# drscotthawley/SPNet

Hardware: AMD Instinct MI355X
Metric: training images/sec on 512×384 fake-ESPI, Xception backbone, 1/2/4/8 GPU (higher is better)
Workload: dtype f32 (bf16x3 MFMA for pointwise fwd/dgrad/wgrad GEMMs); 1 GPU; configs[1]: Xception, fake-ESPI 512x384 (HxW 384x512x1, model_type 'big'), batch 32 per GPU, full train step (augment+fwd+custom_loss+bwd+Adam+l2); global_batch=32, pool_frames_per_gpu=4096, parallelism=dp1, n_ranks_seen=1, devices_visible=1, wgrad_overlap=True

## Files before the change

### include/spnet_hip.h

```cpp
#ifndef SPNET_HIP_H
#define SPNET_HIP_H
#include <stdint.h>
#ifdef __cplusplus
extern "C" {
#endif

int spnet_gemm_f32(const float* A, int a_major, int lda, const float* B, int b_major, int ldb, float* C,
                   int ldc, int M, int N, int K, int split_k, float* workspace, long ws_floats,
                   const float* bias, int tile, void* stream);
long spnet_bf16x3_kp(int K);
long spnet_bf16x3_plane_elems(long R, int K);
int spnet_split_bf16x3(const float* W, void* planes, int K, int N, void* stream);
int spnet_split_rows_bf16x3(const float* A, long lda, void* planes, long R, int K, void* stream);
int spnet_split_bf16x3_batched(const void* jobs, int njobs, long max_elems, void* stream);
int spnet_gemm_bf16x3_fwd(const float* A, int lda, const void* planes, float* C, int ldc, int M, int N, int K, void* stream);
int spnet_gemm_bf16x3_fwd_colstats(const float* A, int lda, const void* planes, float* C, int ldc, int M, int N, int K,
                                   float* colstats, int* stat_rows, void* stream);
int spnet_gemm_bf16x3_pp(const void* a_planes, const void* b_planes, float* C, int ldc, int M, int N, int K, float* colstats,
                         int* stat_rows, void* stream);
long spnet_gemm_bf16x3_wgrad_ksplit(int cin, int cout, int M, int nbatch);
int spnet_gemm_bf16x3_pp_dwfwd(const void* z_planes, const void* w_planes, int B, int H, int W, int cin, int cout,
                               const float* scale_shift, int relu_next, const float* w_next, void* out_planes, void* stream);
long spnet_gemm_bf16x3_dwbwd_rows(long M);
long spnet_gemm_bf16x3_dwbwd_ok(int H, int W, int cin);
int spnet_gemm_bf16x3_pp_dwbwd(const void* dy_planes, const void* w_planes, int B, int H, int W, int cin, int cout,
                               const float* x_fwd, const float* w, float* dx, int relu_in, const float* add, float* partial,
                               const float* in_scale, const float* in_shift, const float* bn_mean, const float* bn_invstd,
                               float* bn_partial, const float* bn_x, void* stream);
int spnet_gemm_bf16x3_wgrad_batched(const void* jobs, int nbatch, int cin, int cout, int M, int ksplit, void* stream);
int spnet_gemm_f32_accumulate(const float* A, int a_major, int lda, const float* B, int b_major, int ldb, float* C,
                              int ldc, int M, int N, int K, int tile, void* stream);

int spnet_gemm_f32_colstats(const float* A, int a_major, int lda, const float* B, int b_major, int ldb,
                            float* C, int ldc, int M, int N, int K, int tile, float* colstats,
                            int* stat_rows, void* stream);
int spnet_gemm_f32_batched(const float* A0, const float* B0, float* C0, const long long* offsets, int nbatch,
                           int a_major, int lda, int b_major, int ldb, int ldc, int M, int N, int K, int tile,
                           void* stream);
long spnet_gemm_batched_ksplit(int M, int N, int K, int nbatch, int* tile_out);
int spnet_gemm_f32_batched_splitk(const float* A0, const float* B0, float* C0, const long long* offsets, int nbatch,
                                  int a_major, int lda, int b_major, int ldb, int ldc, int M, int N, int K, int tile,
                                  int ksplit, float* workspace, long ws_floats, void* stream);

int spnet_gemm_f32_bnblend(const float* g, const float* yp, const float* coef, int cld, int lda, const float* B,
                           int ldb, float* C, int ldc, int M, int N, int K, int tile, float* dy_out, void* stream);

int spnet_conv3x3_fwd(const float* x, const float* w, float* y, int B, int H, int W, int cin, int cout,
                      void* stream);
int spnet_conv3x3_dgrad(const float* dy, const float* w, float* dx, int B, int H, int W, int cin, int cout,
                        void* stream);
long spnet_conv3x3_wgrad_ws(int B, int H, int W, int cin, int cout);
int spnet_conv3x3_wgrad(const float* x, const float* dy, float* dw, int B, int H, int W, int cin, int cout,
                        float* workspace, long ws_floats, void* stream);
int spnet_transpose_batched(const void* jobs, int njobs, int max_rows, int max_cols, void* stream);
int spnet_reduce_slabs(const float* ws, int nslab, int M, int N, float* out, int ldc, void* stream);
int spnet_gather_s2(const float* x, float* xs, int B, int H, int W, int C, void* stream);
int spnet_scatter_add_s2(const float* dxs, float* dx, int B, int H, int W, int C, void* stream);

int spnet_reduce_rows(const float* in, int P, int L, float* out, void* stream);
int spnet_reduce_rows_ws(const float* in, int P, int L, float* out, float* scratch, long scratch_floats, void* stream);
int spnet_reduce_rows_batched(const void* jobs, int njobs, int max_L, void* stream);
long spnet_dwconv3x3_strided_ws(int B, int H, int W, int C, int stride);
int spnet_dwconv3x3_strided(int op, const float* a, const float* b, float* out, int B, int H, int W, int C, int stride,
                            float* workspace, void* stream);
int spnet_dwconv3x3_tiled_fwd(const float* x, const float* w, float* y, int B, int H, int W, int C,
                              int relu_in, const float* in_scale, const float* in_shift, void* stream);
int spnet_dwconv3x3_tiled_fwd_bnfin(const float* x, const float* w, float* y, int B, int H, int W, int C, int relu_in,
                                    const float* partial, int rows, long M, const float* gamma, const float* beta,
                                    float* moving_mean, float* moving_var, float* save_mean, float* save_invstd,
                                    float* scale_shift, float eps, float momentum, void* stream);
int spnet_dwconv3x3_tiled_fwd_x3(const float* x, const float* w, void* y_planes, int B, int H, int W, int C,
                                 int relu_in, const float* in_scale, const float* in_shift, void* stream);
int spnet_dwconv3x3_tiled_fwd_bnfin_x3(const float* x, const float* w, void* y_planes, int B, int H, int W, int C, int relu_in,
                                       const float* partial, int rows, long M, const float* gamma, const float* beta,
                                       float* moving_mean, float* moving_var, float* save_mean, float* save_invstd,
                                       float* scale_shift, float eps, float momentum, void* stream);
int spnet_dwconv3x3_stream_fwd_x3(const float* x, const float* w, void* y_planes, int B, int H, int W, int C, int relu_in,
                                  const float* in_scale, const float* in_shift, int rows_per_seg, void* stream);
long spnet_dwconv3x3_tiled_bwd_ws(int B, int H, int W, int C);
long spnet_dwconv3x3_tiled_rows(int B, int H, int W, int C);
int spnet_dwconv3x3_tiled_bwd(const float* dy, const float* x_fwd, const float* w, float* dx, float* dw,
                              int B, int H, int W, int C, int relu_in, const float* add, float* workspace,
                              const float* in_scale, const float* in_shift, const float* bn_mean,
                              const float* bn_invstd, float* bn_partial, const float* bn_x, void* stream);
long spnet_dwconv3x3_prefers_stream(int B, int H, int W, int C, int backward);
long spnet_dwconv3x3_stream_rows(int B, int H, int W, int C, int rows_per_seg);
long spnet_dwconv3x3_stream_bwd_ws(int B, int H, int W, int C, int rows_per_seg);
int spnet_dwconv3x3_stream_fwd(const float* x, const float* w, float* y, int B, int H, int W, int C, int relu_in,
                               const float* in_scale, const float* in_shift, int rows_per_seg, void* stream);
int spnet_dwconv3x3_stream_bwd(const float* dy, const float* x_fwd, const float* w, float* dx, float* dw, int B, int H,
                               int W, int C, int relu_in, const float* add, float* workspace, const float* in_scale,
                               const float* in_shift, const float* bn_mean, const float* bn_invstd, float* bn_partial,
                               const float* bn_x, int rows_per_seg, void* stream);

long spnet_bn_ws(long M, int C);
int spnet_bn_fwd_train(const float* x, long M, int C, const float* gamma, const float* beta,
                       float* moving_mean, float* moving_var, float* save_mean, float* save_invstd,
                       float* scale_shift, int act, const float* residual, int res_bcast, float* y,
                       float eps, float momentum, float* workspace, void* stream);
int spnet_bn_fwd_infer(const float* x, long M, int C, const float* gamma, const float* beta,
                       const float* moving_mean, const float* moving_var, float* scale_shift, int act,
                       const float* residual, int res_bcast, float* y, float eps, void* stream);
int spnet_bn_bwd(const float* x, const float* dy, long M, int C, const float* gamma, const float* beta,
                 const float* save_mean, const float* save_invstd, int act, float* dx, float* dgamma,
                 float* dbeta, float* coeffs, float* workspace, void* stream);
int spnet_bn_finalize_fwd(float* partial, int P, long M, int C, const float* gamma, const float* beta,
                          float* moving_mean, float* moving_var, float* save_mean, float* save_invstd,
                          float* scale_shift, float eps, float momentum, void* stream);
int spnet_bn_infer_coeffs(int C, const float* gamma, const float* beta, const float* moving_mean,
                          const float* moving_var, float* scale_shift, float eps, void* stream);
int spnet_bn_apply(const float* x, long M, int C, const float* scale_shift, int act, const float* residual,
                   int res_bcast, float* y, void* stream);
int spnet_bn_finalize_apply(float* partial, int P, const float* x, long M, int C, const float* gamma,
                            const float* beta, float* moving_mean, float* moving_var, float* save_mean,
                            float* save_invstd, float* scale_shift, int act, const float* residual, float* y, float eps,
                            float momentum, void* stream);
int spnet_bn_finalize_apply_ld(float* partial, int P, const float* x, long M, int C, const float* gamma,
                               const float* beta, float* moving_mean, float* moving_var, float* save_mean,
                               float* save_invstd, float* scale_shift, int act, const float* residual, float* y, long ldy,
                               float eps, float momentum, void* stream);
int spnet_bn_fwd_train_ld(const float* x, long M, int C, const float* gamma, const float* beta, float* moving_mean,
                          float* moving_var, float* save_mean, float* save_invstd, float* scale_shift, int act,
                          const float* residual, int res_bcast, float* y, long ldy, float eps, float momentum,
                          float* workspace, void* stream);
int spnet_bn_fwd_infer_ld(const float* x, long M, int C, const float* gamma, const float* beta, const float* moving_mean,
                          const float* moving_var, float* scale_shift, int act, const float* residual, int res_bcast,
                          float* y, long ldy, float eps, void* stream);
int spnet_bn_bwd_from_partials(const float* x, const float* dy, long M, int C, const float* gamma,
                               const float* beta, const float* save_mean, const float* save_invstd, int P,
                               const float* partial, float* dx, float* dgamma, float* dbeta, float* coeffs,
                               void* stream);
int spnet_bn_bwd_x3(const float* x, const float* dy, long M, int C, const float* gamma, const float* beta,
                    const float* save_mean, const float* save_invstd, int act, void* dx_planes, float* dgamma,
                    float* dbeta, float* coeffs, float* workspace, void* stream);
int spnet_bn_bwd_from_partials_x3(const float* x, const float* dy, long M, int C, const float* gamma,
                                  const float* beta, const float* save_mean, const float* save_invstd, int P,
                                  const float* partial, void* dx_planes, float* dgamma, float* dbeta, float* coeffs,
                                  void* stream);

int spnet_bn_bwd_coeffs_from_partials(int P, const float* partial, long M, int C, const float* gamma,
                                      const float* save_mean, const float* save_invstd, float* dgamma, float* dbeta,
                                      float* coef, int cld, void* stream);
int spnet_bn_bwd_coeffs(const float* x, const float* dy, long M, int C, const float* gamma, const float* beta,
                        const float* save_mean, const float* save_invstd, float* dgamma, float* dbeta, float* coef,
                        int cld, float* workspace, void* stream);

int spnet_maxpool3x3s2_add_fwd(const float* x, const float* residual, float* y, uint32_t* idx4, int B,
                               int H, int W, int C, const float* x_ss, const float* r_ss, void* stream);
int spnet_maxpool3x3s2_bwd(const float* dy, const uint32_t* idx4, float* dx, int B, int H, int W, int C,
                           void* stream);
long spnet_maxpool3x3s2_bwd_rows(int B, int H, int W, int C, int max_rows);
int spnet_maxpool3x3s2_bwd_bnsums(const float* dy, const uint32_t* idx4, float* dx, int B, int H, int W, int C,
                                  const float* yp, const float* mean, const float* invstd, float* partial, int rows,
                                  void* stream);
int spnet_avgpool2_fwd(const float* x, float* y, int B, int H, int W, int C, void* stream);
int spnet_avgpool2_bwd(const float* dy, float* dx, int B, int H, int W, int C, void* stream);

int spnet_maxpool3x3s2_valid_fwd(const float* x, float* y, uint32_t* idx4, int B, int H, int W, int C, void* stream);
int spnet_maxpool3x3s2_valid_bwd(const float* dy, const uint32_t* idx4, float* dx, int B, int H, int W, int C, void* stream);
int spnet_avgpool3x3s1_same(const float* in, float* out, int B, int H, int W, int C, int backward, void* stream);
int spnet_patches(const float* in, float* out, int B, int H, int W, int C, int KH, int KW, int stride, int same, int backward,
                  void* stream);
int spnet_patches_ld(const float* in, long ldx, float* out, int B, int H, int W, int C, int KH, int KW, int stride, int same,
                     void* stream);
int spnet_conv_gemm_f32(const float* x, long ldx, const float* Wk, float* y, int ldy, int B, int H, int W, int C, int Cout,
                        int KH, int KW, int stride, int same, const float* bias, int tile, float* colstats,
                        int* stat_rows, void* stream);
long spnet_grad_bnsums_rows(long npix, int max_rows);
int spnet_patches_bwd_bnsums(const float* dcol, float* dx, int B, int H, int W, int C, int KH, int KW, int stride, int same,
                             const float* y, const float* yp, const float* mean, const float* invstd, int relu,
                             float* partial, int rows, void* stream);
int spnet_copy_cols_bnsums(const float* src, int lds, float* dst, long M, int C, const float* y, long ldy, const float* yp,
                           const float* mean, const float* invstd, int relu, float* partial, int rows, void* stream);
int spnet_patches_bwd_bnsums_ld(const float* dcol, float* dx, long lddx, int B, int H, int W, int C, int KH, int KW, int stride,
                                int same, const float* y, long ldy, const float* yp, long ldyp, const float* mean,
                                const float* invstd, int relu, float* partial, long ldp, int rows, void* stream);
int spnet_copy_cols_bnsums_ld(const float* src, int lds, float* dst, long ldd, long M, int C, const float* y, long ldy,
                              const float* yp, long ldyp, const float* mean, const float* invstd, int relu, float* partial,
                              long ldp, int rows, void* stream);
int spnet_copy_cols_batched(const void* jobs, int njobs, long max_elems, void* stream);
int spnet_resadd(const float* x, const float* up, float* y, long n, float scale, int relu, void* stream);
int spnet_resadd_bwd(const float* y, const float* g, float* dx, float* dup, long n, float scale, int relu, void* stream);
int spnet_copy_cols(const float* src, int lds, float* dst, int ldd, long rows, int cols, int accumulate, void* stream);

int spnet_conv3x3_small(int op, int cin, int cout, int stride, int same, const float* a, const float* b,
                        float* out, int B, int H, int W, float* workspace, long ws_floats, void* stream);

int spnet_stem_head(int op, const float* x, const float* a, float* out, float* out2, int B, int H, int W,
                    float* workspace, long ws_floats, void* stream);

int spnet_ellipse_loss(const float* y_true, const float* y_pred, float* grad, float* parts,
                       float* loss_out, int B, int ncols, int hybrid, void* stream);
int spnet_selective_sigmoid(float* y, float* grad, int B, int ncols, int start, int step, int backward, void* stream);
int spnet_decode(const float* y_norm, const float* means, const float* ranges, float* out, int B,
                 int ncols, int sigmoid_noobj, void* stream);

int spnet_ellipse_iou(const float* yp, const float* yt, long npairs, int nx, int ny, double* iou, void* stream);

int spnet_calc_errors(const float* yp, const float* yt, long N, int ncols, int* counts, float* pix_err, void* stream);

int spnet_adam_step(float* p, const float* g, float* m, float* v, long n, long l2_n, float lr_t,
                    float beta1, float beta2, float eps, float l2, float grad_scale, const float* mask,
                    float* sq_scratch, float* l2_loss_out, const float* lr_t_dev, void* stream);
long spnet_adam_parts(long n);
int spnet_adam_part(float* p, const float* g, float* m, float* v, long n, long l2_n, float lr_t, float beta1, float beta2,
                    float eps, float l2, float grad_scale, const float* mask, float* sq_partial, const float* lr_t_dev,
                    void* stream);
int spnet_adam_l2_sum(const float* sq_partial, int count, float l2, float* l2_loss_out, void* stream);

int spnet_u8_to_input(const unsigned char* src, float* dst, long n, void* stream);
int spnet_resize_u8(const unsigned char* src, int N, int H, int W, const int* xtab, int xtaps, const int* ytab, int ytaps,
                    int OH, int OW, unsigned char* out_u8, float* out_f, void* stream);
int spnet_gather_rows(const float* src, long src_rows, const void* index, int idx_bytes, float* dst, int n, long L,
                      void* stream);

int spnet_minmax(const float* x, int N, long hw, float* mm, float* scratch, void* stream);
int spnet_cutout(const float* src, const int* src_index, float* dst, int N, int H, int W,
                 const int* rects, const float* vals, const int* nrect, void* stream);
int spnet_saltpepper(float* x, int N, int H, int W, const int* coords, int n_salt, int n_pepper,
                     const int* flag, const float* mm, void* stream);
int spnet_gaussian_blur(const float* src, float* dst, int N, int H, int W, const int* ksize, void* stream);
int spnet_warp_affine(const float* src, float* dst, int N, int H, int W, int C, const float* minv,
                      void* stream);
int spnet_warp_affine_fixed(const float* src, float* dst, int N, int H, int W, int C, const int* xrow, const int* xcol,
                            void* stream);
int spnet_warp_chain_u8(const unsigned char* src, int n_src, const int* sel, const void* params, int N, int H, int W,
                        unsigned char* out_u8, float* out_f, void* stream);
int spnet_dropout(const float* x, float* y, long n, unsigned seed, float rate, const unsigned* seed_dev,
                  void* stream);

int spnet_fake_espi(const float* waves, const float* nodes, const int* nnode, int N, int H, int W, unsigned seed,
                    int noise, float* out_f, unsigned char* out_u8, void* stream);

long spnet_bandpass_ws(int N, int H, int W);
int spnet_bandpass_project(const void* x, int x_kind, int N, int H, int W, const int* flip, float* win, float* ws,
                           void* stream);
int spnet_bandpass_apply(const void* x, int x_kind, const int* sel, int n_src, int N, int H, int W, const float* table,
                         int n_table, const int* row, const float* s, float* out_f, int f_kind, unsigned char* out_u8,
                         float* ws, void* stream);

int spnet_gemm_f32_bnrelu(const float* x, int ldx, const float* coef, int cld, const float* W, int ldw, float* Y, int ldy,
                          int M, int N, int K, int tile, float* colstats, int* stat_rows, void* stream);
int spnet_pad_nhwc(const float* in, float* out, int B, int H, int W, int C, int pt, int pb, int pl, int pr, int backward,
                   void* stream);
long spnet_dense_conv7_ws(int B, int H, int W);
int spnet_dense_conv7(int op, const float* a, const float* b, float* out, int B, int H, int W, float* workspace,
                      long ws_floats, void* stream);
long spnet_dense_rows(long M);
int spnet_dense_colsums_ld(const float* x, long ldx, long M, int C, float* partial, void* stream);
int spnet_dense_coeffs(int c, int cld, const float* gamma, const float* beta, const float* mean, const float* invstd,
                       const float* bmean, const float* bvar, float* mm, float* mv, float* coef, float eps, float momentum,
                       int training, void* stream);
int spnet_dense_apply_ld(const float* x, long ldx, long M, int C, const float* coef, int cld, int relu, float* y, long ldy,
                         void* stream);
int spnet_dense_consumer_bwd(const float* dz, long ldz, const float* x, long ldx, long M, int c, const float* coef, int cld,
                             const float* mean, const float* invstd, const float* gamma, int relu, float* G, long ldg,
                             float* partial, void* stream);
int spnet_dense_consumer_fin(const float* partial, int P, int c, const float* gamma, float* dgamma, float* dbeta, float* u,
                             float* v, void* stream);
int spnet_dense_producer_fin(const float* G, long ldg, const float* u, const float* v, const float* x, long ldx,
                             const float* mean, const float* invstd, long M, int c0, int c1, float* out, long ldo,
                             void* stream);

#ifdef __cplusplus
}
#endif
#endif
```

### spnet_amd/_lib.py

```python
import ctypes
import os
from ctypes import POINTER, byref, c_float, c_int, c_long, c_uint, c_void_p

_HERE = os.path.dirname(os.path.abspath(__file__))
LIB_PATH = os.environ.get("SPNET_HIP_LIB") or os.path.join(_HERE, "lib", "libspnet_hip.so")

if not os.path.exists(LIB_PATH):
    raise ImportError(
        "spnet_amd: %s is missing -- build it with `python -c 'import __graft_entry__ as g; g.build()'` "
        "or `make -C spnet_amd/csrc` (hipcc, gfx950).  There is no CPU fallback." % LIB_PATH)

import numpy as np
import torch

_lib = ctypes.CDLL(LIB_PATH)

P = c_void_p

_SIGS = {
    "spnet_gemm_f32": (c_int, [P, c_int, c_int, P, c_int, c_int, P, c_int, c_int, c_int, c_int, c_int, P, c_long, P, c_int, P]),
    "spnet_bf16x3_kp": (c_long, [c_int]),
    "spnet_bf16x3_plane_elems": (c_long, [c_long, c_int]),
    "spnet_split_bf16x3": (c_int, [P, P, c_int, c_int, P]),
    "spnet_split_rows_bf16x3": (c_int, [P, c_long, P, c_long, c_int, P]),
    "spnet_gemm_bf16x3_pp": (c_int, [P, P, P, c_int, c_int, c_int, c_int, P, P, P]),
    "spnet_gemm_bf16x3_wgrad_ksplit": (c_long, [c_int, c_int, c_int, c_int]),
    "spnet_gemm_bf16x3_dwbwd_rows": (c_long, [c_long]),
    "spnet_gemm_bf16x3_dwbwd_ok": (c_long, [c_int, c_int, c_int]),
    "spnet_gemm_bf16x3_pp_dwbwd": (c_int, [P, P, c_int, c_int, c_int, c_int, c_int, P, P, P, c_int, P, P, P, P, P, P, P, P, P]),
    "spnet_gemm_bf16x3_pp_dwfwd": (c_int, [P, P, c_int, c_int, c_int, c_int, c_int, P, c_int, P, P, P]),
    "spnet_gemm_bf16x3_wgrad_batched": (c_int, [P, c_int, c_int, c_int, c_int, c_int, P]),
    "spnet_split_bf16x3_batched": (c_int, [P, c_int, c_long, P]),
    "spnet_gemm_bf16x3_fwd": (c_int, [P, c_int, P, P, c_int, c_int, c_int, c_int, P]),
    "spnet_gemm_bf16x3_fwd_colstats": (c_int, [P, c_int, P, P, c_int, c_int, c_int, c_int, P, P, P]),
    "spnet_gemm_f32_accumulate": (c_int, [P, c_int, c_int, P, c_int, c_int, P, c_int, c_int, c_int, c_int, c_int, P]),
    "spnet_conv3x3_fwd": (c_int, [P, P, P, c_int, c_int, c_int, c_int, c_int, P]),
    "spnet_conv3x3_dgrad": (c_int, [P, P, P, c_int, c_int, c_int, c_int, c_int, P]),
    "spnet_conv3x3_wgrad_ws": (c_long, [c_int, c_int, c_int, c_int, c_int]),
    "spnet_conv3x3_wgrad": (c_int, [P, P, P, c_int, c_int, c_int, c_int, c_int, P, c_long, P]),
    "spnet_reduce_slabs": (c_int, [P, c_int, c_int, c_int, P, c_int, P]),
    "spnet_transpose_batched": (c_int, [P, c_int, c_int, c_int, P]),
    "spnet_gather_s2": (c_int, [P, P, c_int, c_int, c_int, c_int, P]),
    "spnet_scatter_add_s2": (c_int, [P, P, c_int, c_int, c_int, c_int, P]),
    "spnet_dwconv3x3_strided_ws": (c_long, [c_int, c_int, c_int, c_int, c_int]),
    "spnet_dwconv3x3_strided": (c_int, [c_int, P, P, P, c_int, c_int, c_int, c_int, c_int, P, P]),
    "spnet_reduce_rows": (c_int, [P, c_int, c_int, P, P]),
    "spnet_reduce_rows_ws": (c_int, [P, c_int, c_int, P, P, c_long, P]),
    "spnet_reduce_rows_batched": (c_int, [P, c_int, c_int, P]),
    "spnet_dwconv3x3_tiled_fwd": (c_int, [P, P, P, c_int, c_int, c_int, c_int, c_int, P, P, P]),
    "spnet_dwconv3x3_tiled_fwd_bnfin": (c_int, [P, P, P, c_int, c_int, c_int, c_int, c_int, P, c_int, c_long, P, P, P, P, P, P, P,
                                                c_float, c_float, P]),
    "spnet_dwconv3x3_tiled_fwd_x3": (c_int, [P, P, P, c_int, c_int, c_int, c_int, c_int, P, P, P]),
    "spnet_dwconv3x3_tiled_fwd_bnfin_x3": (c_int, [P, P, P, c_int, c_int, c_int, c_int, c_int, P, c_int, c_long, P, P, P, P, P, P, P,
                                                   c_float, c_float, P]),
    "spnet_dwconv3x3_stream_fwd_x3": (c_int, [P, P, P, c_int, c_int, c_int, c_int, c_int, P, P, c_int, P]),
    "spnet_dwconv3x3_tiled_bwd_ws": (c_long, [c_int, c_int, c_int, c_int]),
    "spnet_dwconv3x3_tiled_rows": (c_long, [c_int, c_int, c_int, c_int]),
    "spnet_dwconv3x3_tiled_bwd": (c_int, [P, P, P, P, P, c_int, c_int, c_int, c_int, c_int, P, P, P, P, P, P, P, P, P]),
    "spnet_dwconv3x3_prefers_stream": (c_long, [c_int, c_int, c_int, c_int, c_int]),
    "spnet_dwconv3x3_stream_rows": (c_long, [c_int, c_int, c_int, c_int, c_int]),
    "spnet_dwconv3x3_stream_bwd_ws": (c_long, [c_int, c_int, c_int, c_int, c_int]),
    "spnet_dwconv3x3_stream_fwd": (c_int, [P, P, P, c_int, c_int, c_int, c_int, c_int, P, P, c_int, P]),
    "spnet_dwconv3x3_stream_bwd": (c_int, [P, P, P, P, P, c_int, c_int, c_int, c_int, c_int, P, P, P, P, P, P, P, P, c_int, P]),
    "spnet_bn_finalize_fwd": (c_int, [P, c_int, c_long, c_int, P, P, P, P, P, P, P, c_float, c_float, P]),
    "spnet_bn_infer_coeffs": (c_int, [c_int, P, P, P, P, P, c_float, P]),
    "spnet_bn_apply": (c_int, [P, c_long, c_int, P, c_int, P, c_int, P, P]),
    "spnet_bn_finalize_apply": (c_int, [P, c_int, P, c_long, c_int, P, P, P, P, P, P, P, c_int, P, P, c_float, c_float, P]),
    "spnet_bn_finalize_apply_ld": (c_int, [P, c_int, P, c_long, c_int, P, P, P, P, P, P, P, c_int, P, P, c_long, c_float, c_float, P]),
    "spnet_bn_bwd_from_partials": (c_int, [P, P, c_long, c_int, P, P, P, P, c_int, P, P, P, P, P, P]),
    "spnet_bn_bwd_from_partials_x3": (c_int, [P, P, c_long, c_int, P, P, P, P, c_int, P, P, P, P, P, P]),
    "spnet_bn_bwd_x3": (c_int, [P, P, c_long, c_int, P, P, P, P, c_int, P, P, P, P, P, P]),
    "spnet_gemm_f32_colstats": (c_int, [P, c_int, c_int, P, c_int, c_int, P, c_int, c_int, c_int, c_int, c_int, P, P, P]),
    "spnet_gemm_f32_bnblend": (c_int, [P, P, P, c_int, c_int, P, c_int, P, c_int, c_int, c_int, c_int, c_int, P, P]),
    "spnet_bn_bwd_coeffs_from_partials": (c_int, [c_int, P, c_long, c_int, P, P, P, P, P, P, c_int, P]),
    "spnet_bn_bwd_coeffs": (c_int, [P, P, c_long, c_int, P, P, P, P, P, P, P, c_int, P, P]),
    "spnet_gemm_f32_batched": (c_int, [P, P, P, P, c_int, c_int, c_int, c_int, c_int, c_int, c_int, c_int, c_int, c_int, P]),
    "spnet_gemm_batched_ksplit": (c_long, [c_int, c_int, c_int, c_int, P]),
    "spnet_gemm_f32_batched_splitk": (c_int, [P, P, P, P, c_int, c_int, c_int, c_int, c_int, c_int, c_int, c_int, c_int, c_int,
                                              c_int, P, c_long, P]),
    "spnet_bn_ws": (c_long, [c_long, c_int]),
    "spnet_bn_fwd_train": (c_int, [P, c_long, c_int, P, P, P, P, P, P, P, c_int, P, c_int, P, c_float, c_float, P, P]),
    "spnet_bn_fwd_infer": (c_int, [P, c_long, c_int, P, P, P, P, P, c_int, P, c_int, P, c_float, P]),
    "spnet_bn_fwd_train_ld": (c_int, [P, c_long, c_int, P, P, P, P, P, P, P, c_int, P, c_int, P, c_long, c_float, c_float, P, P]),
    "spnet_bn_fwd_infer_ld": (c_int, [P, c_long, c_int, P, P, P, P, P, c_int, P, c_int, P, c_long, c_float, P]),
    "spnet_bn_bwd": (c_int, [P, P, c_long, c_int, P, P, P, P, c_int, P, P, P, P, P, P]),
    "spnet_maxpool3x3s2_add_fwd": (c_int, [P, P, P, P, c_int, c_int, c_int, c_int, P, P, P]),
    "spnet_maxpool3x3s2_bwd": (c_int, [P, P, P, c_int, c_int, c_int, c_int, P]),
    "spnet_maxpool3x3s2_bwd_rows": (c_long, [c_int, c_int, c_int, c_int, c_int]),
    "spnet_maxpool3x3s2_bwd_bnsums": (c_int, [P, P, P, c_int, c_int, c_int, c_int, P, P, P, P, c_int, P]),
    "spnet_maxpool3x3s2_valid_fwd": (c_int, [P, P, P, c_int, c_int, c_int, c_int, P]),
    "spnet_maxpool3x3s2_valid_bwd": (c_int, [P, P, P, c_int, c_int, c_int, c_int, P]),
    "spnet_avgpool3x3s1_same": (c_int, [P, P, c_int, c_int, c_int, c_int, c_int, P]),
    "spnet_patches": (c_int, [P, P, c_int, c_int, c_int, c_int, c_int, c_int, c_int, c_int, c_int, P]),
    "spnet_patches_ld": (c_int, [P, c_long, P, c_int, c_int, c_int, c_int, c_int, c_int, c_int, c_int, P]),
    "spnet_conv_gemm_f32": (c_int, [P, c_long, P, P, c_int, c_int, c_int, c_int, c_int, c_int, c_int, c_int, c_int, c_int, P, c_int, P, P, P]),
    "spnet_grad_bnsums_rows": (c_long, [c_long, c_int]),
    "spnet_patches_bwd_bnsums": (c_int, [P, P, c_int, c_int, c_int, c_int, c_int, c_int, c_int, c_int, P, P, P, P, c_int, P,
                                         c_int, P]),
    "spnet_copy_cols_bnsums": (c_int, [P, c_int, P, c_long, c_int, P, c_long, P, P, P, c_int, P, c_int, P]),
    "spnet_patches_bwd_bnsums_ld": (c_int, [P, P, c_long, c_int, c_int, c_int, c_int, c_int, c_int, c_int, c_int, P, c_long, P,
                                            c_long, P, P, c_int, P, c_long, c_int, P]),
    "spnet_copy_cols_bnsums_ld": (c_int, [P, c_int, P, c_long, c_long, c_int, P, c_long, P, c_long, P, P, c_int, P, c_long,
                                          c_int, P]),
    "spnet_copy_cols_batched": (c_int, [P, c_int, c_long, P]),
    "spnet_resadd": (c_int, [P, P, P, c_long, c_float, c_int, P]),
    "spnet_resadd_bwd": (c_int, [P, P, P, P, c_long, c_float, c_int, P]),
    "spnet_copy_cols": (c_int, [P, c_int, P, c_int, c_long, c_int, c_int, P]),
    "spnet_avgpool2_fwd": (c_int, [P, P, c_int, c_int, c_int, c_int, P]),
    "spnet_avgpool2_bwd": (c_int, [P, P, c_int, c_int, c_int, c_int, P]),
    "spnet_conv3x3_small": (c_int, [c_int, c_int, c_int, c_int, c_int, P, P, P, c_int, c_int, c_int, P, c_long, P]),
    "spnet_stem_head": (c_int, [c_int, P, P, P, P, c_int, c_int, c_int, P, c_long, P]),
    "spnet_ellipse_loss": (c_int, [P, P, P, P, P, c_int, c_int, c_int, P]),
    "spnet_selective_sigmoid": (c_int, [P, P, c_int, c_int, c_int, c_int, c_int, P]),
    "spnet_decode": (c_int, [P, P, P, P, c_int, c_int, c_int, P]),
    "spnet_ellipse_iou": (c_int, [P, P, c_long, c_int, c_int, P, P]),
    "spnet_calc_errors": (c_int, [P, P, c_long, c_int, P, P, P]),
    "spnet_adam_step": (c_int, [P, P, P, P, c_long, c_long, c_float, c_float, c_float, c_float, c_float, c_float, P, P, P, P, P]),
    "spnet_adam_parts": (c_long, [c_long]),
    "spnet_adam_part": (c_int, [P, P, P, P, c_long, c_long, c_float, c_float, c_float, c_float, c_float, c_float, P, P, P, P]),
    "spnet_adam_l2_sum": (c_int, [P, c_int, c_float, P, P]),
    "spnet_u8_to_input": (c_int, [P, P, c_long, P]),
    "spnet_resize_u8": (c_int, [P, c_int, c_int, c_int, P, c_int, P, c_int, c_int, c_int, P, P, P]),
    "spnet_gather_rows": (c_int, [P, c_long, P, c_int, P, c_int, c_long, P]),
    "spnet_minmax": (c_int, [P, c_int, c_long, P, P, P]),
    "spnet_cutout": (c_int, [P, P, P, c_int, c_int, c_int, P, P, P, P]),
    "spnet_saltpepper": (c_int, [P, c_int, c_int, c_int, P, c_int, c_int, P, P, P]),
    "spnet_gaussian_blur": (c_int, [P, P, c_int, c_int, c_int, P, P]),
    "spnet_warp_affine": (c_int, [P, P, c_int, c_int, c_int, c_int, P, P]),
    "spnet_warp_affine_fixed": (c_int, [P, P, c_int, c_int, c_int, c_int, P, P, P]),
    "spnet_warp_chain_u8": (c_int, [P, c_int, P, P, c_int, c_int, c_int, P, P, P]),
    "spnet_fake_espi": (c_int, [P, P, P, c_int, c_int, c_int, c_uint, c_int, P, P, P]),
    "spnet_dropout": (c_int, [P, P, c_long, c_uint, c_float, P, P]),
    "spnet_bandpass_ws": (c_long, [c_int, c_int, c_int]),
    "spnet_bandpass_project": (c_int, [P, c_int, c_int, c_int, c_int, P, P, P, P]),
    "spnet_bandpass_apply": (c_int, [P, c_int, P, c_int, c_int, c_int, c_int, P, c_int, P, P, P, c_int, P, P, P]),
    "spnet_gemm_f32_bnrelu": (c_int, [P, c_int, P, c_int, P, c_int, P, c_int, c_int, c_int, c_int, c_int, P, P, P]),
    "spnet_pad_nhwc": (c_int, [P, P, c_int, c_int, c_int, c_int, c_int, c_int, c_int, c_int, c_int, P]),
    "spnet_dense_conv7_ws": (c_long, [c_int, c_int, c_int]),
    "spnet_dense_conv7": (c_int, [c_int, P, P, P, c_int, c_int, c_int, P, c_long, P]),
    "spnet_dense_rows": (c_long, [c_long]),
    "spnet_dense_colsums_ld": (c_int, [P, c_long, c_long, c_int, P, P]),
    "spnet_dense_coeffs": (c_int, [c_int, c_int, P, P, P, P, P, P, P, P, P, c_float, c_float, c_int, P]),
    "spnet_dense_apply_ld": (c_int, [P, c_long, c_long, c_int, P, c_int, c_int, P, c_long, P]),
    "spnet_dense_consumer_bwd": (c_int, [P, c_long, P, c_long, c_long, c_int, P, c_int, P, P, P, c_int, P, c_long, P, P]),
    "spnet_dense_consumer_fin": (c_int, [P, c_int, c_int, P, P, P, P, P, P]),
    "spnet_dense_producer_fin": (c_int, [P, c_long, P, P, P, c_long, P, P, c_long, c_int, c_int, P, c_long, P]),
}

EXPORTS = tuple(_SIGS)


class HipError(RuntimeError):
    pass


_TRACER = [None]


def set_tracer(tracer):
    _TRACER[0] = tracer


def _bind(name, restype, argtypes):
    fn = getattr(_lib, name)
    fn.restype = restype
    fn.argtypes = argtypes
    if restype is not c_int:
        return fn

    def checked(*args):
        tr = _TRACER[0]
        if tr is None:
            rc = fn(*args)
        else:
            tok = tr(name, args, None)
            rc = fn(*args)
            tr(name, args, tok)
        if rc != 0:
            raise HipError("%s failed with hipError_t %d" % (name, rc))
    checked.__name__ = name
    return checked


for _n, (_r, _a) in _SIGS.items():
    globals()[_n] = _bind(_n, _r, _a)


def _public_stream():
    return torch.cuda.current_stream().cuda_stream


def _resolve_current_stream():
    raw = getattr(torch._C, "_cuda_getCurrentRawStream", None)
    dev = getattr(torch._C, "_cuda_getDevice", None)
    if raw is None or dev is None:
        return _public_stream, "public"
    return (lambda: raw(dev())), "raw"


current_stream, STREAM_ACCESSOR = _resolve_current_stream()


def gather_rows(src, index, dst):
    n = int(index.numel())
    rows = int(src.shape[0])
    L_ = src.numel() // max(rows, 1)
    if dst.numel() != n * L_ or src.dtype != torch.float32 or dst.dtype != torch.float32 or not (src.is_contiguous() and dst.is_contiguous()):
        raise ValueError("gather_rows: shape / dtype / layout mismatch")
    ib = {torch.int32: 4, torch.int64: 8}[index.dtype]
    spnet_gather_rows(src.data_ptr(), rows, index.data_ptr(), ib, dst.data_ptr(), n, L_, current_stream())


def ptr(t):
    return None if t is None else t.data_ptr()


class AsyncUploader:

    def __init__(self, device, depth=None):
        self.device = device
        self.depth = int(os.environ.get("SPNET_UPLOAD_DEPTH", "1")) if depth is None else depth
        self.rings, self.count = {}, {}

# ... 18 lines not shown
```

### spnet_amd/csrc/bn.hip

```cpp
#include "x3t.h"

#define BN_MAX_PARTS 256

__device__ __forceinline__ float act_fwd(float v, int act) {
  if (act == 1) return fmaxf(v, 0.f);
  if (act == 2) return v > 0.f ? v : 0.1f * v;
  if (act == 3) return fminf(fmaxf(v, 0.f), 6.f);
  return v;
}
__device__ __forceinline__ float act_grad(float out_pre, int act) {
  if (act == 1) return out_pre > 0.f ? 1.f : 0.f;
  if (act == 2) return out_pre > 0.f ? 1.f : 0.1f;
  if (act == 3) return (out_pre > 0.f && out_pre < 6.f) ? 1.f : 0.f;
  return 1.f;
}

template <int MODE>
__global__ __launch_bounds__(256) void bn_partial_vec_kernel(
    const float* __restrict__ x, const float* __restrict__ dy, long M, int C,
    const float* __restrict__ mean, const float* __restrict__ invstd,
    const float* __restrict__ gamma, const float* __restrict__ beta, int act,
    float* __restrict__ partial) {
  extern __shared__ __attribute__((aligned(16))) float4 red4[];
  const int c4n = C >> 2;
// ... 668 lines not shown
                       const float* beta, const float* save_mean, const float* save_invstd,
                       int act, float* dx, unsigned short* planes, float* dgamma, float* dbeta, float* coeffs,
                       float* workspace, void* stream) {
  hipStream_t st = (hipStream_t)stream;
  if ((C & 3) && C > 4) return (int)hipErrorInvalidValue;
  if (planes && !bn_planes_ok(planes, M, C)) return (int)hipErrorInvalidValue;
  const long ps = x3t_plane_elems(M, C);
  const int parts = bn_parts(M, C);
  launch_partial<1>(x, dy, M, C, save_mean, save_invstd, gamma, beta, act, workspace, parts, st);
  if (!(C & 3) && bn_fuse_ok(parts, M, C)) {
    const int rps = bn_fuse_rows_per_slab(M, C);
    const int chunks = (C + BN_FUSE_CH - 1) / BN_FUSE_CH;
    dim3 grid((unsigned)(chunks * ((M + rps - 1) / rps)));
    hipLaunchKernelGGL(bn_bwd_fused_vec_kernel, grid, dim3(256), 0, st, x, dy, M, C, workspace, parts, gamma, beta,
                       save_mean, save_invstd, act, dgamma, dbeta, dx, rps, chunks, planes, ps);
    SPNET_RETURN_LAUNCH_STATUS();
  }
  hipLaunchKernelGGL(bn_bwd_finalize_kernel<0>, dim3((C + BN_FIN_CH - 1) / BN_FIN_CH), dim3(256), 0, st, workspace, parts,
                     C, M, gamma, save_invstd, save_mean, dgamma, dbeta, coeffs, coeffs + C, coeffs + 2 * C);
  if (C & 3) {
    const long n = M * C;
    hipLaunchKernelGGL(bn_bwd_apply_scalar_kernel, dim3(spnet_ew_grid(n, 256)), dim3(256), 0, st, x,
                       dy, n, C, save_mean, save_invstd, gamma, beta, act, coeffs, coeffs + C,
                       coeffs + 2 * C, dx);
  } else {
    const long n4 = M * (C / 4);
    hipLaunchKernelGGL(bn_bwd_apply_vec_kernel, dim3(spnet_ew_grid(n4, 256)), dim3(256), 0, st, x, dy,
                       M, C, save_mean, save_invstd, gamma, beta, act, coeffs, coeffs + C,
                       coeffs + 2 * C, dx, planes, ps);
  }
  SPNET_RETURN_LAUNCH_STATUS();
}
extern "C" int spnet_bn_bwd(const float* x, const float* dy, long M, int C, const float* gamma,
                            const float* beta, const float* save_mean, const float* save_invstd,
                            int act, float* dx, float* dgamma, float* dbeta, float* coeffs,
                            float* workspace, void* stream) {
  return bn_bwd_impl(x, dy, M, C, gamma, beta, save_mean, save_invstd, act, dx, nullptr, dgamma, dbeta, coeffs, workspace, stream);
}
extern "C" int spnet_bn_bwd_x3(const float* x, const float* dy, long M, int C, const float* gamma,
                               const float* beta, const float* save_mean, const float* save_invstd,
                               int act, void* dx_planes, float* dgamma, float* dbeta, float* coeffs,
                               float* workspace, void* stream) {
  if (!dx_planes) return (int)hipErrorInvalidValue;
  return bn_bwd_impl(x, dy, M, C, gamma, beta, save_mean, save_invstd, act, nullptr, reinterpret_cast<unsigned short*>(dx_planes),
                     dgamma, dbeta, coeffs, workspace, stream);
}


extern "C" int spnet_bn_finalize_fwd(float* partial, int P, long M, int C, const float* gamma,
                                     const float* beta, float* moving_mean, float* moving_var,
                                     float* save_mean, float* save_invstd, float* scale_shift, float eps,
                                     float momentum, void* stream) {
  const unsigned gx = (C + BN_FIN_CH - 1) / BN_FIN_CH;
  if (P >= BN_SLICE_MIN_P) {
    const int L = P / BN_SLICES, S = BN_SLICES;
    hipLaunchKernelGGL(bn_slice_partials_kernel, dim3(gx, S), dim3(256), 0, (hipStream_t)stream,
                       partial, P, C, L, S);
    hipLaunchKernelGGL(bn_fwd_finalize_kernel, dim3(gx), dim3(256), 0, (hipStream_t)stream, partial, S, C, M, gamma,
                       beta, moving_mean, moving_var, save_mean, save_invstd, scale_shift, scale_shift + C, eps,
                       momentum, L);
    SPNET_RETURN_LAUNCH_STATUS();
  }
  hipLaunchKernelGGL(bn_fwd_finalize_kernel, dim3(gx), dim3(256), 0,
                     (hipStream_t)stream, partial, P, C, M, gamma, beta, moving_mean, moving_var, save_mean,
                     save_invstd, scale_shift, scale_shift + C, eps, momentum, 0);
  SPNET_RETURN_LAUNCH_STATUS();
}

extern "C" int spnet_bn_infer_coeffs(int C, const float* gamma, const float* beta, const float* moving_mean,
                                     const float* moving_var, float* scale_shift, float eps, void* stream) {
  hipLaunchKernelGGL(bn_infer_coeffs_kernel, dim3((C + 255) / 256), dim3(256), 0, (hipStream_t)stream, C, gamma,
                     beta, moving_mean, moving_var, scale_shift, scale_shift + C, eps);
  SPNET_RETURN_LAUNCH_STATUS();
}

extern "C" int spnet_bn_apply(const float* x, long M, int C, const float* scale_shift, int act,
                              const float* residual, int res_bcast, float* y, void* stream) {
  if ((C & 3) && C > 4) return (int)hipErrorInvalidValue;
  if (res_bcast && !(C & 3)) return (int)hipErrorInvalidValue;
  launch_apply(x, M, C, scale_shift, scale_shift + C, act, residual, res_bcast, y, (hipStream_t)stream);
  SPNET_RETURN_LAUNCH_STATUS();
}

extern "C" int spnet_bn_finalize_apply_ld(float* partial, int P, const float* x, long M, int C, const float* gamma,
                                          const float* beta, float* moving_mean, float* moving_var, float* save_mean,
                                          float* save_invstd, float* scale_shift, int act, const float* residual, float* y,
                                          long ldy, float eps, float momentum, void* stream) {
  hipStream_t st = (hipStream_t)stream;
  if ((C & 3) || P < 1 || (ldy & 3) || ldy < C) return (int)hipErrorInvalidValue;
  if (bn_fuse_ok(P, M, C)) {
    const int rps = bn_fuse_rows_per_slab(M, C);
    const int chunks = (C + BN_FUSE_CH - 1) / BN_FUSE_CH;
    dim3 grid((unsigned)(chunks * ((M + rps - 1) / rps)));
    hipLaunchKernelGGL(bn_fwd_fused_vec_kernel, grid, dim3(256), 0, st, x, M, C, partial, P, gamma, beta, moving_mean,
                       moving_var, save_mean, save_invstd, scale_shift, scale_shift + C, eps, momentum, act, residual, y,
                       rps, chunks, ldy);
    SPNET_RETURN_LAUNCH_STATUS();
  }
  {
    const int rc = spnet_bn_finalize_fwd(partial, P, M, C, gamma, beta, moving_mean, moving_var, save_mean, save_invstd,
                                         scale_shift, eps, momentum, stream);
    if (rc) return rc;
  }
  launch_apply(x, M, C, scale_shift, scale_shift + C, act, residual, 0, y, st, ldy);
  SPNET_RETURN_LAUNCH_STATUS();
}
extern "C" int spnet_bn_finalize_apply(float* partial, int P, const float* x, long M, int C, const float* gamma,
                                       const float* beta, float* moving_mean, float* moving_var, float* save_mean,
                                       float* save_invstd, float* scale_shift, int act, const float* residual, float* y,
                                       float eps, float momentum, void* stream) {
  return spnet_bn_finalize_apply_ld(partial, P, x, M, C, gamma, beta, moving_mean, moving_var, save_mean, save_invstd,
                                    scale_shift, act, residual, y, C, eps, momentum, stream);
}

static int bn_bwd_from_partials_impl(const float* x, const float* dy, long M, int C, const float* gamma,
                                     const float* beta, const float* save_mean,
                                     const float* save_invstd, int P, const float* partial, float* dx, unsigned short* planes,
                                     float* dgamma, float* dbeta, float* coeffs, void* stream) {
  hipStream_t st = (hipStream_t)stream;
  if (C & 3) return (int)hipErrorInvalidValue;
  if (planes && !bn_planes_ok(planes, M, C)) return (int)hipErrorInvalidValue;
  const long ps = x3t_plane_elems(M, C);
  if (bn_fuse_ok(P, M, C)) {
    const int rps = bn_fuse_rows_per_slab(M, C);
    const int chunks = (C + BN_FUSE_CH - 1) / BN_FUSE_CH;
    dim3 grid((unsigned)(chunks * ((M + rps - 1) / rps)));
    hipLaunchKernelGGL(bn_bwd_fused_vec_kernel, grid, dim3(256), 0, st, x, dy, M, C, partial, P, gamma, beta, save_mean,
                       save_invstd, 0, dgamma, dbeta, dx, rps, chunks, planes, ps);
    SPNET_RETURN_LAUNCH_STATUS();
  }
  hipLaunchKernelGGL(bn_bwd_finalize_kernel<0>, dim3((C + BN_FIN_CH - 1) / BN_FIN_CH), dim3(256), 0, st, partial, P,
                     C, M, gamma, save_invstd, save_mean, dgamma, dbeta, coeffs, coeffs + C, coeffs + 2 * C);
  const long n4 = M * (C / 4);
  hipLaunchKernelGGL(bn_bwd_apply_vec_kernel, dim3(spnet_ew_grid(n4, 256)), dim3(256), 0, st, x, dy, M, C,
                     save_mean, save_invstd, gamma, beta, 0, coeffs, coeffs + C, coeffs + 2 * C, dx, planes, ps);
  SPNET_RETURN_LAUNCH_STATUS();
}
extern "C" int spnet_bn_bwd_from_partials(const float* x, const float* dy, long M, int C, const float* gamma,
                                          const float* beta, const float* save_mean,
                                          const float* save_invstd, int P, const float* partial, float* dx,
                                          float* dgamma, float* dbeta, float* coeffs, void* stream) {
  return bn_bwd_from_partials_impl(x, dy, M, C, gamma, beta, save_mean, save_invstd, P, partial, dx, nullptr, dgamma, dbeta,
                                   coeffs, stream);
}
extern "C" int spnet_bn_bwd_from_partials_x3(const float* x, const float* dy, long M, int C, const float* gamma,
                                             const float* beta, const float* save_mean,
                                             const float* save_invstd, int P, const float* partial, void* dx_planes,
                                             float* dgamma, float* dbeta, float* coeffs, void* stream) {
  if (!dx_planes) return (int)hipErrorInvalidValue;
  return bn_bwd_from_partials_impl(x, dy, M, C, gamma, beta, save_mean, save_invstd, P, partial, nullptr,
                                   reinterpret_cast<unsigned short*>(dx_planes), dgamma, dbeta, coeffs, stream);
}

extern "C" int spnet_bn_bwd_coeffs_from_partials(int P, const float* partial, long M, int C, const float* gamma,
                                                 const float* save_mean, const float* save_invstd, float* dgamma,
                                                 float* dbeta, float* coef, int cld, void* stream) {
  if (cld < C || !coef) return (int)hipErrorInvalidValue;
  hipLaunchKernelGGL(bn_bwd_finalize_kernel<1>, dim3((C + BN_FIN_CH - 1) / BN_FIN_CH), dim3(256), 0, (hipStream_t)stream,
                     partial, P, C, M, gamma, save_invstd, save_mean, dgamma, dbeta, coef, coef + cld, coef + 2 * cld);
  SPNET_RETURN_LAUNCH_STATUS();
}

extern "C" int spnet_bn_bwd_coeffs(const float* x, const float* dy, long M, int C, const float* gamma,
                                   const float* beta, const float* save_mean, const float* save_invstd,
                                   float* dgamma, float* dbeta, float* coef, int cld, float* workspace, void* stream) {
  hipStream_t st = (hipStream_t)stream;
  if ((C & 3) || cld < C || !coef) return (int)hipErrorInvalidValue;
  const int parts = bn_parts(M, C);
  launch_partial<1>(x, dy, M, C, save_mean, save_invstd, gamma, beta, 0, workspace, parts, st);
  hipLaunchKernelGGL(bn_bwd_finalize_kernel<1>, dim3((C + BN_FIN_CH - 1) / BN_FIN_CH), dim3(256), 0, st, workspace, parts,
                     C, M, gamma, save_invstd, save_mean, dgamma, dbeta, coef, coef + cld, coef + 2 * cld);
  SPNET_RETURN_LAUNCH_STATUS();
}
```

### spnet_amd/csrc/common.h

```cpp
#pragma once
#include <hip/hip_runtime.h>
#include <stdint.h>

#define SPNET_WAVE 64

static inline int spnet_cdiv(long a, long b) { return (int)((a + b - 1) / b); }

#define SPNET_RETURN_LAUNCH_STATUS()            \
  do {                                          \
    hipError_t e__ = hipGetLastError();         \
    return (int)e__;                            \
  } while (0)

static inline int spnet_ew_grid(long n_items, int block) {
  long g = (n_items + block - 1) / block;
  if (g > 2048 * 4) g = 2048 * 4;
  if (g < 1) g = 1;
  return (int)g;
}

__device__ __forceinline__ float wave_sum(float v) {
#pragma unroll
  for (int off = 32; off > 0; off >>= 1) v += __shfl_xor(v, off, 64);
  return v;
}
__device__ __forceinline__ float wave_max(float v) {
#pragma unroll
  for (int off = 32; off > 0; off >>= 1) v = fmaxf(v, __shfl_xor(v, off, 64));
  return v;
}
__device__ __forceinline__ float wave_min(float v) {
#pragma unroll
  for (int off = 32; off > 0; off >>= 1) v = fminf(v, __shfl_xor(v, off, 64));
  return v;
}

__device__ __forceinline__ float spnet_u8_to_input_f(unsigned v) {
  return __fmul_rn(__fsub_rn(__fdiv_rn((float)v, 255.f), 0.5f), 2.f);
}

__device__ __forceinline__ float bn_moving_update(float moving, float momentum, float value) {
  return __fadd_rn(__fmul_rn(momentum, moving), __fmul_rn(1.f - momentum, value));
}

__device__ __forceinline__ float bn_shift(float beta, float mean, float scale) {
  return __fsub_rn(beta, __fmul_rn(mean, scale));
}

struct BnChannelStats {
  float mean, invstd, scale, shift, unbiased_var;
};
__device__ __forceinline__ BnChannelStats bn_channel_stats(double s, double q, long M, float gamma, float beta, float eps) {
  BnChannelStats r;
  const double mean = s / (double)M;
  double var = __dsub_rn(q / (double)M, __dmul_rn(mean, mean));
  if (var < 0.0) var = 0.0;
  r.mean = (float)mean;
  r.invstd = (float)(1.0 / sqrt(__dadd_rn(var, (double)eps)));
  r.scale = __fmul_rn(gamma, r.invstd);
  r.shift = bn_shift(beta, r.mean, r.scale);
  r.unbiased_var = (float)((M > 1) ? __dmul_rn(var, (double)M / (double)(M - 1)) : var);
  return r;
}

__device__ __forceinline__ int xcd_remap(int bid, int nblk) {
  const int nx = 8;
  int q = nblk / nx, r = nblk % nx;
  int x = bid % nx, i = bid / nx;
  int base = (x < r) ? x * (q + 1) : r * (q + 1) + (x - r) * q;
  return base + i;
}
```

### spnet_amd/csrc/gemm_bf16x3.hip

```cpp
#include "x3t.h"
#include <type_traits>

typedef short bf16x8 __attribute__((ext_vector_type(8)));
typedef short bf16x4 __attribute__((ext_vector_type(4)));
typedef float f32x4v __attribute__((ext_vector_type(4)));
typedef __attribute__((address_space(3))) void* lds_ptr_t;
typedef __attribute__((address_space(3))) bf16x4* lds_b64_t;

#define X3_BM 96
#define X3_BN 96
#define X3_LDR 32
#define X3_SWZ(ROW_, CHUNK_) ((((CHUNK_) ^ (0 - ((ROW_) >> 2))) & 3) * 8)
#define X3_PLANE (X3_BM * X3_LDR)
#define X3_STEP (6 * X3_PLANE)
#define X3_PIECES 36
#define X3_PER 9
#define X3_NDMA X3_PER

__device__ __forceinline__ void x3_split_job(const float* __restrict__ W, unsigned short* __restrict__ planes, int K, long N,
                                             long sn, long sk) {
  const int nk = (K + 31) / 32;
  const long npieces = ((N + 15) / 16) * nk, ps = npieces * 512;
  const int lane = threadIdx.x & 63, wave = threadIdx.x >> 6;
  const int r16 = lane >> 2, chunk = ((lane & 3) ^ (0 - (r16 >> 2))) & 3;
  const bool vec = sk == 1 && !(sn & 3) && !((uintptr_t)W & 15);
  for (long piece = (long)blockIdx.x * 4 + wave; piece < npieces; piece += (long)gridDim.x * 4) {
    const long n = (piece / nk) * 16 + r16;
    const int k0 = (int)(piece % nk) * 32 + chunk * 8;
    float v[8];
    if (vec && n < N && k0 + 8 <= K) {
      const float4 a = *reinterpret_cast<const float4*>(W + n * sn + k0), b = *reinterpret_cast<const float4*>(W + n * sn + k0 + 4);
      v[0] = a.x; v[1] = a.y; v[2] = a.z; v[3] = a.w; v[4] = b.x; v[5] = b.y; v[6] = b.z; v[7] = b.w;
    } else {
#pragma unroll
      for (int e = 0; e < 8; ++e) v[e] = (n < N && k0 + e < K) ? W[n * sn + (long)(k0 + e) * sk] : 0.f;
    }
    uint4 h, m, l;
    x3_split_pk(v[0], v[1], h.x, m.x, l.x);
    x3_split_pk(v[2], v[3], h.y, m.y, l.y);
    x3_split_pk(v[4], v[5], h.z, m.z, l.z);
    x3_split_pk(v[6], v[7], h.w, m.w, l.w);
    unsigned short* dst = planes + piece * 512 + lane * 8;
    *reinterpret_cast<uint4*>(dst) = h;
    *reinterpret_cast<uint4*>(dst + ps) = m;
    *reinterpret_cast<uint4*>(dst + 2 * ps) = l;
  }
}
__global__ __launch_bounds__(256) void split_bf16x3_tiled_kernel(const long long* __restrict__ jobs) {
  const long long* jb = jobs + 6 * blockIdx.y;
  x3_split_job(reinterpret_cast<const float*>(jb[0]), reinterpret_cast<unsigned short*>(jb[1]), (int)jb[2], jb[3], jb[4], jb[5]);
}
__global__ __launch_bounds__(256) void split_bf16x3_one_kernel(const float* __restrict__ W, unsigned short* __restrict__ planes,
                                                               int K, long N, long sn, long sk) {
  x3_split_job(W, planes, K, N, sn, sk);
}

#define X3_DMA(SOFF_, KSTRIDE_A_, KSTRIDE_B_, KS_, BUF_)                                                       \
  do {                                                                                                         \
    unsigned short* base_ = smem + ((BUF_) & 1) * X3_STEP;                                                     \
    _Pragma("unroll") for (int i = 0; i < X3_PER; ++i) {                                                       \
      const int c = wave + 4 * i;                                                                              \
      const bool is_a = i < 4 ? true : (i > 4 ? false : (c < 18));                                             \
      const __amdgpu_buffer_rsrc_t rs_ = is_a ? rs_a : rs_b;                                                   \
      __builtin_amdgcn_raw_ptr_buffer_load_lds(rs_, (lds_ptr_t)(base_ + c * 512), 16, lane * 16,               \
                                               SOFF_[i] + (KS_) * (is_a ? (KSTRIDE_A_) : (KSTRIDE_B_)), 0, 0); \
    }                                                                                                          \
  } while (0)
#define X3_MFMA(FA_, FB_)                                                                                      \
  _Pragma("unroll") for (int t = 0; t < 6; ++t)                                                                \
  _Pragma("unroll") for (int i = 0; i < 3; ++i)                                                                \
  _Pragma("unroll") for (int j = 0; j < 3; ++j)                                                                \
      acc[i][j] = __builtin_amdgcn_mfma_f32_16x16x32_bf16(FA_[i][TA[t]], FB_[j][TB[t]], acc[i][j], 0, 0, 0)
#define X3_BODY(KS_, CA_, CB_, NA_, NB_, DMA_, RD_, READ_, RPG_)                                               \
  do {                                                                                                         \
    __syncthreads();                                                        \
    if (DMA_) X3_ISSUE((KS_) + 2, (KS_));                                                                      \
    if (RD_) READ_((KS_) + 1, NA_, NB_);                                                                       \
    X3_MFMA(CA_, CB_);                                                                                         \
    if ((DMA_) && (RD_)) {                                                                                     \
      _Pragma("unroll") for (int g = 0; g < 18; ++g) {                                                         \
        __builtin_amdgcn_sched_group_barrier(0x008, 1, 0);                                                     \
        if (g % 2 == 0 && g / 2 < X3_NDMA) __builtin_amdgcn_sched_group_barrier(0x020, 1, 0);                  \
        __builtin_amdgcn_sched_group_barrier(0x008, 1, 0);                                                     \
        __builtin_amdgcn_sched_group_barrier(0x100, RPG_, 0);                                                  \
        __builtin_amdgcn_sched_group_barrier(0x008, 1, 0);                                                     \
      }                                                                                                        \
    }                                                                                                          \
    __builtin_amdgcn_sched_barrier(0);                                                                         \
  } while (0)
#define X3_PIPELINE(NSTEPS_, READ_, RPG_)                                                                      \
  do {                                                                                                         \
    bf16x8 xa[3][3], xb[3][3], ya[3][3], yb[3][3];                                                             \
    X3_ISSUE(0, 0);                                                                                            \
    if ((NSTEPS_) > 1) {                                                                                       \
      X3_ISSUE(1, 1);                                                                                          \
      asm volatile("s_waitcnt vmcnt(%0)" ::"n"(X3_NDMA) : "memory");                                            \
    } else {                                                                                                   \
      asm volatile("s_waitcnt vmcnt(0)" ::: "memory");                                                         \
    }                                                                                                          \
    __builtin_amdgcn_s_barrier();                                                                              \
    READ_(0, xa, xb);                                                                                          \
    int ks = 0;                                                                                                \
    for (; ks + 3 < (NSTEPS_); ks += 2) {                                                                      \
      X3_BODY(ks, xa, xb, ya, yb, true, true, READ_, RPG_);                                                    \
      X3_BODY(ks + 1, ya, yb, xa, xb, true, true, READ_, RPG_);                                                \
    }                                                                                                          \
    for (; ks < (NSTEPS_); ks += 2) {                                                                          \
      if (ks + 2 < (NSTEPS_)) X3_BODY(ks, xa, xb, ya, yb, true, true, READ_, RPG_);                            \
      else if (ks + 1 < (NSTEPS_)) X3_BODY(ks, xa, xb, ya, yb, false, true, READ_, RPG_);                      \
      else X3_BODY(ks, xa, xb, ya, yb, false, false, READ_, RPG_);                                             \
      if (ks + 1 < (NSTEPS_)) {                                                                                \
        if (ks + 3 < (NSTEPS_)) X3_BODY(ks + 1, ya, yb, xa, xb, true, true, READ_, RPG_);                      \
        else if (ks + 2 < (NSTEPS_)) X3_BODY(ks + 1, ya, yb, xa, xb, false, true, READ_, RPG_);                \
        else X3_BODY(ks + 1, ya, yb, xa, xb, false, false, READ_, RPG_);                                       \
      }                                                                                                        \
    }                                                                                                          \
  } while (0)

#define X3_STORE_C(C_, LDC_, ROW0_, COL0_, MROWS_, NCOLS_)                                                     \
  _Pragma("unroll") for (int i = 0; i < 3; ++i)                                                                \
  _Pragma("unroll") for (int r = 0; r < 4; ++r) {                                                              \
    const int row = (ROW0_) + wm * 48 + i * 16 + kg * 4 + r;                                                   \
    if (row < (MROWS_)) {                                                                                      \
      _Pragma("unroll") for (int j = 0; j < 3; ++j) {                                                          \
        const int col = (COL0_) + wn * 48 + j * 16 + p16;                                                      \
        if (col < (NCOLS_)) (C_)[(long)row * (LDC_) + col] = acc[i][j][r];                                     \
      }                                                                                                        \
    }                                                                                                          \
  }

#define X3_COLSTATS()                                                                                          \
  do {                                                                                                         \
    __syncthreads();                                                                                           \
    float* sred = reinterpret_cast<float*>(smem);                              \
    _Pragma("unroll") for (int j = 0; j < 3; ++j) {                                                            \
      float sv = 0.f, qv = 0.f;                                                                                \
      _Pragma("unroll") for (int i = 0; i < 3; ++i)                                                            \
      _Pragma("unroll") for (int r = 0; r < 4; ++r) {                                                          \
        const int row = m0 + wm * 48 + i * 16 + kg * 4 + r;                                                    \
        const float v = row < M ? acc[i][j][r] : 0.f;                                                          \
        sv += v;                                                                                               \
        qv = fmaf(v, v, qv);                                                                                   \
      }                                                                                                        \
      sv += __shfl_xor(sv, 16, 64); qv += __shfl_xor(qv, 16, 64);                                              \
      sv += __shfl_xor(sv, 32, 64); qv += __shfl_xor(qv, 32, 64);                                              \
      if (lane < 16) {                                                                                         \
        const int cl = wn * 48 + j * 16 + p16;                                                                 \
        sred[(0 * 2 + wm) * X3_BN + cl] = sv;                                                                  \
        sred[(1 * 2 + wm) * X3_BN + cl] = qv;                                                                  \
      }                                                                                                        \
    }                                                                                                          \
    __syncthreads();                                                                                           \
    if (tid < 2 * X3_BN) {                                                                                     \
      const int q = tid / X3_BN, cl = tid % X3_BN, col = n0 + cl;                                              \
      if (col < N) colstats[((long)tm * 2 + q) * N + col] = sred[(q * 2 + 0) * X3_BN + cl] + sred[(q * 2 + 1) * X3_BN + cl]; \
    }                                                                                                          \
  } while (0)

__global__ __launch_bounds__(256, 2) void gemm_bf16x3_pp_kernel(const unsigned short* __restrict__ Ap, long a_ps,
                                                                const unsigned short* __restrict__ Bp, long b_ps,
                                                                float* __restrict__ C, int ldc, int M, int N, int nk, int tiles_n,
                                                                float* __restrict__ colstats) {
  __shared__ __attribute__((aligned(16))) unsigned short smem[2 * X3_STEP];
  const int tid = threadIdx.x, lane = tid & 63;
  const int wave = __builtin_amdgcn_readfirstlane(tid >> 6);
  const int wm = wave >> 1, wn = wave & 1;
  const int lid = xcd_remap(blockIdx.x, gridDim.x);
  const int tn = lid % tiles_n, tm = lid / tiles_n;
  const int m0 = tm * X3_BM, n0 = tn * X3_BN;
  const int rg_a = (M + 15) / 16, rg_b = (N + 15) / 16;
  const __amdgpu_buffer_rsrc_t rs_a = __builtin_amdgcn_make_buffer_rsrc((void*)Ap, 0, (int)(3 * a_ps * 2), 0x00020000);
  const __amdgpu_buffer_rsrc_t rs_b = __builtin_amdgcn_make_buffer_rsrc((void*)Bp, 0, (int)(3 * b_ps * 2), 0x00020000);
  int soff[X3_PER];
#pragma unroll
  for (int i = 0; i < X3_PER; ++i) {
    const int c = wave + 4 * i;
    soff[i] = c < 18 ? (int)(((c / 6) * a_ps + (long)min(m0 / 16 + c % 6, rg_a - 1) * nk * 512) * 2)
                     : (int)((((c - 18) / 6) * b_ps + (long)min(n0 / 16 + (c - 18) % 6, rg_b - 1) * nk * 512) * 2);
  }
#define X3_ISSUE(KS_, BUF_) X3_DMA(soff, 1024, 1024, KS_, BUF_)
  f32x4v acc[3][3];
#pragma unroll
  for (int i = 0; i < 3; ++i)
#pragma unroll
    for (int j = 0; j < 3; ++j)
#pragma unroll
      for (int r = 0; r < 4; ++r) acc[i][j][r] = 0.f;
  const int p16 = lane & 15, kg = lane >> 4;
  constexpr int TA[6] = {2, 1, 0, 1, 0, 0}, TB[6] = {0, 1, 2, 0, 1, 0};
  const int a_off = (wm * 48 + p16) * X3_LDR + X3_SWZ(p16, kg);
  const int b_off = (3 * X3_BM + wn * 48 + p16) * X3_LDR + X3_SWZ(p16, kg);
#define X3_READ_ROWS(KS_, FA_, FB_)                                                                            \
  do {                                                                                                         \
    const unsigned short* base_ = smem + ((KS_) & 1) * X3_STEP;                                                \
    _Pragma("unroll") for (int p = 0; p < 3; ++p)                                                              \
    _Pragma("unroll") for (int t = 0; t < 3; ++t) {                                                            \
      FA_[t][p] = *reinterpret_cast<const bf16x8*>(base_ + a_off + (p * X3_BM + t * 16) * X3_LDR);             \
      FB_[t][p] = *reinterpret_cast<const bf16x8*>(base_ + b_off + (p * X3_BN + t * 16) * X3_LDR);             \
    }                                                                                                          \
  } while (0)
  X3_PIPELINE(nk, X3_READ_ROWS, 1);
#undef X3_ISSUE
  X3_STORE_C(C, ldc, m0, n0, M, N);
  if (colstats) X3_COLSTATS();
}

#undef X3_NDMA
#define X3_NDMA 7
#define FB_BM 192
#define FB_STEP (3 * (FB_BM + X3_BN) * X3_LDR)
#define FB_LD 100
template <int MODE, bool ADD, bool BNX>
__global__ __launch_bounds__(512, 2) void gemm_bf16x3_pp_dwbwd_kernel(
    const unsigned short* __restrict__ Ap, long a_ps, const unsigned short* __restrict__ Bp, long b_ps, int M, int N, int nk,
    int tiles_n, int H, int W, const float* __restrict__ x, const float* __restrict__ wt, float* __restrict__ dx, int relu_in,
    const float* __restrict__ add, float* __restrict__ partial, const float* __restrict__ in_scale,
    const float* __restrict__ in_shift, const float* __restrict__ bn_mean, const float* __restrict__ bn_invstd,
    float* __restrict__ bn_partial, const float* __restrict__ bn_x, unsigned short* __restrict__ out_planes, long out_ps) {
  __shared__ __attribute__((aligned(16))) unsigned short smem[2 * FB_STEP];
  const int tid = threadIdx.x, lane = tid & 63;
  const int wave = __builtin_amdgcn_readfirstlane(tid >> 6);
  const int wm = wave >> 1, wn = wave & 1;
  const int lid = xcd_remap(blockIdx.x, gridDim.x);
  const int tn = lid % tiles_n, tm = lid / tiles_n;
  const int m0 = tm * FB_BM, n0 = tn * X3_BN;
  const int rg_a = (M + 15) / 16, rg_b = (N + 15) / 16;
  const __amdgpu_buffer_rsrc_t rs_a = __builtin_amdgcn_make_buffer_rsrc((void*)Ap, 0, (int)(3 * a_ps * 2), 0x00020000);
  const __amdgpu_buffer_rsrc_t rs_b = __builtin_amdgcn_make_buffer_rsrc((void*)Bp, 0, (int)(3 * b_ps * 2), 0x00020000);
  int soff[X3_NDMA];
#pragma unroll
  for (int i = 0; i < X3_NDMA; ++i) {
    const int c = min(wave + 8 * i, 53);
    soff[i] = c < 36 ? (int)(((c / 12) * a_ps + (long)min(m0 / 16 + c % 12, rg_a - 1) * nk * 512) * 2)
                     : (int)((((c - 36) / 6) * b_ps + (long)min(n0 / 16 + (c - 36) % 6, rg_b - 1) * nk * 512) * 2);
  }
#define X3_ISSUE(KS_, BUF_)                                                                                    \
  do {                                                                                                         \
    unsigned short* base_ = smem + ((BUF_) & 1) * FB_STEP;                                                     \
    _Pragma("unroll") for (int i = 0; i < X3_NDMA; ++i) {                                                      \
      const int c = min(wave + 8 * i, 53);                                                                     \
      const bool is_a = i < 4 ? true : (i > 4 ? false : (c < 36));                                             \
      const __amdgpu_buffer_rsrc_t rs_ = is_a ? rs_a : rs_b;                                                   \
      __builtin_amdgcn_raw_ptr_buffer_load_lds(rs_, (lds_ptr_t)(base_ + c * 512), 16, lane * 16,               \
                                               soff[i] + (KS_) * 1024, 0, 0);                                  \
    }                                                                                                          \
  } while (0)
  f32x4v acc[3][3];
#pragma unroll
  for (int i = 0; i < 3; ++i)
#pragma unroll
    for (int j = 0; j < 3; ++j)
#pragma unroll
      for (int r = 0; r < 4; ++r) acc[i][j][r] = 0.f;
  const int p16 = lane & 15, kg = lane >> 4;
  constexpr int TA[6] = {2, 1, 0, 1, 0, 0}, TB[6] = {0, 1, 2, 0, 1, 0};
  const int a_off = (wm * 48 + p16) * X3_LDR + X3_SWZ(p16, kg);
  const int b_off = (3 * FB_BM + wn * 48 + p16) * X3_LDR + X3_SWZ(p16, kg);
#define FB_READ_ROWS(KS_, FA_, FB_)                                                                            \
  do {                                                                                                         \
    const unsigned short* base_ = smem + ((KS_) & 1) * FB_STEP;                                                \
    _Pragma("unroll") for (int p = 0; p < 3; ++p)                                                              \
    _Pragma("unroll") for (int t = 0; t < 3; ++t) {                                                            \
      FA_[t][p] = *reinterpret_cast<const bf16x8*>(base_ + a_off + (p * FB_BM + t * 16) * X3_LDR);             \
      FB_[t][p] = *reinterpret_cast<const bf16x8*>(base_ + b_off + (p * X3_BN + t * 16) * X3_LDR);             \
    }                                                                                                          \
  } while (0)
  X3_PIPELINE(nk, FB_READ_ROWS, 1);
#undef X3_ISSUE

#ifdef FB_SKIP_EPILOGUE
  {
    float keep = 0.f;
#pragma unroll
    for (int i = 0; i < 3; ++i)
#pragma unroll
      for (int j = 0; j < 3; ++j)
#pragma unroll
        for (int r = 0; r < 4; ++r) keep += acc[i][j][r];
    if (keep == 1.2345f) dx[0] = keep;
    return;
  }
#endif
  if constexpr (MODE == 1) {
    typedef float v4 __attribute__((ext_vector_type(4)));
    const v4 zero = {0.f, 0.f, 0.f, 0.f};
    __syncthreads();
    float* ct = reinterpret_cast<float*>(smem);
    float scv[3], shv[3];
#pragma unroll
    for (int j = 0; j < 3; ++j) {
      const int col = min(n0 + wn * 48 + j * 16 + p16, N - 1);
      scv[j] = in_scale ? in_scale[col] : 1.f;
      shv[j] = in_scale ? in_shift[col] : 0.f;
    }
#pragma unroll
    for (int i = 0; i < 3; ++i)
#pragma unroll
      for (int r = 0; r < 4; ++r)
#pragma unroll
        for (int j = 0; j < 3; ++j) {
          float v = acc[i][j][r];
          if (in_scale) v = fmaf(v, scv[j], shv[j]);
          if (relu_in) v = fmaxf(v, 0.f);
          ct[(wm * 48 + i * 16 + kg * 4 + r) * FB_LD + wn * 48 + j * 16 + p16] = v;
        }
    const int cq = tid & 31, pg = tid >> 5;
    const int c = n0 + cq * 4;
    const bool active = cq < 24 && c < N;
    const int nk_out = (N + 31) >> 5;
    auto walk_fwd = [&](auto ph_tag, auto pw_tag) {
      constexpr int PH = decltype(ph_tag)::value, PW = decltype(pw_tag)::value, HW = PH * PW;
      constexpr int WALKS = (FB_BM / PH) / 16;
      v4 k[9];
      const int cc = active ? c : 0;
#pragma unroll
      for (int tp = 0; tp < 9; ++tp) k[tp] = *reinterpret_cast<const v4*>(wt + (long)tp * N + cc);
      __syncthreads();
#define FB_FMA(D_, A_, B_) D_ = v4{fmaf(A_.x, B_.x, D_.x), fmaf(A_.y, B_.y, D_.y), fmaf(A_.z, B_.z, D_.z), fmaf(A_.w, B_.w, D_.w)}
#pragma unroll
      for (int wk = 0; wk < WALKS; ++wk) {
        const int col = pg + 16 * wk, img = col / PW, w = col % PW;
        const int base = img * HW + w;
        const bool ok = active && m0 + img * HW < M;
        const float* col0 = ct + base * FB_LD + cq * 4;
        const int ol = w > 0 ? -FB_LD : 0, orr = w < PW - 1 ? FB_LD : 0;
        const float fl = w > 0 ? 1.f : 0.f, fr = w < PW - 1 ? 1.f : 0.f;
        v4 a_prev = zero, a_cur = zero;
#pragma unroll
        for (int r = -1; r <= PH; ++r) {
          v4 v0 = zero, v1 = zero, v2 = zero;
          if (r >= 0 && r < PH) {
            const float* rp = col0 + r * PW * FB_LD;
            v0 = *reinterpret_cast<const v4*>(rp + ol) * fl;
            v1 = *reinterpret_cast<const v4*>(rp);
            v2 = *reinterpret_cast<const v4*>(rp + orr) * fr;
          }
          FB_FMA(a_prev, v0, k[6]); FB_FMA(a_prev, v1, k[7]); FB_FMA(a_prev, v2, k[8]);
          FB_FMA(a_cur, v0, k[3]); FB_FMA(a_cur, v1, k[4]); FB_FMA(a_cur, v2, k[5]);
          v4 a_next = v0 * k[0];
          FB_FMA(a_next, v1, k[1]); FB_FMA(a_next, v2, k[2]);
          const int t = r - 1;
          if (t >= 0 && t < PH && ok)
            x3t_store4(out_planes, out_ps, x3t_off(m0 + base + t * PW, c, nk_out), a_prev.x, a_prev.y, a_prev.z, a_prev.w);
          a_prev = a_cur;
          a_cur = a_next;
        }
      }
#undef FB_FMA
    };
    if (H == 12) walk_fwd(std::integral_constant<int, 12>{}, std::integral_constant<int, 16>{});
    else walk_fwd(std::integral_constant<int, 6>{}, std::integral_constant<int, 8>{});
    return;
  }
  __syncthreads();
  float* ct = reinterpret_cast<float*>(smem);
#pragma unroll
  for (int i = 0; i < 3; ++i)
#pragma unroll
    for (int r = 0; r < 4; ++r)
#pragma unroll
      for (int j = 0; j < 3; ++j)
        ct[(wm * 48 + i * 16 + kg * 4 + r) * FB_LD + wn * 48 + j * 16 + p16] = acc[i][j][r];
  const int cq = tid & 31, pg = tid >> 5;
  const int c = n0 + cq * 4;
  const bool active = cq < 24 && c < N;
  typedef float v4 __attribute__((ext_vector_type(4)));
  const v4 zero = {0.f, 0.f, 0.f, 0.f};
  v4 accw[9], bsg = zero, bsgx = zero;
#pragma unroll
  for (int tp = 0; tp < 9; ++tp) accw[tp] = zero;
  auto walk_columns = [&](auto ph_tag, auto pw_tag) {
    constexpr int PH = decltype(ph_tag)::value, PW = decltype(pw_tag)::value, HW = PH * PW;
    constexpr int WALKS = (FB_BM / PH) / 16;
    static_assert(PH * WALKS == 12, "12 pixels per thread");
    v4 xq[12], aq[ADD ? 12 : 1], bq[BNX ? 12 : 1];
    int base[WALKS];
    bool ok[WALKS], lft[WALKS], rgt[WALKS];
#pragma unroll
    for (int wk = 0; wk < WALKS; ++wk) {
      const int col = pg + 16 * wk, img = col / PW, w = col % PW;
      base[wk] = img * HW + w;
      ok[wk] = active && m0 + img * HW < M;
      lft[wk] = w > 0;
      rgt[wk] = w < PW - 1;
#pragma unroll
      for (int h = 0; h < PH; ++h) {
        const long o = (long)(m0 + (ok[wk] ? base[wk] + h * PW : 0)) * N + (active ? c : 0);
        xq[wk * PH + h] = *reinterpret_cast<const v4*>(x + o);
        if (ADD) aq[wk * PH + h] = *reinterpret_cast<const v4*>(add + o);
        if (BNX) bq[wk * PH + h] = *reinterpret_cast<const v4*>(bn_x + o);
      }
    }
    v4 k[9], sc = {1.f, 1.f, 1.f, 1.f}, sh = zero, mu = zero, is = zero;
    const int cc = active ? c : 0;
#pragma unroll
    for (int tp = 0; tp < 9; ++tp) k[tp] = *reinterpret_cast<const v4*>(wt + (long)tp * N + cc);
    const bool affine = in_scale != nullptr;
    if (affine) { sc = *reinterpret_cast<const v4*>(in_scale + cc); sh = *reinterpret_cast<const v4*>(in_shift + cc); }
    if (bn_partial) { mu = *reinterpret_cast<const v4*>(bn_mean + cc); is = *reinterpret_cast<const v4*>(bn_invstd + cc); }
    __syncthreads();
#define FB_FMA(D_, A_, B_) D_ = v4{fmaf(A_.x, B_.x, D_.x), fmaf(A_.y, B_.y, D_.y), fmaf(A_.z, B_.z, D_.z), fmaf(A_.w, B_.w, D_.w)}
#pragma unroll
    for (int wk = 0; wk < WALKS; ++wk) {
      const float* col0 = ct + base[wk] * FB_LD + cq * 4;
      const int ol = lft[wk] ? -FB_LD : 0, orr = rgt[wk] ? FB_LD : 0;
      const float fl = lft[wk] ? 1.f : 0.f, fr = rgt[wk] ? 1.f : 0.f;
      v4 m0_ = zero, m1 = zero, m2 = zero;
      v4 c0 = *reinterpret_cast<const v4*>(col0 + ol) * fl, c1 = *reinterpret_cast<const v4*>(col0),
         c2 = *reinterpret_cast<const v4*>(col0 + orr) * fr;
#pragma unroll
      for (int h = 0; h < PH; ++h) {
        v4 n0_ = zero, n1 = zero, n2 = zero;
        if (h + 1 < PH) {
          const float* rn = col0 + (h + 1) * PW * FB_LD;
          n0_ = *reinterpret_cast<const v4*>(rn + ol) * fl;
          n1 = *reinterpret_cast<const v4*>(rn);
          n2 = *reinterpret_cast<const v4*>(rn + orr) * fr;
        }
        const v4 raw = xq[wk * PH + h];
        v4 a = raw;
        if (affine) a = v4{fmaf(raw.x, sc.x, sh.x), fmaf(raw.y, sc.y, sh.y), fmaf(raw.z, sc.z, sh.z), fmaf(raw.w, sc.w, sh.w)};
        const v4 xin = relu_in ? v4{fmaxf(a.x, 0.f), fmaxf(a.y, 0.f), fmaxf(a.z, 0.f), fmaxf(a.w, 0.f)} : a;
        v4 res = n2 * k[0];
        FB_FMA(res, n1, k[1]); FB_FMA(res, n0_, k[2]);
        FB_FMA(res, c2, k[3]); FB_FMA(res, c1, k[4]); FB_FMA(res, c0, k[5]);
        FB_FMA(res, m2, k[6]); FB_FMA(res, m1, k[7]); FB_FMA(res, m0_, k[8]);
        if (relu_in) res = v4{a.x > 0.f ? res.x : 0.f, a.y > 0.f ? res.y : 0.f, a.z > 0.f ? res.z : 0.f, a.w > 0.f ? res.w : 0.f};
        if (ADD) res += aq[wk * PH + h];
        if (ok[wk]) {
          FB_FMA(accw[0], xin, n2); FB_FMA(accw[1], xin, n1); FB_FMA(accw[2], xin, n0_);
          FB_FMA(accw[3], xin, c2); FB_FMA(accw[4], xin, c1); FB_FMA(accw[5], xin, c0);
          FB_FMA(accw[6], xin, m2); FB_FMA(accw[7], xin, m1); FB_FMA(accw[8], xin, m0_);
          *reinterpret_cast<v4*>(dx + (long)(m0 + base[wk] + h * PW) * N + c) = res;
          if (bn_partial) {
            const v4 pre = BNX ? bq[wk * PH + h] : raw;
            bsg += res;
            bsgx = v4{fmaf(res.x, (pre.x - mu.x) * is.x, bsgx.x), fmaf(res.y, (pre.y - mu.y) * is.y, bsgx.y),
                      fmaf(res.z, (pre.z - mu.z) * is.z, bsgx.z), fmaf(res.w, (pre.w - mu.w) * is.w, bsgx.w)};
          }
        }
        m0_ = c0; m1 = c1; m2 = c2;
        c0 = n0_; c1 = n1; c2 = n2;
      }
    }
  };
  if (H == 12) walk_columns(std::integral_constant<int, 12>{}, std::integral_constant<int, 16>{});
  else walk_columns(std::integral_constant<int, 6>{}, std::integral_constant<int, 8>{});
  __syncthreads();
  v4* red = reinterpret_cast<v4*>(smem);
#pragma unroll
  for (int tp = 0; tp < 9; ++tp) red[(tp * 16 + pg) * 32 + cq] = accw[tp];
  red[(9 * 16 + pg) * 32 + cq] = bsg;
  red[(10 * 16 + pg) * 32 + cq] = bsgx;
  __syncthreads();
  for (int q = tid; q < 11 * 32; q += 512) {
    const int tp = q / 32, ll = q % 32, co = n0 + ll * 4;
    if (ll < 24 && co < N && (tp < 9 || bn_partial)) {
      v4 sum = red[(tp * 16) * 32 + ll];
      for (int g = 1; g < 16; ++g) sum += red[(tp * 16 + g) * 32 + ll];
      if (tp < 9) *reinterpret_cast<v4*>(partial + ((long)tm * 9 + tp) * N + co) = sum;
      else *reinterpret_cast<v4*>(bn_partial + ((long)tm * 2 + (tp - 9)) * N + co) = sum;
    }
  }
}
#undef X3_NDMA
#define X3_NDMA X3_PER

__global__ __launch_bounds__(256, 2) void gemm_bf16x3_wgrad_kernel(const long long* __restrict__ jobs, int cin, int cout, int M,
                                                                   int tiles_n, int tiles, int nbatch, int steps_per_slice) {
  __shared__ __attribute__((aligned(16))) unsigned short smem[2 * X3_STEP];
  const int wid = xcd_remap(blockIdx.x, gridDim.x);
  const int lid = wid % tiles, job = (wid / tiles) % nbatch, slice = wid / (tiles * nbatch);
  const long long* jb = jobs + 3 * job;
  const unsigned short* __restrict__ Zp = reinterpret_cast<const unsigned short*>(jb[0]);
  const unsigned short* __restrict__ Gp = reinterpret_cast<const unsigned short*>(jb[1]);
  float* __restrict__ dst = reinterpret_cast<float*>(jb[2]) + (long)slice * cin * cout;
  const int tid = threadIdx.x, lane = tid & 63;
  const int wave = __builtin_amdgcn_readfirstlane(tid >> 6);
  const int wm = wave >> 1, wn = wave & 1;
  const int tn = lid % tiles_n, tm = lid / tiles_n;
  const int m0 = tm * X3_BM, n0 = tn * X3_BN;
  const int nkz = (cin + 31) / 32, nkg = (cout + 31) / 32, rgm = (M + 15) / 16;
  const long z_ps = (long)rgm * nkz * 512, g_ps = (long)rgm * nkg * 512;
  const int nsteps_all = (M + 31) / 32;
  const int s_beg = slice * steps_per_slice, nsteps = min(steps_per_slice, nsteps_all - s_beg);
  const __amdgpu_buffer_rsrc_t rs_a = __builtin_amdgcn_make_buffer_rsrc((void*)Zp, 0, (int)(3 * z_ps * 2), 0x00020000);
  const __amdgpu_buffer_rsrc_t rs_b = __builtin_amdgcn_make_buffer_rsrc((void*)Gp, 0, (int)(3 * g_ps * 2), 0x00020000);
  int soff[X3_PER];
#pragma unroll
  for (int i = 0; i < X3_PER; ++i) {
    const int c = wave + 4 * i;
    const int q = c < 18 ? c : c - 18;
    const int plane = q / 6, j = (q % 6) / 2, half = q % 2;
    soff[i] = c < 18 ? (int)((plane * z_ps + ((long)(2 * s_beg + half) * nkz + min(m0 / 32 + j, nkz - 1)) * 512) * 2)
                     : (int)((plane * g_ps + ((long)(2 * s_beg + half) * nkg + min(n0 / 32 + j, nkg - 1)) * 512) * 2);
  }
  const bool odd_tail = (rgm & 1) && s_beg + nsteps == nsteps_all;
  const int kst_a = nkz * 2048, kst_b = nkg * 2048;
#define X3_ISSUE(KS_, BUF_)                                                                                    \
  do {                                                                                                         \
    unsigned short* base_ = smem + ((BUF_) & 1) * X3_STEP;                                                     \
    const bool tail_ = odd_tail && (KS_) == nsteps - 1;                                                        \
    _Pragma("unroll") for (int i = 0; i < X3_PER; ++i) {                                                       \
      const int c = wave + 4 * i;                                                                              \
      const bool is_a = i < 4 ? true : (i > 4 ? false : (c < 18));                                             \
      const __amdgpu_buffer_rsrc_t rs_ = is_a ? rs_a : rs_b;                                                   \
      const int so_ = (tail_ && (c & 1)) ? 0x7ffffff0 : soff[i] + (KS_) * (is_a ? kst_a : kst_b);              \
      __builtin_amdgcn_raw_ptr_buffer_load_lds(rs_, (lds_ptr_t)(base_ + c * 512), 16, lane * 16, so_, 0, 0);   \
    }                                                                                                          \
  } while (0)
  f32x4v acc[3][3];
#pragma unroll
  for (int i = 0; i < 3; ++i)
#pragma unroll
    for (int j = 0; j < 3; ++j)
#pragma unroll
      for (int r = 0; r < 4; ++r) acc[i][j][r] = 0.f;
  const int p16 = lane & 15, kg = lane >> 4;
  constexpr int TA[6] = {2, 1, 0, 1, 0, 0}, TB[6] = {0, 1, 2, 0, 1, 0};
  const int tq = p16 >> 2, tp = p16 & 3;
  int zaddr[3][2], gaddr[3][2];
#pragma unroll
  for (int t = 0; t < 3; ++t)
#pragma unroll
    for (int h2 = 0; h2 < 2; ++h2) {
      const int r16 = 8 * (kg & 1) + 4 * h2 + tq;
      const int ctz = 3 * wm + t, ctg = 3 * wn + t;
      const int cz = 2 * (ctz & 1) + (tp >> 1), cg = 2 * (ctg & 1) + (tp >> 1);
      zaddr[t][h2] = ((ctz >> 1) * 2 + (kg >> 1)) * 512 + r16 * 32 + X3_SWZ(r16, cz) + (tp & 1) * 4;
      gaddr[t][h2] = 18 * 512 + ((ctg >> 1) * 2 + (kg >> 1)) * 512 + r16 * 32 + X3_SWZ(r16, cg) + (tp & 1) * 4;
    }
#define X3_TR(PTR_) __builtin_amdgcn_ds_read_tr16_b64_v4i16((lds_b64_t)(PTR_))
#define X3_READ_COLS(KS_, FA_, FB_)                                                                            \
  do {                                                                                                         \
    unsigned short* base_ = smem + ((KS_) & 1) * X3_STEP;                                                      \
    _Pragma("unroll") for (int p = 0; p < 3; ++p)                                                              \
    _Pragma("unroll") for (int t = 0; t < 3; ++t) {                                                            \
      const bf16x4 a0_ = X3_TR(base_ + p * 6 * 512 + zaddr[t][0]), a1_ = X3_TR(base_ + p * 6 * 512 + zaddr[t][1]);   \
      const bf16x4 b0_ = X3_TR(base_ + p * 6 * 512 + gaddr[t][0]), b1_ = X3_TR(base_ + p * 6 * 512 + gaddr[t][1]);   \
      FA_[t][p] = __builtin_shufflevector(a0_, a1_, 0, 1, 2, 3, 4, 5, 6, 7);                                   \
      FB_[t][p] = __builtin_shufflevector(b0_, b1_, 0, 1, 2, 3, 4, 5, 6, 7);                                   \
    }                                                                                                          \
  } while (0)
  X3_PIPELINE(nsteps, X3_READ_COLS, 2);
#undef X3_ISSUE
  X3_STORE_C(dst, cout, m0, n0, cin, cout);
}

#define X3_BSRC(S_) (Bp + ((S_) / 384) * plane_stride + ((long)min(n0 / 16 + ((S_) % 384) / 64, rg_b - 1) * nk + ks_) * 512 + ((S_) % 64) * 8)
#define X3_BDST(S_) (base_ + (3 + (S_) / 384) * X3_PLANE + ((S_) % 384) * 8)

__global__ __launch_bounds__(256, 2) void gemm_bf16x3_fwd_kernel(const float* __restrict__ A, int lda,
                                                                 const unsigned short* __restrict__ Bp,
                                                                 float* __restrict__ C, int ldc, int M, int N, int K,
                                                                 int tiles_n, float* __restrict__ colstats) {
  __shared__ __attribute__((aligned(16))) unsigned short smem[2 * X3_STEP];
  const int tid = threadIdx.x, lane = tid & 63;
  const int wave = __builtin_amdgcn_readfirstlane(tid >> 6);
  const int wm = wave >> 1, wn = wave & 1;
  const int lid = xcd_remap(blockIdx.x, gridDim.x);
  const int tn = lid % tiles_n, tm = lid / tiles_n;
  const int m0 = tm * X3_BM, n0 = tn * X3_BN;
  const int nk = (K + 31) / 32, rg_b = (N + 15) / 16;
  const long plane_stride = (long)rg_b * nk * 512;

  float4 ax0, ax1, ax2, ay0, ay1, ay2;
  uint4 bx0, bx1, bx2, bx3, bx4, by0, by1, by2, by3, by4;
  const int ar0 = min(m0 + tid / 8, M - 1), ar1 = min(m0 + (tid + 256) / 8, M - 1), ar2 = min(m0 + (tid + 512) / 8, M - 1);
  const int akq = (tid % 8) * 4;
  const float4 zero4 = make_float4(0.f, 0.f, 0.f, 0.f);
  const int s4 = tid < 128 ? tid + 1024 : tid;
#define X3_FETCH(KS_, S_)                                                                                      \
  do {                                                                                                         \
    const int ks_ = (KS_);                                                                                     \
    const int kk_ = min(ks_ * 32 + akq, K - 4);     \
    a##S_##0 = *reinterpret_cast<const float4*>(A + (long)ar0 * lda + kk_);                                    \
    a##S_##1 = *reinterpret_cast<const float4*>(A + (long)ar1 * lda + kk_);                                    \
    a##S_##2 = *reinterpret_cast<const float4*>(A + (long)ar2 * lda + kk_);                                    \
    b##S_##0 = *reinterpret_cast<const uint4*>(X3_BSRC(tid));                                                  \
    b##S_##1 = *reinterpret_cast<const uint4*>(X3_BSRC(tid + 256));                                            \
    b##S_##2 = *reinterpret_cast<const uint4*>(X3_BSRC(tid + 512));                                            \
    b##S_##3 = *reinterpret_cast<const uint4*>(X3_BSRC(tid + 768));                                            \
    b##S_##4 = *reinterpret_cast<const uint4*>(X3_BSRC(s4));                                                   \
  } while (0)
#define X3_SPLIT_STORE(AV_, S_)                                                                                \
  do {                                                                                                         \
    unsigned h0_, m0_, l0_, h1_, m1_, l1_;                                                                     \
    const float4 v_ = kok_ ? (AV_) : zero4;                                                                    \
    x3_split_pk(v_.x, v_.y, h0_, m0_, l0_);                                                                    \
    x3_split_pk(v_.z, v_.w, h1_, m1_, l1_);                                                                    \
    const int o_ = ((S_) / 8) * X3_LDR + X3_SWZ((S_) / 8, akq / 8) + (akq & 4);                                \
    *reinterpret_cast<uint2*>(base_ + 0 * X3_PLANE + o_) = make_uint2(h0_, h1_);                               \
    *reinterpret_cast<uint2*>(base_ + 1 * X3_PLANE + o_) = make_uint2(m0_, m1_);                               \
    *reinterpret_cast<uint2*>(base_ + 2 * X3_PLANE + o_) = make_uint2(l0_, l1_);                               \
  } while (0)
#define X3_STAGE(KS_, S_, ALLK_)                                                                               \
  do {                                                                                                         \
    unsigned short* base_ = smem + ((KS_) & 1) * X3_STEP;                                                      \
    const bool kok_ = (ALLK_) || (KS_) * 32 + akq < K;         \
    X3_SPLIT_STORE(a##S_##0, tid);                                                                             \
    X3_SPLIT_STORE(a##S_##1, tid + 256);                                                                       \
    X3_SPLIT_STORE(a##S_##2, tid + 512);                                                                       \
    *reinterpret_cast<uint4*>(X3_BDST(tid)) = b##S_##0;                                                        \
    *reinterpret_cast<uint4*>(X3_BDST(tid + 256)) = b##S_##1;                                                  \
    *reinterpret_cast<uint4*>(X3_BDST(tid + 512)) = b##S_##2;                                                  \
    *reinterpret_cast<uint4*>(X3_BDST(tid + 768)) = b##S_##3;                                                  \
    *reinterpret_cast<uint4*>(X3_BDST(s4)) = b##S_##4;      \
  } while (0)

  f32x4v acc[3][3];
#pragma unroll
  for (int i = 0; i < 3; ++i)
#pragma unroll
    for (int j = 0; j < 3; ++j)
#pragma unroll
      for (int r = 0; r < 4; ++r) acc[i][j][r] = 0.f;

  X3_FETCH(0, x);
  X3_STAGE(0, x, false);
  const int p16 = lane & 15, kg = lane >> 4;
  constexpr int TA[6] = {2, 1, 0, 1, 0, 0}, TB[6] = {0, 1, 2, 0, 1, 0};
#define X3_FBODY(KS_, S_, STEADY_)                                                                             \
    if ((STEADY_) || (KS_) + 1 < nk) {                                                                         \
      X3_STAGE((KS_) + 1, S_, STEADY_);                                                                        \
      X3_MFMA(af, bfr);                                                                                        \
      _Pragma("unroll") for (int g = 0; g < 54; ++g) {                                                         \
        __builtin_amdgcn_sched_group_barrier(0x008, 1, 0);                                                     \
        __builtin_amdgcn_sched_group_barrier(0x002, 2, 0);                                                     \
        if (g % 3 == 0) __builtin_amdgcn_sched_group_barrier(0x200, 1, 0);                                     \
      }                                                                                                        \
      if ((STEADY_) || (KS_) + 3 < nk) X3_FETCH((KS_) + 3, S_);                                                \
    } else {                                                                                                   \
      X3_MFMA(af, bfr);                                                                                        \
    }
#define X3_ITER(KS_, S_, STEADY_)                                                                              \
  do {                                                                                                         \
    const unsigned short* base = smem + ((KS_) & 1) * X3_STEP;                                                 \
    bf16x8 af[3][3], bfr[3][3];                                                             \
    _Pragma("unroll") for (int t = 0; t < 3; ++t)                                                              \
    _Pragma("unroll") for (int p = 0; p < 3; ++p) {                                                            \
      af[t][p] = *reinterpret_cast<const bf16x8*>(base + p * X3_PLANE + (wm * 48 + t * 16 + p16) * X3_LDR + X3_SWZ(p16, kg));        \
      bfr[t][p] = *reinterpret_cast<const bf16x8*>(base + (3 + p) * X3_PLANE + (wn * 48 + t * 16 + p16) * X3_LDR + X3_SWZ(p16, kg)); \
    }                                                                                                          \
    X3_FBODY(KS_, S_, STEADY_);                                                                                \
    __syncthreads();                                                                                           \
  } while (0)
  int ks = 0;
  if (nk > 4) {
    X3_FETCH(1, x);
    X3_FETCH(2, y);
    __syncthreads();
    for (; ks + 4 < nk; ks += 2) {
      X3_ITER(ks, x, true);
      X3_ITER(ks + 1, y, true);
    }
  } else {
    if (nk > 1) X3_FETCH(1, x);
    if (nk > 2) X3_FETCH(2, y);
    __syncthreads();
  }
  for (; ks < nk; ks += 2) {
    X3_ITER(ks, x, false);
    if (ks + 1 < nk) X3_ITER(ks + 1, y, false);
  }
  X3_STORE_C(C, ldc, m0, n0, M, N);
  if (colstats) X3_COLSTATS();
}

extern "C" long spnet_bf16x3_kp(int K) { return (long)(K + 31) / 32 * 32; }
extern "C" long spnet_bf16x3_plane_elems(long R, int K) { return x3t_plane_elems(R, K); }

extern "C" int spnet_split_bf16x3_batched(const void* jobs, int njobs, long max_elems, void* stream) {
  if (!jobs || njobs < 1 || max_elems < 1) return (int)hipErrorInvalidValue;
  long gx = (max_elems / 512 + 3) / 4;
  if (gx > 2048) gx = 2048;
  if (gx < 1) gx = 1;
  hipLaunchKernelGGL(split_bf16x3_tiled_kernel, dim3((unsigned)gx, njobs), dim3(256), 0, (hipStream_t)stream,
                     reinterpret_cast<const long long*>(jobs));
  SPNET_RETURN_LAUNCH_STATUS();
}

static int x3_split_one(const float* W, void* planes, int K, long N, long sn, long sk, void* stream) {
  if (!W || !planes || K < 1 || N < 1 || (((uintptr_t)planes) & 15)) return (int)hipErrorInvalidValue;
  long gx = (x3t_plane_elems(N, K) / 512 + 3) / 4;
  if (gx > 2048) gx = 2048;
  hipLaunchKernelGGL(split_bf16x3_one_kernel, dim3((unsigned)gx), dim3(256), 0, (hipStream_t)stream, W,
                     reinterpret_cast<unsigned short*>(planes), K, N, sn, sk);
  SPNET_RETURN_LAUNCH_STATUS();
}
extern "C" int spnet_split_bf16x3(const float* W, void* planes, int K, int N, void* stream) {
  return x3_split_one(W, planes, K, N, 1, N, stream);
}
extern "C" int spnet_split_rows_bf16x3(const float* A, long lda, void* planes, long R, int K, void* stream) {
  return x3_split_one(A, planes, K, R, lda, 1, stream);
}

static bool x3_planes_ok(const void* p, long R, int K) {
  return p && !(((uintptr_t)p) & 15) && 3 * x3t_plane_elems(R, K) * 2 < (1L << 31);
}

static int x3_launch(const float* A, int lda, const void* planes, float* C, int ldc, int M, int N, int K, float* colstats,
                     int* stat_rows, void* stream) {
  if (!A || !C || M < 1 || N < 1 || K < 4 || (lda & 3) || (K & 3)) return (int)hipErrorInvalidValue;
  if ((((uintptr_t)A) & 15) || !x3_planes_ok(planes, N, K)) return (int)hipErrorInvalidValue;
  const int tm = spnet_cdiv(M, X3_BM), tn = spnet_cdiv(N, X3_BN);
  if (stat_rows) *stat_rows = tm;
  hipLaunchKernelGGL(gemm_bf16x3_fwd_kernel, dim3(tm * tn), dim3(256), 0, (hipStream_t)stream, A, lda,
                     reinterpret_cast<const unsigned short*>(planes), C, ldc, M, N, K, tn, colstats);
  SPNET_RETURN_LAUNCH_STATUS();
}

extern "C" int spnet_gemm_bf16x3_fwd(const float* A, int lda, const void* planes, float* C, int ldc, int M, int N, int K,
                                     void* stream) {
  return x3_launch(A, lda, planes, C, ldc, M, N, K, nullptr, nullptr, stream);
}

extern "C" int spnet_gemm_bf16x3_fwd_colstats(const float* A, int lda, const void* planes, float* C, int ldc, int M, int N,
                                              int K, float* colstats, int* stat_rows, void* stream) {
  if (!colstats || !stat_rows) return (int)hipErrorInvalidValue;
  return x3_launch(A, lda, planes, C, ldc, M, N, K, colstats, stat_rows, stream);
}

extern "C" int spnet_gemm_bf16x3_pp(const void* a_planes, const void* b_planes, float* C, int ldc, int M, int N, int K,
                                    float* colstats, int* stat_rows, void* stream) {
  if (!C || M < 1 || N < 1 || K < 1 || ldc < N || (colstats && !stat_rows)) return (int)hipErrorInvalidValue;
  if (!x3_planes_ok(a_planes, M, K) || !x3_planes_ok(b_planes, N, K)) return (int)hipErrorInvalidValue;
  const int tm = spnet_cdiv(M, X3_BM), tn = spnet_cdiv(N, X3_BN);
  if (stat_rows) *stat_rows = tm;
  hipLaunchKernelGGL(gemm_bf16x3_pp_kernel, dim3(tm * tn), dim3(256), 0, (hipStream_t)stream,
                     reinterpret_cast<const unsigned short*>(a_planes), x3t_plane_elems(M, K),
                     reinterpret_cast<const unsigned short*>(b_planes), x3t_plane_elems(N, K), C, ldc, M, N, (K + 31) / 32, tn,
                     colstats);
  SPNET_RETURN_LAUNCH_STATUS();
}

extern "C" long spnet_gemm_bf16x3_dwbwd_rows(long M) { return (M + FB_BM - 1) / FB_BM; }
extern "C" long spnet_gemm_bf16x3_dwbwd_ok(int H, int W, int cin) {
  return (((H == 12 && W == 16) || (H == 6 && W == 8)) && !(cin & 3)) ? 1 : 0;
}
extern "C" int spnet_gemm_bf16x3_pp_dwbwd(const void* dy_planes, const void* w_planes, int B, int H, int W, int cin, int cout,
                                          const float* x_fwd, const float* w, float* dx, int relu_in, const float* add,
                                          float* partial, const float* in_scale, const float* in_shift, const float* bn_mean,
                                          const float* bn_invstd, float* bn_partial, const float* bn_x, void* stream) {
  const long M = (long)B * H * W;
  if (!x_fwd || !w || !dx || !partial || B < 1 || !spnet_gemm_bf16x3_dwbwd_ok(H, W, cin)) return (int)hipErrorInvalidValue;
  if (bn_partial && (!bn_mean || !bn_invstd)) return (int)hipErrorInvalidValue;
  if (!x3_planes_ok(dy_planes, M, cout) || !x3_planes_ok(w_planes, cin, cout)) return (int)hipErrorInvalidValue;
  if ((((uintptr_t)x_fwd) | ((uintptr_t)dx) | ((uintptr_t)add) | ((uintptr_t)bn_x) | ((uintptr_t)w)) & 15) return (int)hipErrorInvalidValue;
  const int tm = spnet_cdiv(M, FB_BM), tn = spnet_cdiv(cin, X3_BN);
#define FB_LAUNCH(ADD_, BNX_)                                                                                  \
  hipLaunchKernelGGL((gemm_bf16x3_pp_dwbwd_kernel<0, ADD_, BNX_>), dim3(tm * tn), dim3(512), 0, (hipStream_t)stream,                \
                     reinterpret_cast<const unsigned short*>(dy_planes), x3t_plane_elems(M, cout),                              \
                     reinterpret_cast<const unsigned short*>(w_planes), x3t_plane_elems(cin, cout), (int)M, cin, (cout + 31) / 32, tn, \
                     H, W, x_fwd, w, dx, relu_in, add, partial, in_scale, in_shift, bn_mean, bn_invstd, bn_partial, bn_x,        \
                     (unsigned short*)nullptr, 0L)
  if (add && bn_x) FB_LAUNCH(true, true);
  else if (add) FB_LAUNCH(true, false);
  else if (bn_x) FB_LAUNCH(false, true);
  else FB_LAUNCH(false, false);
#undef FB_LAUNCH
  SPNET_RETURN_LAUNCH_STATUS();
}

extern "C" int spnet_gemm_bf16x3_pp_dwfwd(const void* z_planes, const void* w_planes, int B, int H, int W, int cin, int cout,
                                          const float* scale_shift, int relu_next, const float* w_next, void* out_planes,
                                          void* stream) {
  const long M = (long)B * H * W;
  if (!w_next || B < 1 || !spnet_gemm_bf16x3_dwbwd_ok(H, W, cout)) return (int)hipErrorInvalidValue;
  if (!x3_planes_ok(z_planes, M, cin) || !x3_planes_ok(w_planes, cout, cin) || !x3_planes_ok(out_planes, M, cout))
    return (int)hipErrorInvalidValue;
  if ((((uintptr_t)w_next) | ((uintptr_t)scale_shift)) & 15) return (int)hipErrorInvalidValue;
  const int tm = spnet_cdiv(M, FB_BM), tn = spnet_cdiv(cout, X3_BN);
  hipLaunchKernelGGL((gemm_bf16x3_pp_dwbwd_kernel<1, false, false>), dim3(tm * tn), dim3(512), 0, (hipStream_t)stream,
                     reinterpret_cast<const unsigned short*>(z_planes), x3t_plane_elems(M, cin),
                     reinterpret_cast<const unsigned short*>(w_planes), x3t_plane_elems(cout, cin), (int)M, cout, (cin + 31) / 32, tn,
                     H, W, (const float*)nullptr, w_next, (float*)nullptr, relu_next, (const float*)nullptr, (float*)nullptr,
                     scale_shift, scale_shift ? scale_shift + cout : nullptr, (const float*)nullptr, (const float*)nullptr,
                     (float*)nullptr, (const float*)nullptr, reinterpret_cast<unsigned short*>(out_planes), x3t_plane_elems(M, cout));
  SPNET_RETURN_LAUNCH_STATUS();
}

extern "C" long spnet_gemm_bf16x3_wgrad_ksplit(int cin, int cout, int M, int nbatch) {
  const long tiles = (long)spnet_cdiv(cin, X3_BM) * spnet_cdiv(cout, X3_BN) * (nbatch < 1 ? 1 : nbatch);
  const int steps = (M + 31) / 32;
  long s = (512 + tiles - 1) / tiles;
  if (s > steps / 24) s = steps / 24;
  if (s < 1) s = 1;
  const int per = (int)((steps + s - 1) / s);
  return (steps + per - 1) / per;
}

extern "C" int spnet_gemm_bf16x3_wgrad_batched(const void* jobs, int nbatch, int cin, int cout, int M, int ksplit,
                                               void* stream) {
  if (!jobs || nbatch < 1 || cin < 1 || cout < 1 || M < 1 || ksplit < 1) return (int)hipErrorInvalidValue;
  if (3 * x3t_plane_elems(M, cin) * 2 >= (1L << 31) || 3 * x3t_plane_elems(M, cout) * 2 >= (1L << 31))
    return (int)hipErrorInvalidValue;
  const int steps = (M + 31) / 32;
  if (ksplit > steps) return (int)hipErrorInvalidValue;
  const int per = (steps + ksplit - 1) / ksplit;
  if ((long)per * (ksplit - 1) >= steps) return (int)hipErrorInvalidValue;
  const int tm = spnet_cdiv(cin, X3_BM), tn = spnet_cdiv(cout, X3_BN);
  if ((long)tm * tn * nbatch * ksplit >= (1L << 31)) return (int)hipErrorInvalidValue;
  hipLaunchKernelGGL(gemm_bf16x3_wgrad_kernel, dim3(tm * tn * nbatch * ksplit), dim3(256), 0, (hipStream_t)stream,
                     reinterpret_cast<const long long*>(jobs), cin, cout, M, tn, tm * tn, nbatch, per);
  SPNET_RETURN_LAUNCH_STATUS();
}
```

### spnet_amd/engine.py

```python
import math
import os
from collections import OrderedDict

import numpy as np
import torch

from . import _lib as L

BN_EPS = 1e-3
BN_MOMENTUM = 0.99
L2_COEF = 1e-4
ACT_NONE, ACT_RELU, ACT_LRELU, ACT_RELU6 = 0, 1, 2, 3
BACKBONES = ("Xception", "MobileNet", "InceptionResNetV2", "DenseNet121")
MOBILENET_BLOCKS = [(64, 1), (128, 2), (128, 1), (256, 2), (256, 1), (512, 2), (512, 1), (512, 1), (512, 1), (512, 1),
                    (512, 1), (1024, 2), (1024, 1)]
K_MAJOR, OUT_MAJOR = 0, 1
WS_FLOATS = 48 * 1024 * 1024
WS_GEMM = (0, 16 * 1024 * 1024)
WS_DW = (16 * 1024 * 1024, 16 * 1024 * 1024)
WS_BNP = (32 * 1024 * 1024, 8 * 1024 * 1024)
WS_MISC = (40 * 1024 * 1024, 8 * 1024 * 1024)
WS_GEMM2 = (48 * 1024 * 1024, 16 * 1024 * 1024)
WS_BNP2 = (64 * 1024 * 1024, 4 * 1024 * 1024)
WS_TOTAL = 68 * 1024 * 1024
ALIGN = 64


def _capture(fn):
    import gc
    torch.cuda.synchronize()
    gc.collect()
    was_enabled = gc.isenabled()
    gc.disable()
    try:
        g = torch.cuda.CUDAGraph()
        with torch.cuda.graph(g):
            fn()
    finally:
        if was_enabled:
            gc.enable()
    return g


_stream = L.current_stream


class KernelTimer:

    def __init__(self):
        self.records = []
        self.tags = {}
        self.keys = {}

    def start(self):
        e = torch.cuda.Event(enable_timing=True)
        e.record()
        return e

    def stop(self, family, start, work, tag=None):
        e = torch.cuda.Event(enable_timing=True)
        e.record()
        self.records.append((family, start, e, work))
        if tag is not None:
            self.tags[len(self.records) - 1] = tag

    def tagged(self):
        out = {}
        for i, tag in self.tags.items():
            fam, s, e, w = self.records[i]
            n, ms, tw = out.get(tag, (0, 0.0, 0.0))
            out[tag] = (n + 1, ms + s.elapsed_time(e), tw + w)
        return out

    def totals(self):
        out = {}
        for fam, s, e, w in self.records:
            n, ms, tw = out.get(fam, (0, 0.0, 0.0))
            out[fam] = (n + 1, ms + s.elapsed_time(e), tw + w)
        return out


def xception_plan():
    blocks = [("entry",)]
    blocks.append(("strided", 2, 64, 128, 128, False, "conv2d_4", "batch_normalization_4"))
    blocks.append(("strided", 3, 128, 256, 256, True, "conv2d_5", "batch_normalization_5"))
    blocks.append(("strided", 4, 256, 728, 728, True, "conv2d_6", "batch_normalization_6"))
    for b in range(5, 13):
        blocks.append(("middle", b, 728))
    blocks.append(("strided", 13, 728, 728, 1024, True, "conv2d_7", "batch_normalization_7"))
    blocks.append(("exit", 14, 1024, 1536, 2048))
    return blocks


def backbone_out_hw(H, W):
    h, w = H // 2, W // 2
    h, w = (h - 3) // 2 + 1, (w - 3) // 2 + 1
    h, w = h - 2, w - 2
    for _ in range(4):
        h, w = (h + 1) // 2, (w + 1) // 2
    return h, w


def irv2_program():
    ops, ctr = [], [3]

    def conv(src, dst, cin, cout, k, stride=1, same=True, relu=True, name=None, bias=False):
        kk = (k, k) if isinstance(k, int) else tuple(k)
        if name is None:
            ctr[0] += 1
            cname, bname = "conv2d_%d" % ctr[0], "batch_normalization_%d" % ctr[0]
        else:
            cname, bname = name, name + "_bn"
        ops.append(("conv", cname, None if bias else bname, src, dst, cin, cout, kk, stride, same, relu, bias))

    conv("in", "x", 3, 32, 3, 2, False)
    conv("x", "x", 32, 32, 3, 1, False)
    conv("x", "x", 32, 64, 3)
    ops.append(("maxpool", "x", "x"))
    conv("x", "x", 64, 80, 1, 1, False)
    conv("x", "x", 80, 192, 3, 1, False)
    ops.append(("maxpool", "x", "x"))
    conv("x", "b0", 192, 96, 1)
    conv("x", "b1", 192, 48, 1)
    conv("b1", "b1", 48, 64, 5)
    conv("x", "b2", 192, 64, 1)
    conv("b2", "b2", 64, 96, 3)
    conv("b2", "b2", 96, 96, 3)
    ops.append(("avgpool", "x", "bp"))
    conv("bp", "bp", 192, 64, 1)
    ops.append(("concat", ["b0", "b1", "b2", "bp"], "x", "mixed_5b"))

    def block(kind, idx, c, scale, relu=True):
        if kind == "block35":
            conv("x", "b0", c, 32, 1)
            conv("x", "b1", c, 32, 1)
            conv("b1", "b1", 32, 32, 3)
            conv("x", "b2", c, 32, 1)
            conv("b2", "b2", 32, 48, 3)
            conv("b2", "b2", 48, 64, 3)
            br, cm = ["b0", "b1", "b2"], 128
        elif kind == "block17":
            conv("x", "b0", c, 192, 1)
            conv("x", "b1", c, 128, 1)
            conv("b1", "b1", 128, 160, (1, 7))
            conv("b1", "b1", 160, 192, (7, 1))
            br, cm = ["b0", "b1"], 384
        else:
            conv("x", "b0", c, 192, 1)
            conv("x", "b1", c, 192, 1)
            conv("b1", "b1", 192, 224, (1, 3))
            conv("b1", "b1", 224, 256, (3, 1))
            br, cm = ["b0", "b1"], 448
        name = "%s_%d" % (kind, idx)
        ops.append(("concat", br, "m", name + "_mixed"))
        conv("m", "up", cm, c, 1, relu=False, name=name + "_conv", bias=True)
        ops.append(("resadd", "x", "up", "x", scale, relu))

    for i in range(1, 11):
        block("block35", i, 320, 0.17)
    conv("x", "b0", 320, 384, 3, 2, False)
    conv("x", "b1", 320, 256, 1)
    conv("b1", "b1", 256, 256, 3)
    conv("b1", "b1", 256, 384, 3, 2, False)
# ... 230 lines not shown
    for i in range(len(owners) - 1, -1, -1):
        key, mid = owners[i]
        if first[key] >= cur_hi:
            continue
        edge = i > 0 and owners[i - 1][1] != mid
        if (cur_hi - first[key]) >= per or edge:
            buckets.append((first[key], cur_hi, first_middle if mid else key))
            cur_hi = first[key]
    tail = [(hhi, cur_hi)] if cur_hi > hhi else []
    if hlo > 0:
        tail.insert(0, (0, hlo))
    return buckets, tail


def _glorot_fans(name, shape):
    if name.endswith("depthwise_kernel"):
        return shape[2] * 9, 9
    if len(shape) == 4:
        rf = shape[0] * shape[1]
        return shape[2] * rf, shape[3] * rf
    return shape[0], shape[1]


class WeightSet:

    def __init__(self, H, W, n_out=576, backbone="Xception", device="cuda:0", seed=0, rank=0):
        lay = param_layout(H, W, n_out, backbone)
        self.p_off, self.s_off, self.l2_n, self.rest_lo = lay["p_off"], lay["s_off"], lay["l2_n"], lay["rest_lo"]
        self.n_theta, self.spec_order = lay["n_theta"], lay["spec_order"]
        self.dev = torch.device(device)
        self.theta = torch.zeros(self.n_theta, device=self.dev, dtype=torch.float32)
        self.stats = torch.zeros(lay["n_stats"], device=self.dev, dtype=torch.float32)
        self.grad = self.m = self.v = None
        self.t = 0
        self.drop_seed = 12345 + 7919 * int(rank)
        self.theta_ver = self.stats_ver = 0
        self.wT = {}
        self.planes = {}
        self._wT_jobs = self._wT_at = self._planes_jobs = self._planes_at = None
        self.init_weights(seed)

    def alloc_train_state(self):
        if self.grad is None:
            self.grad, self.m, self.v = (torch.zeros(self.n_theta, device=self.dev, dtype=torch.float32) for _ in range(3))

    def init_weights(self, seed=0):
        self.theta_ver += 1
        self.stats_ver += 1
        g = torch.Generator().manual_seed(seed)
        host = torch.zeros(self.n_theta, dtype=torch.float32)
        for name, (off, n, shape) in self.p_off.items():
            if name.endswith("/gamma"):
                host[off:off + n] = 1.0
            elif name.endswith("kernel"):
                fi, fo = _glorot_fans(name, shape)
                lim = math.sqrt(6.0 / (fi + fo))
                host[off:off + n] = ((torch.rand(n, generator=g, dtype=torch.float64) * 2 - 1) * lim).float()
        self.theta.copy_(host)
        hs = torch.zeros(self.stats.numel(), dtype=torch.float32)
        for name, (off, n, _) in self.s_off.items():
            if name.endswith("moving_variance"):
                hs[off:off + n] = 1.0
        self.stats.copy_(hs)
        if self.m is not None:
            self.m.zero_()
            self.v.zero_()
        self.t = 0

    def state_dict(self):
        out = OrderedDict()
        for name in self.spec_order:
            if name in self.p_off:
                off, n, shape = self.p_off[name]
                out[name] = self.theta[off:off + n].reshape(shape).cpu().clone()
            else:
                off, n, shape = self.s_off[name]
                out[name] = self.stats[off:off + n].reshape(shape).cpu().clone()
        return out

    def load_state_dict(self, sd):
        self.theta_ver += 1
        self.stats_ver += 1
        for name in self.spec_order:
            t = torch.as_tensor(np.asarray(sd[name]), dtype=torch.float32).reshape(-1)
            if name in self.p_off:
                off, n, _ = self.p_off[name]
                dst = self.theta
            else:
                off, n, _ = self.s_off[name]
                dst = self.stats
            if t.numel() != n:
                raise ValueError("shape mismatch for %s: got %d values, need %d" % (name, t.numel(), n))
            dst[off:off + n].copy_(t.to(self.dev))

    def grad_dict(self):
        return OrderedDict((name, self.grad[off:off + n].reshape(shape).cpu().clone())
                           for name, (off, n, shape) in self.p_off.items())

    def transposed(self, wname):
        if wname not in self.wT:
            self.wT[wname] = torch.empty(self.p_off[wname][1], device=self.dev, dtype=torch.float32)
            self._wT_jobs = self._wT_at = None
        return self.wT[wname]

    def refresh_transposes(self):
        if self._wT_at == self.theta_ver:
            return
        if self.wT:
            if self._wT_jobs is None:
                flat, mr, mc = [], 1, 1
                for name, dst in self.wT.items():
                    off, n, shape = self.p_off[name]
                    R, C = int(shape[-2]), int(shape[-1])
                    flat += [self.theta.data_ptr() + 4 * off, dst.data_ptr(), R, C]
                    mr, mc = max(mr, R), max(mc, C)
                self._wT_jobs = (torch.tensor(flat, dtype=torch.int64, device=self.dev), len(self.wT), mr, mc)
            table, nj, mr, mc = self._wT_jobs
            L.spnet_transpose_batched(table.data_ptr(), nj, mr, mc, _stream())
        self._wT_at = self.theta_ver

    def need_planes(self, wname, fwd, dgrad):
        ent = self.planes.setdefault(wname, [None, None])
        cin, cout = (int(v) for v in self.p_off[wname][2][-2:])
        for i, (want, R, K) in enumerate(((fwd, cout, cin), (dgrad, cin, cout))):
            if want and ent[i] is None:
                ent[i] = torch.zeros(3 * int(L.spnet_bf16x3_plane_elems(R, K)), dtype=torch.int16, device=self.dev)
                self._planes_jobs = self._planes_at = None

    def refresh_planes(self):
        if self._planes_at == self.theta_ver:
            return
        if self.planes:
            if self._planes_jobs is None:
                flat, mx = [], 1
                for wname, (pf, pd) in self.planes.items():
                    off, n, shape = self.p_off[wname]
                    cin, cout = int(shape[-2]), int(shape[-1])
                    w = self.theta.data_ptr() + 4 * off
                    if pf is not None:
                        flat += [w, pf.data_ptr(), cin, cout, 1, cout]
                        mx = max(mx, pf.numel() // 3)
                    if pd is not None:
                        flat += [w, pd.data_ptr(), cout, cin, cout, 1]
                        mx = max(mx, pd.numel() // 3)
                self._planes_jobs = (torch.tensor(flat, dtype=torch.int64, device=self.dev), len(flat) // 6, mx)
            table, nj, mx = self._planes_jobs
            L.spnet_split_bf16x3_batched(table.data_ptr(), nj, mx, _stream())
        self._planes_at = self.theta_ver


class Engine:
    def __init__(self, H, W, batch, n_out=576, device="cuda:0", loss_type="same", seed=0,
                 train=True, adam_eps=1e-7, share_from=None, rank=0, sigmoid_cols=None, backbone="Xception",
                 pointwise="bf16x3", x3_min_tiles=192, fuse_dw_bwd=True, early_head=True):
        if pointwise not in ("bf16x3", "f32"):
            raise ValueError("pointwise must be 'bf16x3' or 'f32'")
        self._pointwise = pointwise
        self.fuse_dw_bwd = bool(fuse_dw_bwd)
        self.fuse_dw_fwd = bool(fuse_dw_bwd)
        self.early_head = bool(early_head)
        self.x3_min_tiles = int(x3_min_tiles)
        self.fuse_min_tiles = 256 if self.x3_min_tiles else 0
        if not torch.cuda.is_available():
            raise RuntimeError("spnet_amd.Engine needs a HIP device (no CPU fallback)")
        self.H, self.W, self.B, self.n_out = int(H), int(W), int(batch), int(n_out)
        self.sigmoid_cols = sigmoid_cols
        if backbone not in BACKBONES:
            raise NotImplementedError("backbone %r: this build implements %s" % (backbone, ", ".join(BACKBONES)))
        self.backbone = backbone
        self.dev = torch.device(device)
        self.loss_type = loss_type
        self.train_capable = bool(train)
        self.adam_eps = adam_eps
        self.prof = None
        self._pw_layers = []
        self._bns = []
        self._irv2 = None
        self._densenet = None
        self.deferred_wgrads = []
        self.dw_reduce_jobs = []
        self._dw_reduce_table = None
        self._wgrad_table = None
        self._first_middle = None
        self.overlap_wgrad = os.environ.get("SPNET_OVERLAP_WGRAD", "1") != "0"
        torch.cuda.set_device(self.dev)
        self._igraph = None
        self._coeffs_at = None
        if share_from is not None:
            self.weights = w = share_from.weights
        else:
            self.weights = w = WeightSet(self.H, self.W, self.n_out, backbone, device, seed, rank)
        if self.train_capable:
            w.alloc_train_state()
        self.p_off, self.s_off, self.l2_n, self.rest_lo = w.p_off, w.s_off, w.l2_n, w.rest_lo
        self.n_theta, self.theta, self.stats = w.n_theta, w.theta, w.stats
        self.update_mask = None
        self._build_graph()
        for pw in self._pw_layers:
            if pw.x3_fwd or pw.x3_dgrad:
                w.need_planes(pw.wname, pw.x3_fwd, pw.x3_dgrad)

    @property
    def pointwise(self):
        return self._pointwise

    def new_planes(self, R, K):
        return torch.zeros(3 * int(L.spnet_bf16x3_plane_elems(R, K)), dtype=torch.int16, device=self.dev)

    grad = property(lambda self: self.weights.grad)
    m = property(lambda self: self.weights.m)
    v = property(lambda self: self.weights.v)

    @property
    def t(self):
        return self.weights.t

    @t.setter
    def t(self, v):
        self.weights.t = int(v)

    @property
    def drop_seed(self):
        return self.weights.drop_seed

    @drop_seed.setter
    def drop_seed(self, v):
        self.weights.drop_seed = int(v) & 0xFFFFFFFF

    def init_weights(self, seed=0):
        self.weights.init_weights(seed)

    def state_dict(self):
        return self.weights.state_dict()

    def load_state_dict(self, sd):
        self.weights.load_state_dict(sd)

    def grad_dict(self):
        return self.weights.grad_dict()

    def P(self, name):
        off, n, shape = self.p_off[name]
        return self.theta[off:off + n]

    def G(self, name):
        off, n, shape = self.p_off[name]
        return self.grad[off:off + n]

    def S(self, name):
        off, n, shape = self.s_off[name]
        return self.stats[off:off + n]

    def new(self, *shape):
        return torch.empty(shape, device=self.dev, dtype=torch.float32)

    def ws_ptr(self, region):
        return self.ws.data_ptr() + 4 * region[0]

    def _build_graph(self):
        B, H, W = self.B, self.H, self.W
        tr = self.train_capable
        self.ws = self.new(WS_TOTAL)
        self.wgrad_stream = torch.cuda.Stream(device=self.dev) if (tr and self.overlap_wgrad) else None
        self.small = self.new(8 * 4096)
        self.nodes = []
        self.x_in = self.new(B, H, W, 1)

        H2, W2 = H // 2, W // 2
        n = self.nodes
        sh = StemHead(self, self.x_in, "conv2d_1"); n.append(sh)
        a1 = BatchNorm(self, sh.y, 3, "batch_normalization_1", ACT_LRELU); n.append(a1)
        c2 = SmallConv(self, a1.y, 3, 3, 1, True, "conv2d_2"); n.append(c2)
        a2 = BatchNorm(self, c2.y, 3, "batch_normalization_2", ACT_LRELU); n.append(a2)
        c3 = SmallConv(self, a2.y, 3, 3, 1, True, "conv2d_3"); n.append(c3)
        s = BatchNorm(self, c3.y, 3, "batch_normalization_3", ACT_NONE, residual=sh.px, res_bcast=True); n.append(s)
        d = Dropout(self, s.y, 0.1); n.append(d)
        self.stem_out = d.y
        if self.backbone == "MobileNet":
            return self._build_mobilenet(d.y)
        if self.backbone == "InceptionResNetV2":
            net = IRv2Backbone(self, d.y); n.append(net)
            self._irv2 = net
            self.backbone_out = net.y
            return self._build_head(net.y)
        if self.backbone == "DenseNet121":
            from .densenet import DenseNetBackbone
            net = DenseNetBackbone(self, d.y); n.append(net)
            self.backbone_out = net.y
            return self._build_head(net.y)
        e1 = SmallConv(self, d.y, 3, 32, 2, False, "block1_conv1"); n.append(e1)
        b1 = BatchNorm(self, e1.y, 32, "block1_conv1_bn", ACT_RELU); n.append(b1)
        e2 = Conv3x3Gemm(self, b1.y, 32, 64, "block1_conv2"); n.append(e2)
        b2 = BatchNorm(self, e2.y, 64, "block1_conv2_bn", ACT_RELU); n.append(b2)
        x = b2.y
        prev_middle = None
        for blk in xception_plan():
            if blk[0] == "strided":
                _, b, cin, c1_, c2_, first_relu, cn, bnn = blk
                node = StridedBlock(self, x, b, cin, c1_, c2_, first_relu, cn, bnn)
            elif blk[0] == "middle":
                node = MiddleBlock(self, x, blk[1], blk[2], prev=prev_middle)
                prev_middle = node
                if self._first_middle is None:
                    self._first_middle = node
            elif blk[0] == "exit":
                node = ExitBlock(self, x, blk[2], blk[3], blk[4])
            else:
                continue
            n.append(node)
            prev_middle = node if blk[0] == "middle" else None
            x = node.y
        self.backbone_out = x
        self._build_head(x)
# ... 401 lines not shown

    def fwd(self, training):
        L.spnet_stem_head(0, L.ptr(self.x), L.ptr(self.w), L.ptr(self.y), L.ptr(self.px), self.e.B, self.H, self.W,
                          None, 0, _stream())

    def bwd(self, g):
        e = self.e
        side = e.wgrad_stream
        region = WS_MISC if side is None else WS_GEMM2

        def call():
            L.spnet_stem_head(2, L.ptr(self.x), L.ptr(g), L.ptr(self.gw), None, e.B, self.H, self.W, e.ws_ptr(region),
                              region[1], _stream())
        if side is None:
            call()
        else:
            side.wait_stream(torch.cuda.current_stream())
            with torch.cuda.stream(side):
                call()
        return None


class AvgPool(Node):
    def __init__(self, eng, x, C, need_dx=True):
        self.e, self.x, self.C = eng, x, C
        B, H, W, _ = x.shape
        self.H, self.W = H, W
        self.y = eng.new(B, H // 2, W // 2, C)
        self.need_dx = need_dx
        self.dx = eng.new(*x.shape) if (eng.train_capable and need_dx) else None

    def fwd(self, training):
        L.spnet_avgpool2_fwd(L.ptr(self.x), L.ptr(self.y), self.e.B, self.H, self.W, self.C, _stream())

    def bwd(self, g):
        if not self.need_dx:
            return g
        L.spnet_avgpool2_bwd(L.ptr(g), L.ptr(self.dx), self.e.B, self.H, self.W, self.C, _stream())
        return self.dx


class BatchNorm(Node):

    def __init__(self, eng, x, C, name, act, residual=None, res_bcast=False, bwd_inplace=True):
        self.e, self.x, self.C, self.act = eng, x, C, act
        self.M = x.numel() // C
        self.pnames = [name]
        self.gamma, self.beta = eng.P(name + "/gamma"), eng.P(name + "/beta")
        self.mm, self.mv = eng.S(name + "/moving_mean"), eng.S(name + "/moving_variance")
        self.residual, self.res_bcast = residual, res_bcast
        self.y = eng.new(*x.shape)
        if eng.train_capable:
            self.ggamma, self.gbeta = eng.G(name + "/gamma"), eng.G(name + "/beta")
            self.save = eng.new(2 * C)
            self.dx = None if bwd_inplace else eng.new(*x.shape)

    def fwd(self, training):
        e, C = self.e, self.C
        ss = e.small[:2 * C]
        if training:
            L.spnet_bn_fwd_train(L.ptr(self.x), self.M, C, L.ptr(self.gamma), L.ptr(self.beta), L.ptr(self.mm),
                                 L.ptr(self.mv), L.ptr(self.save), self.save[C:].data_ptr(), L.ptr(ss), self.act,
                                 L.ptr(self.residual), int(self.res_bcast), L.ptr(self.y), BN_EPS, BN_MOMENTUM,
                                 e.ws_ptr(WS_MISC), _stream())
        else:
            L.spnet_bn_fwd_infer(L.ptr(self.x), self.M, C, L.ptr(self.gamma), L.ptr(self.beta), L.ptr(self.mm),
                                 L.ptr(self.mv), L.ptr(ss), self.act, L.ptr(self.residual), int(self.res_bcast),
                                 L.ptr(self.y), BN_EPS, _stream())

    def bwd(self, g):
        e, C = self.e, self.C
        co = e.small[:3 * C]
        out = g if self.dx is None else self.dx
        L.spnet_bn_bwd(L.ptr(self.x), L.ptr(g), self.M, C, L.ptr(self.gamma), L.ptr(self.beta), L.ptr(self.save),
                       self.save[C:].data_ptr(), self.act, L.ptr(out), L.ptr(self.ggamma), L.ptr(self.gbeta),
                       L.ptr(co), e.ws_ptr(WS_MISC), _stream())
        return out


class Dropout(Node):
    def __init__(self, eng, x, rate):
        self.e, self.x, self.rate = eng, x, rate
        self.y = eng.new(*x.shape) if eng.train_capable else x
        self.seed = 0

    def fwd(self, training):
        if training:
            L.spnet_dropout(L.ptr(self.x), L.ptr(self.y), self.x.numel(), 0, self.rate, self.e.seed_ptr, _stream())
        elif self.y is not self.x:
            self.y.copy_(self.x)

    def bwd(self, g):
        L.spnet_dropout(L.ptr(g), L.ptr(g), g.numel(), 0, self.rate, self.e.seed_ptr, _stream())
        return g


class Pointwise:

    def __init__(self, eng, M, cin, cout, wname, defer_wgrad=False, allow_blend=True):
        self.e, self.M, self.cin, self.cout = eng, M, cin, cout
        self.w = eng.P(wname)
        self.wname = wname
        self.gw = eng.G(wname) if eng.train_capable else None
        x3 = eng.pointwise == "bf16x3" and cin % 4 == 0 and cout % 4 == 0
        tiles = lambda n: ((M + 95) // 96) * ((n + 95) // 96)
        self.x3_fwd = x3 and cout >= 256 and tiles(cout) >= eng.x3_min_tiles
        self.x3_dgrad = x3 and cin >= 256 and tiles(cin) >= eng.x3_min_tiles and eng.train_capable
        eng._pw_layers.append(self)
        self.blend = bool(allow_blend and eng.train_capable and cin <= 128)
        self.wT = eng.weights.transposed(wname) if self.blend else None
        self.defer_wgrad = defer_wgrad

    def planes(self, form):
        return self.e.weights.planes[self.wname][form]

    def _x3(self, tag, A, lda, planes, C, ldc, N, K, colstats_region=None):
        e = self.e
        prof = e.prof
        t0 = prof.start() if prof is not None else None
        rows = 0
        if colstats_region is None:
            L.spnet_gemm_bf16x3_fwd(L.ptr(A), lda, L.ptr(planes), L.ptr(C), ldc, self.M, N, K, _stream())
        else:
            if (self.M + 95) // 96 * 2 * N > colstats_region[1]:
                raise RuntimeError("BatchNorm partial region too small for M=%d N=%d" % (self.M, N))
            L.spnet_gemm_bf16x3_fwd_colstats(L.ptr(A), lda, L.ptr(planes), L.ptr(C), ldc, self.M, N, K,
                                             e.ws_ptr(colstats_region), __import__("ctypes").addressof(_stat_rows), _stream())
            rows = _stat_rows.value
        if prof is not None:
            prof.stop("gemm", t0, 2.0 * self.M * N * K, (tag, self.M, N, K))
        return rows

    def _x3p(self, tag, a_planes, b_planes, C, N, K, colstats_region=None):
        e = self.e
        prof = e.prof
        t0 = prof.start() if prof is not None else None
        rows = 0
        if colstats_region is None:
            L.spnet_gemm_bf16x3_pp(L.ptr(a_planes), L.ptr(b_planes), L.ptr(C), N, self.M, N, K, None, None, _stream())
        else:
            if (self.M + 95) // 96 * 2 * N > colstats_region[1]:
                raise RuntimeError("BatchNorm partial region too small for M=%d N=%d" % (self.M, N))
            L.spnet_gemm_bf16x3_pp(L.ptr(a_planes), L.ptr(b_planes), L.ptr(C), N, self.M, N, K, e.ws_ptr(colstats_region),
                                   __import__("ctypes").addressof(_stat_rows), _stream())
            rows = _stat_rows.value
        if prof is not None:
            prof.stop("gemm", t0, 2.0 * self.M * N * K, (tag, self.M, N, K))
        return rows

    def fwd_p(self, zp, y, colstats_region=None):
        tag = "x3p aB" if colstats_region is None else "x3p aB+stats"
        return self._x3p(tag, zp, self.planes(0), y, self.cout, self.cin, colstats_region)

    def bwd_p(self, zp, dyp, dx):
        e = self.e
        if self.defer_wgrad:
            e.deferred_wgrads.append(("x3", zp, dyp, self.gw, self.cin, self.cout, self.M))
        else:
            e._flush_x3_wgrads([("x3", zp, dyp, self.gw, self.cin, self.cout, self.M)])
        if dx is not None:
            self._x3p("x3p ab", dyp, self.planes(1), dx, self.cin, self.cout)

    def fwd(self, x, y):
        if self.x3_fwd and self.e.pointwise == "bf16x3":
            self._x3("x3 aB", x, self.cin, self.planes(0), y, self.cout, self.cout, self.cin)
            return
        _gemm(x, K_MAJOR, self.cin, self.w, OUT_MAJOR, self.cout, y, self.cout, self.M, self.cout, self.cin, self.e)

    def fwd_colstats(self, x, y, region=WS_BNP):
        if self.x3_fwd and self.e.pointwise == "bf16x3":
            return self._x3("x3 aB+stats", x, self.cin, self.planes(0), y, self.cout, self.cout, self.cin,
                            colstats_region=region)
        return _gemm_colstats(x, self.cin, self.w, self.cout, y, self.cout, self.M, self.cout, self.cin, self.e,
                              region=region)

    def bwd(self, x, dy, dx):
        e = self.e
        side = e.wgrad_stream
        if self.defer_wgrad:
            e.deferred_wgrads.append((x, dy, self.gw, self.cin, self.cout, self.M))
        elif side is None:
            _gemm(x, OUT_MAJOR, self.cin, dy, OUT_MAJOR, self.cout, self.gw, self.cout, self.cin, self.cout, self.M, e)
        else:
            side.wait_stream(torch.cuda.current_stream())
            with torch.cuda.stream(side):
                _gemm(x, OUT_MAJOR, self.cin, dy, OUT_MAJOR, self.cout, self.gw, self.cout, self.cin, self.cout,
                      self.M, e, region=WS_GEMM2)
        if dx is not None and self.x3_dgrad and e.pointwise == "bf16x3":
            self._x3("x3 ab", dy, self.cout, self.planes(1), dx, self.cin, self.cin, self.cout)
        elif dx is not None:
            _gemm(dy, K_MAJOR, self.cout, self.w, K_MAJOR, self.cout, dx, self.cin, self.M, self.cin, self.cout, e)


    def bwd_blend(self, x, g, yp, bn, dyb, dx):
        e = self.e
        prof = e.prof
        t0 = prof.start() if prof is not None else None
        L.spnet_gemm_f32_bnblend(L.ptr(g), L.ptr(yp), L.ptr(bn.coef), bn.cld, self.cout, L.ptr(self.wT), self.cin,
                                 L.ptr(dx), self.cin, self.M, self.cin, self.cout, 0, L.ptr(dyb), _stream())
        if prof is not None:
            prof.stop("gemm", t0, 2.0 * self.M * self.cin * self.cout, ("aB blend", self.M, self.cin, self.cout))
        side = e.wgrad_stream
        if self.defer_wgrad:
            e.deferred_wgrads.append((x, dyb, self.gw, self.cin, self.cout, self.M))
        elif side is None:
            _gemm(x, OUT_MAJOR, self.cin, dyb, OUT_MAJOR, self.cout, self.gw, self.cout, self.cin, self.cout, self.M, e)
        else:
            side.wait_stream(torch.cuda.current_stream())
            with torch.cuda.stream(side):
                _gemm(x, OUT_MAJOR, self.cin, dyb, OUT_MAJOR, self.cout, self.gw, self.cout, self.cin, self.cout,
                      self.M, e, region=WS_GEMM2)


class Conv3x3Gemm(Node):

    def __init__(self, eng, x, cin, cout, name):
        self.e, self.x, self.cin, self.cout = eng, x, cin, cout
        B, H, W, _ = x.shape
        self.H, self.W = H, W
        self.OH, self.OW = H - 2, W - 2
        self.y = eng.new(B, self.OH, self.OW, cout)
        self.w = eng.P(name + "/kernel")
        self.pnames = [name]
        if eng.train_capable:
            self.gw = eng.G(name + "/kernel")
            self.dx = eng.new(*x.shape)
            if L.spnet_conv3x3_wgrad_ws(B, H, W, cin, cout) > min(WS_GEMM[1], WS_GEMM2[1]):
                raise RuntimeError("split-K workspace too small for %s" % name)

    def _timed(self, flops, call):
        prof = self.e.prof
        if prof is None:
            return call()
        t0 = prof.start()
        call()
        prof.stop("gemm", t0, flops, ("conv3x3 implicit", int(flops / (2.0 * 9 * self.cin * self.cout)), self.cout, 9 * self.cin))

    def fwd(self, training):
        e = self.e
        self._timed(2.0 * e.B * self.OH * self.OW * 9 * self.cin * self.cout,
                    lambda: L.spnet_conv3x3_fwd(L.ptr(self.x), L.ptr(self.w), L.ptr(self.y), e.B, self.H, self.W,
                                                self.cin, self.cout, _stream()))

    def _wgrad(self, g, region):
        e = self.e
        self._timed(2.0 * e.B * self.OH * self.OW * 9 * self.cin * self.cout,
                    lambda: L.spnet_conv3x3_wgrad(L.ptr(self.x), L.ptr(g), L.ptr(self.gw), e.B, self.H, self.W,
                                                  self.cin, self.cout, e.ws_ptr(region), region[1], _stream()))

    def bwd(self, g):
        e = self.e
        side = e.wgrad_stream
        if side is None:
            self._wgrad(g, WS_GEMM)
        else:
            side.wait_stream(torch.cuda.current_stream())
            with torch.cuda.stream(side):
                self._wgrad(g, WS_GEMM2)
        self._timed(2.0 * e.B * self.H * self.W * 9 * self.cout * self.cin,
                    lambda: L.spnet_conv3x3_dgrad(L.ptr(g), L.ptr(self.w), L.ptr(self.dx), e.B, self.H, self.W,
                                                  self.cin, self.cout, _stream()))
        return self.dx


class BN:

    def __init__(self, eng, C, M, name, eps=BN_EPS):
        self.e, self.C, self.M, self.eps = eng, C, M, eps
        self.gamma, self.beta = eng.P(name + "/gamma"), eng.P(name + "/beta")
        self.mm, self.mv = eng.S(name + "/moving_mean"), eng.S(name + "/moving_variance")
        self.ss = eng.new(2 * C)
        eng._bns.append(self)
        if eng.train_capable:
            self.ggamma, self.gbeta = eng.G(name + "/gamma"), eng.G(name + "/beta")
            self.save = eng.new(2 * C)
            self.cld = (C + 63) // 64 * 64
            self.coef = torch.zeros(3 * self.cld, device=eng.dev, dtype=torch.float32)

    def coeffs_from_partials(self, rows):
        e = self.e
        L.spnet_bn_bwd_coeffs_from_partials(rows, e.ws_ptr(WS_BNP), self.M, self.C, L.ptr(self.gamma), self.mean_ptr,
                                            self.invstd_ptr, L.ptr(self.ggamma), L.ptr(self.gbeta), L.ptr(self.coef),
                                            self.cld, _stream())

    def coeffs_full(self, x, g):
        e = self.e
        L.spnet_bn_bwd_coeffs(L.ptr(x), L.ptr(g), self.M, self.C, L.ptr(self.gamma), L.ptr(self.beta), self.mean_ptr,
                              self.invstd_ptr, L.ptr(self.ggamma), L.ptr(self.gbeta), L.ptr(self.coef), self.cld,
                              e.ws_ptr(WS_MISC), _stream())

    @property
    def scale_ptr(self):
        return self.ss.data_ptr()

    @property
    def shift_ptr(self):
        return self.ss.data_ptr() + 4 * self.C

    @property
    def mean_ptr(self):
        return self.save.data_ptr()

    @property
    def invstd_ptr(self):
        return self.save.data_ptr() + 4 * self.C

    def finalize(self, rows, region=WS_BNP):
        e = self.e
        L.spnet_bn_finalize_fwd(e.ws_ptr(region), rows, self.M, self.C, L.ptr(self.gamma), L.ptr(self.beta),
                                L.ptr(self.mm), L.ptr(self.mv), self.mean_ptr, self.invstd_ptr, L.ptr(self.ss),
                                self.eps, BN_MOMENTUM, _stream())

    def infer(self):
        L.spnet_bn_infer_coeffs(self.C, L.ptr(self.gamma), L.ptr(self.beta), L.ptr(self.mm), L.ptr(self.mv),
                                L.ptr(self.ss), self.eps, _stream())

    def apply(self, x, y, act, residual=None):
        L.spnet_bn_apply(L.ptr(x), self.M, self.C, L.ptr(self.ss), act, L.ptr(residual), 0, L.ptr(y), _stream())

    def bwd_full(self, x, g, out, act):
        e, C = self.e, self.C
        L.spnet_bn_bwd(L.ptr(x), L.ptr(g), self.M, C, L.ptr(self.gamma), L.ptr(self.beta), self.mean_ptr,
                       self.invstd_ptr, act, L.ptr(out), L.ptr(self.ggamma), L.ptr(self.gbeta), L.ptr(e.small[:3 * C]),
                       e.ws_ptr(WS_MISC), _stream())
        return out

    def bwd_from_partials(self, x, g, out, rows):
        e, C = self.e, self.C
        L.spnet_bn_bwd_from_partials(L.ptr(x), L.ptr(g), self.M, C, L.ptr(self.gamma), L.ptr(self.beta),
                                     self.mean_ptr, self.invstd_ptr, rows, e.ws_ptr(WS_BNP), L.ptr(out),
                                     L.ptr(self.ggamma), L.ptr(self.gbeta), L.ptr(e.small[:3 * C]), _stream())
        return out


    def bwd_full_x3(self, x, g, out_planes, act):
        e, C = self.e, self.C
        L.spnet_bn_bwd_x3(L.ptr(x), L.ptr(g), self.M, C, L.ptr(self.gamma), L.ptr(self.beta), self.mean_ptr,
                          self.invstd_ptr, act, L.ptr(out_planes), L.ptr(self.ggamma), L.ptr(self.gbeta),
                          L.ptr(e.small[:3 * C]), e.ws_ptr(WS_MISC), _stream())
        return out_planes

    def bwd_from_partials_x3(self, x, g, out_planes, rows):
        e, C = self.e, self.C
        L.spnet_bn_bwd_from_partials_x3(L.ptr(x), L.ptr(g), self.M, C, L.ptr(self.gamma), L.ptr(self.beta),
                                        self.mean_ptr, self.invstd_ptr, rows, e.ws_ptr(WS_BNP), L.ptr(out_planes),
                                        L.ptr(self.ggamma), L.ptr(self.gbeta), L.ptr(e.small[:3 * C]), _stream())
        return out_planes


class Ref:

    def __init__(self, t, bn=None, stats_bn=None, stats_x=None):
        self.t, self.bn = t, bn
        self.stats_bn, self.stats_x = stats_bn, stats_x


def _dw_fwd(x, w, y, B, H, W, C, relu_in, scale_ptr, shift_ptr):
    if L.spnet_dwconv3x3_prefers_stream(B, H, W, C, 0):
        L.spnet_dwconv3x3_stream_fwd(L.ptr(x), L.ptr(w), L.ptr(y), B, H, W, C, relu_in, scale_ptr, shift_ptr, 0, _stream())
    else:
        L.spnet_dwconv3x3_tiled_fwd(L.ptr(x), L.ptr(w), L.ptr(y), B, H, W, C, relu_in, scale_ptr, shift_ptr, _stream())


def _dw_fwd_x3(x, w, zp, B, H, W, C, relu_in, scale_ptr, shift_ptr):
    if L.spnet_dwconv3x3_prefers_stream(B, H, W, C, 0):
        L.spnet_dwconv3x3_stream_fwd_x3(L.ptr(x), L.ptr(w), L.ptr(zp), B, H, W, C, relu_in, scale_ptr, shift_ptr, 0, _stream())
    else:
        L.spnet_dwconv3x3_tiled_fwd_x3(L.ptr(x), L.ptr(w), L.ptr(zp), B, H, W, C, relu_in, scale_ptr, shift_ptr, _stream())


class _DwBwdPlan:

    def __init__(self, B, H, W, C):
        self.B, self.H, self.W, self.C = B, H, W, C
        self.stream = bool(L.spnet_dwconv3x3_prefers_stream(B, H, W, C, 1))
        if self.stream:
            self.rows = int(L.spnet_dwconv3x3_stream_rows(B, H, W, C, 0))
            self.ws_floats = int(L.spnet_dwconv3x3_stream_bwd_ws(B, H, W, C, 0))
        else:
            self.rows = int(L.spnet_dwconv3x3_tiled_rows(B, H, W, C))
            self.ws_floats = int(L.spnet_dwconv3x3_tiled_bwd_ws(B, H, W, C))

    def run(self, dz, x, w, dx, relu_in, add, wpart, scale_ptr, shift_ptr, mean_ptr, invstd_ptr, bn_partial_ptr, bn_x):
        a = (L.ptr(dz), L.ptr(x), L.ptr(w), L.ptr(dx), None, self.B, self.H, self.W, self.C, relu_in, L.ptr(add),
             L.ptr(wpart), scale_ptr, shift_ptr, mean_ptr, invstd_ptr, bn_partial_ptr, L.ptr(bn_x))
        if self.stream:
            L.spnet_dwconv3x3_stream_bwd(*a, 0, _stream())
        else:
            L.spnet_dwconv3x3_tiled_bwd(*a, _stream())


class SepConvBN:

    def __init__(self, eng, src, cin, cout, name, relu_in, mode="lazy", act=ACT_NONE, residual=None,
                 bwd_inplace=True, defer_wgrad=False):
        self.e, self.src, self.cin, self.cout, self.relu_in = eng, src, cin, cout, int(relu_in)
        self.mode, self.act, self.residual, self.bwd_inplace = mode, act, residual, bwd_inplace
        B, H, W, _ = src.t.shape
        self.H, self.W = H, W
        self.M = B * H * W
        self.wd = eng.P(name + "/depthwise_kernel")
        self.yp = eng.new(B, H, W, cout)
        self.pw = Pointwise(eng, self.M, cin, cout, name + "/pointwise_kernel", defer_wgrad=defer_wgrad)
        self.x3p = eng.pointwise == "bf16x3" and self.pw.x3_fwd and (self.pw.x3_dgrad or not eng.train_capable)
        self.z = None if self.x3p else eng.new(B, H, W, cin)
        self.zp = eng.new_planes(self.M, cin) if self.x3p else None
        self.bn = BN(eng, cout, self.M, name + "_bn")
        self.y = eng.new(B, H, W, cout) if mode == "apply" else None
        self.dwb = _DwBwdPlan(B, H, W, cin)
        self.fuse_bwd = bool(self.x3p and eng.train_capable and eng.fuse_dw_bwd and L.spnet_gemm_bf16x3_dwbwd_ok(H, W, cin)
                             and ((self.M + 191) // 192) * ((cin + 95) // 96) >= eng.fuse_min_tiles)
        if self.fuse_bwd:
            self.dwb.rows = int(L.spnet_gemm_bf16x3_dwbwd_rows(self.M))
            self.dwb.ws_floats = self.dwb.rows * 9 * cin
        self.rows_src = self.dwb.rows
        if self.rows_src * 2 * cin > WS_BNP[1]:
            raise RuntimeError("workspace regions too small for %s" % name)
        self.consumer_rows = 0
        self.consumer_unit = None
        self._dw_done = False
        self.fin_by_consumer = False
        self.pending_rows = 0
        if eng.train_capable:
            self.gwd = eng.G(name + "/depthwise_kernel")
            self.dz = None if self.fuse_bwd else eng.new(B, H, W, cin)
            self.dx = eng.new(B, H, W, cin)
            self.wpart = eng.new(self.dwb.ws_floats)
            eng.dw_reduce_jobs.append((self.wpart, self.gwd, self.rows_src, 9 * cin))
            self.blend = (act == ACT_NONE or mode != "apply") and self.pw.blend
            self.dyb = eng.new(B, H, W, cout) if self.blend else None
            self.dbn = None if (bwd_inplace or self.blend or self.x3p) else eng.new(B, H, W, cout)
            self.dyp = eng.new_planes(self.M, cout) if self.x3p else None
        if src.bn is not None and hasattr(src, "owner"):
            src.owner.consumer_rows = self.rows_src
            src.owner.consumer_unit = self
            src.owner.fin_by_consumer = eng.train_capable

    def ref(self):
        if self.mode == "apply":
            return Ref(self.y)
        r = Ref(self.yp, self.bn)
        r.owner = self
        return r

    def fwd(self, training):
        e, sb = self.e, self.src.bn
        prof = e.prof
        if prof is not None:
            t0 = prof.start()
        owner = getattr(self.src, "owner", None)
        ran_dw = True
        if self._dw_done and not training:
            self._dw_done = ran_dw = False
        elif training and owner is not None and owner.pending_rows:
            bnfin = L.spnet_dwconv3x3_tiled_fwd_bnfin_x3 if self.x3p else L.spnet_dwconv3x3_tiled_fwd_bnfin
            bnfin(L.ptr(self.src.t), L.ptr(self.wd), L.ptr(self.zp if self.x3p else self.z), e.B, self.H, self.W,
                  self.cin, self.relu_in, e.ws_ptr(WS_BNP), owner.pending_rows, sb.M,
                  L.ptr(sb.gamma), L.ptr(sb.beta), L.ptr(sb.mm), L.ptr(sb.mv), sb.mean_ptr,
                  sb.invstd_ptr, L.ptr(sb.ss), BN_EPS, BN_MOMENTUM, _stream())
            owner.pending_rows = 0
        else:
            (_dw_fwd_x3 if self.x3p else _dw_fwd)(self.src.t, self.wd, self.zp if self.x3p else self.z, e.B, self.H, self.W,
                                                  self.cin, self.relu_in, sb.scale_ptr if sb else None,
                                                  sb.shift_ptr if sb else None)
        if prof is not None and ran_dw:
            prof.stop("dw", t0, 2.0 * 4 * self.M * self.cin, ("dw fwd", self.H, self.W, self.cin))
        if training:
            rows = self.pw.fwd_p(self.zp, self.yp, WS_BNP) if self.x3p else self.pw.fwd_colstats(self.z, self.yp)
            if self.fin_by_consumer and rows <= 128:
                self.pending_rows = rows
            elif self.mode == "apply":
                bn = self.bn
                L.spnet_bn_finalize_apply(e.ws_ptr(WS_BNP), rows, L.ptr(self.yp), self.M, self.cout, L.ptr(bn.gamma),
                                          L.ptr(bn.beta), L.ptr(bn.mm), L.ptr(bn.mv), bn.mean_ptr, bn.invstd_ptr,
                                          L.ptr(bn.ss), self.act, L.ptr(self.residual), L.ptr(self.y), BN_EPS,
                                          BN_MOMENTUM, _stream())
                return
            else:
                self.bn.finalize(rows)
        else:
            nxt = self.consumer_unit
            if (self.x3p and self.mode == "lazy" and nxt is not None and nxt.x3p and e.fuse_dw_fwd
                    and L.spnet_gemm_bf16x3_dwbwd_ok(self.H, self.W, self.cout)
                    and ((self.M + 191) // 192) * ((self.cout + 95) // 96) >= e.fuse_min_tiles):
                t0 = prof.start() if prof is not None else None
                L.spnet_gemm_bf16x3_pp_dwfwd(L.ptr(self.zp), L.ptr(self.pw.planes(0)), e.B, self.H, self.W, self.cin,
                                             self.cout, L.ptr(self.bn.ss), nxt.relu_in, L.ptr(nxt.wd), L.ptr(nxt.zp), _stream())
                if prof is not None:
                    prof.stop("gemm", t0, 2.0 * self.M * self.cin * self.cout, ("x3p aB+dwfwd", self.M, self.cout, self.cin))
                nxt._dw_done = True
                return
            if self.x3p:
                self.pw.fwd_p(self.zp, self.yp)
            else:
                self.pw.fwd(self.z, self.yp)
        if self.mode == "apply":
            self.bn.apply(self.yp, self.y, self.act, self.residual)

    def bwd(self, g, add=None):
        e, sb = self.e, self.src.bn
        from_partials = self.mode == "lazy" or (self.consumer_rows and self.act == ACT_NONE)
        if self.blend:
            if from_partials:
                self.bn.coeffs_from_partials(self.consumer_rows)
            else:
                self.bn.coeffs_full(self.yp, g)
            self.pw.bwd_blend(self.z, g, self.yp, self.bn, self.dyb, self.dz)
        elif self.x3p:
            if from_partials:
                self.bn.bwd_from_partials_x3(self.yp, g, self.dyp, self.consumer_rows)
            else:
                self.bn.bwd_full_x3(self.yp, g, self.dyp, self.act if self.mode == "apply" else ACT_NONE)
            self.pw.bwd_p(self.zp, self.dyp, self.dz)
            if self.fuse_bwd:
                st = self.src.stats_bn if self.src.stats_bn is not None else sb
                prof = e.prof
                t0 = prof.start() if prof is not None else None
                L.spnet_gemm_bf16x3_pp_dwbwd(L.ptr(self.dyp), L.ptr(self.pw.planes(1)), e.B, self.H, self.W, self.cin,
                                             self.cout, L.ptr(self.src.t), L.ptr(self.wd), L.ptr(self.dx), self.relu_in,
                                             L.ptr(add), L.ptr(self.wpart), sb.scale_ptr if sb else None,
                                             sb.shift_ptr if sb else None, st.mean_ptr if st else None,
                                             st.invstd_ptr if st else None, e.ws_ptr(WS_BNP) if st else None,
                                             L.ptr(self.src.stats_x), _stream())
                if prof is not None:
                    prof.stop("gemm", t0, 2.0 * self.M * self.cin * self.cout, ("x3p ab+dwbwd", self.M, self.cin, self.cout))
                return self.dx
        else:
            out = g if self.bwd_inplace else self.dbn
            if from_partials:
                dy = self.bn.bwd_from_partials(self.yp, g, out, self.consumer_rows)
            else:
                dy = self.bn.bwd_full(self.yp, g, out, self.act if self.mode == "apply" else ACT_NONE)
            self.pw.bwd(self.z, dy, self.dz)
        st = self.src.stats_bn if self.src.stats_bn is not None else sb
        prof = e.prof
        if prof is not None:
            t0 = prof.start()
        self.dwb.run(self.dz, self.src.t, self.wd, self.dx, self.relu_in, add, self.wpart,
                     sb.scale_ptr if sb else None, sb.shift_ptr if sb else None,
                     st.mean_ptr if st else None, st.invstd_ptr if st else None,
                     e.ws_ptr(WS_BNP) if st else None, self.src.stats_x)
        if prof is not None:
            prof.stop("dw", t0, 3.0 * 4 * self.M * self.cin, ("dw bwd", self.H, self.W, self.cin))
        return self.dx


class MiddleBlock(Node):

    def __init__(self, eng, x, b, C, prev=None):
        self.x = x
        self.pnames = [n for k in (1, 2, 3) for n in ("block%d_sepconv%d" % (b, k), "block%d_sepconv%d_bn" % (b, k))]
        src = Ref(x)
        if prev is not None and eng.train_capable:
            src = Ref(x, stats_bn=prev.u3.bn, stats_x=prev.u3.yp)
        d = eng.train_capable
        self.u1 = SepConvBN(eng, src, C, C, "block%d_sepconv1" % b, True, mode="lazy", defer_wgrad=d)
        if src.stats_bn is not None:
            prev.u3.consumer_rows = self.u1.rows_src
        self.u2 = SepConvBN(eng, self.u1.ref(), C, C, "block%d_sepconv2" % b, True, mode="lazy", defer_wgrad=d)
        self.u3 = SepConvBN(eng, self.u2.ref(), C, C, "block%d_sepconv3" % b, True, mode="apply", residual=x,
                            bwd_inplace=False, defer_wgrad=d)
        self.y = self.u3.y

    def fwd(self, training):
        self.u1.fwd(training)
        self.u2.fwd(training)
        self.u3.fwd(training)

    def bwd(self, g):
        d = self.u3.bwd(g)
        d = self.u2.bwd(d)
        return self.u1.bwd(d, add=g)


class StridedBlock(Node):

    def __init__(self, eng, x, b, cin, c1, c2, first_relu, conv_name, bn_name):
        self.e, self.x, self.cin, self.c2 = eng, x, cin, c2
        self.pnames = [conv_name, bn_name] + [n for k in (1, 2) for n in ("block%d_sepconv%d" % (b, k),
                                                                           "block%d_sepconv%d_bn" % (b, k))]
        B, H, W, _ = x.shape
        self.H, self.W = H, W
        OH, OW = (H + 1) // 2, (W + 1) // 2
        self.OH, self.OW = OH, OW
        self.Ms = B * OH * OW
        self.xs = eng.new(B, OH, OW, cin)
        self.yr = eng.new(B, OH, OW, c2)
        self.pwr = Pointwise(eng, self.Ms, cin, c2, conv_name + "/kernel")
        self.bnr = BN(eng, c2, self.Ms, bn_name)
        self.u1 = SepConvBN(eng, Ref(x), cin, c1, "block%d_sepconv1" % b, first_relu, mode="lazy")
        self.u2 = SepConvBN(eng, self.u1.ref(), c1, c2, "block%d_sepconv2" % b, True, mode="pool")
        self.y = eng.new(B, OH, OW, c2)
        if eng.train_capable:
            self.idx = torch.empty(B * OH * OW * (c2 // 4), device=eng.dev, dtype=torch.int32)
            self.dxs = eng.new(B, OH, OW, cin)
            self.blend = self.pwr.blend
            self.dyr = eng.new(B, OH, OW, c2) if self.blend else None
            self.dpool = eng.new(B, H, W, c2)
            rows = L.spnet_maxpool3x3s2_bwd_rows(B, H, W, c2, 1024 if self.u2.blend else 128)
            self.pool_stats = rows * 2 * c2 <= WS_BNP[1]
            if self.pool_stats:
                self.u2.consumer_rows = self.pool_rows = rows
        else:
            self.idx = None

    def fwd(self, training):
        e = self.e
        side = e.wgrad_stream if training else None
        main = torch.cuda.current_stream()
        if side is not None:
            side.wait_stream(main)
            torch.cuda.set_stream(side)
        L.spnet_gather_s2(L.ptr(self.x), L.ptr(self.xs), e.B, self.H, self.W, self.cin, _stream())
        if training:
            region = WS_BNP2 if side is not None else WS_BNP
            self.bnr.finalize(self.pwr.fwd_colstats(self.xs, self.yr, region=region), region=region)
        else:
            self.pwr.fwd(self.xs, self.yr)
        if side is not None:
            torch.cuda.set_stream(main)
        self.u1.fwd(training)
        self.u2.fwd(training)
        if side is not None:
            main.wait_stream(side)
        L.spnet_maxpool3x3s2_add_fwd(L.ptr(self.u2.yp), L.ptr(self.yr), L.ptr(self.y),
                                     L.ptr(self.idx) if training else None, e.B, self.H, self.W, self.c2,
                                     L.ptr(self.u2.bn.ss), L.ptr(self.bnr.ss), _stream())

    def bwd(self, g):
        e = self.e
        if self.pool_stats:
            bn2 = self.u2.bn
            L.spnet_maxpool3x3s2_bwd_bnsums(L.ptr(g), L.ptr(self.idx), L.ptr(self.dpool), e.B, self.H, self.W, self.c2,
                                            L.ptr(self.u2.yp), bn2.mean_ptr, bn2.invstd_ptr, e.ws_ptr(WS_BNP),
                                            self.pool_rows, _stream())
        else:
            L.spnet_maxpool3x3s2_bwd(L.ptr(g), L.ptr(self.idx), L.ptr(self.dpool), e.B, self.H, self.W, self.c2, _stream())
        if self.blend:
            self.bnr.coeffs_full(self.yr, g)
            self.pwr.bwd_blend(self.xs, g, self.yr, self.bnr, self.dyr, self.dxs)
        else:
            gr = self.bnr.bwd_full(self.yr, g, g, ACT_NONE)
            self.pwr.bwd(self.xs, gr, self.dxs)
        d = self.u2.bwd(self.dpool)
        dx = self.u1.bwd(d)
        L.spnet_scatter_add_s2(L.ptr(self.dxs), L.ptr(dx), e.B, self.H, self.W, self.cin, _stream())
        return dx


class ExitBlock(Node):

    def __init__(self, eng, x, cin, c1, c2):
        self.pnames = ["block14_sepconv1", "block14_sepconv1_bn", "block14_sepconv2", "block14_sepconv2_bn"]
        self.u1 = SepConvBN(eng, Ref(x), cin, c1, "block14_sepconv1", False, mode="lazy")
        self.u2 = SepConvBN(eng, self.u1.ref(), c1, c2, "block14_sepconv2", True, mode="apply", act=ACT_RELU)
        self.y = self.u2.y

    def fwd(self, training):
        self.u1.fwd(training)
        self.u2.fwd(training)

    def bwd(self, g):
        return self.u1.bwd(self.u2.bwd(g))


class _T:

    def __init__(self, buf):
        self.buf, self.g = buf, None
        self.owner, self.consumers = None, 0


class IRv2Backbone(Node):

    def __init__(self, eng, x):
        self.e = eng
# ... 648 lines not shown
```

Baseline: 3236 images/sec.

## Finalize BatchNorm stats in last-arriving GEMM block instead of separate launch

Adds a 'last block arrives' pattern to the bf16x3 pointwise forward GEMM and the fused dwbwd GEMM. Each block writes per-tile column partials with agent-scope stores and bumps a per-column-tile atomic counter, and the last block combines the partials to produce BN mean/invstd/scale/shift and moving stats (forward) or dgamma/dbeta and backward coefficients (backward). The backward BN then runs a light apply-only kernel with the precomputed coefficients. This removes separate finalize/coefficient kernel launches and a pass over the partials. In exchange it adds atomics, a serialized tail in the last block, and counter state that must be reset correctly.

```diff
diff --git a/include/spnet_hip.h b/include/spnet_hip.h
--- a/include/spnet_hip.h
+++ b/include/spnet_hip.h
@@ -27,6 +27,16 @@
                                const float* x_fwd, const float* w, float* dx, int relu_in, const float* add, float* partial,
                                const float* in_scale, const float* in_shift, const float* bn_mean, const float* bn_invstd,
                                float* bn_partial, const float* bn_x, void* stream);
+int spnet_gemm_bf16x3_pp_bnlast(const void* a_planes, const void* b_planes, float* C, int ldc, int M, int N, int K,
+                                float* colstats, int* stat_rows, const float* gamma, const float* beta, float* moving_mean,
+                                float* moving_var, float* save_mean, float* save_invstd, float* scale_shift, float eps,
+                                float momentum, void* counters, void* stream);
+int spnet_gemm_bf16x3_pp_dwbwd_bnlast(const void* dy_planes, const void* w_planes, int B, int H, int W, int cin, int cout,
+                                      const float* x_fwd, const float* w, float* dx, int relu_in, const float* add,
+                                      float* partial, const float* in_scale, const float* in_shift, const float* bn_mean,
+                                      const float* bn_invstd, float* bn_partial, const float* bn_x, const float* bn_gamma,
+                                      float* bn_dgamma, float* bn_dbeta, float* bn_coef, int cld, void* counters,
+                                      void* stream);
 int spnet_gemm_bf16x3_wgrad_batched(const void* jobs, int nbatch, int cin, int cout, int M, int ksplit, void* stream);
 int spnet_gemm_f32_accumulate(const float* A, int a_major, int lda, const float* B, int b_major, int ldb, float* C,
                               int ldc, int M, int N, int K, int tile, void* stream);
@@ -137,6 +147,12 @@
                                   const float* beta, const float* save_mean, const float* save_invstd, int P,
                                   const float* partial, void* dx_planes, float* dgamma, float* dbeta, float* coeffs,
                                   void* stream);
+int spnet_bn_bwd_apply(const float* x, const float* dy, long M, int C, const float* gamma, const float* beta,
+                       const float* save_mean, const float* save_invstd, const float* coef, int cld, float* dx,
+                       void* stream);
+int spnet_bn_bwd_apply_x3(const float* x, const float* dy, long M, int C, const float* gamma, const float* beta,
+                          const float* save_mean, const float* save_invstd, const float* coef, int cld, void* dx_planes,
+                          void* stream);
 
 int spnet_bn_bwd_coeffs_from_partials(int P, const float* partial, long M, int C, const float* gamma,
                                       const float* save_mean, const float* save_invstd, float* dgamma, float* dbeta,
diff --git a/spnet_amd/_lib.py b/spnet_amd/_lib.py
--- a/spnet_amd/_lib.py
+++ b/spnet_amd/_lib.py
@@ -28,6 +28,9 @@
     "spnet_gemm_bf16x3_dwbwd_rows": (c_long, [c_long]),
     "spnet_gemm_bf16x3_dwbwd_ok": (c_long, [c_int, c_int, c_int]),
     "spnet_gemm_bf16x3_pp_dwbwd": (c_int, [P, P, c_int, c_int, c_int, c_int, c_int, P, P, P, c_int, P, P, P, P, P, P, P, P, P]),
+    "spnet_gemm_bf16x3_pp_bnlast": (c_int, [P, P, P, c_int, c_int, c_int, c_int, P, P, P, P, P, P, P, P, P, c_float, c_float, P, P]),
+    "spnet_gemm_bf16x3_pp_dwbwd_bnlast": (c_int, [P, P, c_int, c_int, c_int, c_int, c_int, P, P, P, c_int, P, P, P, P, P, P, P, P,
+                                                  P, P, P, P, c_int, P, P]),
     "spnet_gemm_bf16x3_pp_dwfwd": (c_int, [P, P, c_int, c_int, c_int, c_int, c_int, P, c_int, P, P, P]),
     "spnet_gemm_bf16x3_wgrad_batched": (c_int, [P, c_int, c_int, c_int, c_int, c_int, P]),
     "spnet_split_bf16x3_batched": (c_int, [P, c_int, c_long, P]),
@@ -69,6 +72,8 @@
     "spnet_bn_finalize_apply_ld": (c_int, [P, c_int, P, c_long, c_int, P, P, P, P, P, P, P, c_int, P, P, c_long, c_float, c_float, P]),
     "spnet_bn_bwd_from_partials": (c_int, [P, P, c_long, c_int, P, P, P, P, c_int, P, P, P, P, P, P]),
     "spnet_bn_bwd_from_partials_x3": (c_int, [P, P, c_long, c_int, P, P, P, P, c_int, P, P, P, P, P, P]),
+    "spnet_bn_bwd_apply": (c_int, [P, P, c_long, c_int, P, P, P, P, P, c_int, P, P]),
+    "spnet_bn_bwd_apply_x3": (c_int, [P, P, c_long, c_int, P, P, P, P, P, c_int, P, P]),
     "spnet_bn_bwd_x3": (c_int, [P, P, c_long, c_int, P, P, P, P, c_int, P, P, P, P, P, P]),
     "spnet_gemm_f32_colstats": (c_int, [P, c_int, c_int, P, c_int, c_int, P, c_int, c_int, c_int, c_int, c_int, P, P, P]),
     "spnet_gemm_f32_bnblend": (c_int, [P, P, P, c_int, c_int, P, c_int, P, c_int, c_int, c_int, c_int, c_int, P, P]),
diff --git a/spnet_amd/csrc/bn.hip b/spnet_amd/csrc/bn.hip
--- a/spnet_amd/csrc/bn.hip
+++ b/spnet_amd/csrc/bn.hip
@@ -844,6 +844,31 @@
                                    reinterpret_cast<unsigned short*>(dx_planes), dgamma, dbeta, coeffs, stream);
 }
 
+static int bn_bwd_apply_impl(const float* x, const float* dy, long M, int C, const float* gamma, const float* beta,
+                             const float* save_mean, const float* save_invstd, const float* coef, int cld, float* dx,
+                             unsigned short* planes, void* stream) {
+  if ((C & 3) || (cld & 3) || cld < C || !coef || M < 1) return (int)hipErrorInvalidValue;
+  if (planes && !bn_planes_ok(planes, M, C)) return (int)hipErrorInvalidValue;
+  const long n4 = M * (C / 4);
+  hipLaunchKernelGGL(bn_bwd_apply_vec_kernel, dim3(spnet_ew_grid(n4, 256)), dim3(256), 0, (hipStream_t)stream, x, dy, M, C,
+                     save_mean, save_invstd, gamma, beta, 0, coef, coef + cld, coef + 2 * cld, dx, planes,
+                     x3t_plane_elems(M, C));
+  SPNET_RETURN_LAUNCH_STATUS();
+}
+extern "C" int spnet_bn_bwd_apply(const float* x, const float* dy, long M, int C, const float* gamma, const float* beta,
+                                  const float* save_mean, const float* save_invstd, const float* coef, int cld, float* dx,
+                                  void* stream) {
+  if (!dx) return (int)hipErrorInvalidValue;
+  return bn_bwd_apply_impl(x, dy, M, C, gamma, beta, save_mean, save_invstd, coef, cld, dx, nullptr, stream);
+}
+extern "C" int spnet_bn_bwd_apply_x3(const float* x, const float* dy, long M, int C, const float* gamma, const float* beta,
+                                     const float* save_mean, const float* save_invstd, const float* coef, int cld,
+                                     void* dx_planes, void* stream) {
+  if (!dx_planes) return (int)hipErrorInvalidValue;
+  return bn_bwd_apply_impl(x, dy, M, C, gamma, beta, save_mean, save_invstd, coef, cld, nullptr,
+                           reinterpret_cast<unsigned short*>(dx_planes), stream);
+}
+
 extern "C" int spnet_bn_bwd_coeffs_from_partials(int P, const float* partial, long M, int C, const float* gamma,
                                                  const float* save_mean, const float* save_invstd, float* dgamma,
                                                  float* dbeta, float* coef, int cld, void* stream) {
diff --git a/spnet_amd/csrc/common.h b/spnet_amd/csrc/common.h
--- a/spnet_amd/csrc/common.h
+++ b/spnet_amd/csrc/common.h
@@ -63,6 +63,138 @@
   return r;
 }
 
+struct BnLastFwd {
+  const float* gamma;
+  const float* beta;
+  float* moving_mean;
+  float* moving_var;
+  float* save_mean;
+  float* save_invstd;
+  float* scale;
+  float* shift;
+  unsigned* counters;
+  long M;
+  float eps, momentum;
+};
+struct BnLastBwd {
+  const float* gamma;
+  const float* invstd;
+  float* dgamma;
+  float* dbeta;
+  float* k1;
+  float* k2;
+  float* k3;
+  unsigned* counters;
+  long M;
+};
+#define BN_LAST_MAX_BLOCKS 32
+
+__device__ __forceinline__ void bn_store_agent(float* p, float v) {
+  __hip_atomic_store(p, v, __ATOMIC_RELAXED, __HIP_MEMORY_SCOPE_AGENT);
+}
+__device__ __forceinline__ float bn_load_agent(const float* p) {
+  return __hip_atomic_load(p, __ATOMIC_RELAXED, __HIP_MEMORY_SCOPE_AGENT);
+}
+
+__device__ __forceinline__ bool bn_last_arriver(unsigned* counter, unsigned expected) {
+  __shared__ unsigned last_flag;
+  asm volatile("s_waitcnt vmcnt(0)" ::: "memory");
+  __syncthreads();
+  if (threadIdx.x == 0) {
+    const unsigned ticket = __hip_atomic_fetch_add(counter, 1u, __ATOMIC_RELAXED, __HIP_MEMORY_SCOPE_AGENT);
+    const bool last = ticket == expected - 1;
+    if (last) {
+      __builtin_amdgcn_fence(__ATOMIC_ACQUIRE, "agent");
+      asm volatile("s_waitcnt vmcnt(0)" ::: "memory");
+      __hip_atomic_store(counter, 0u, __ATOMIC_RELAXED, __HIP_MEMORY_SCOPE_AGENT);
+    }
+    last_flag = last ? 1u : 0u;
+  }
+  __syncthreads();
+  return last_flag != 0u;
+}
+
+template <int NCH>
+__device__ __forceinline__ bool bn_last_combine(const float* partial, int P, int C, int c0, double* dred, double* s_out,
+                                                double* q_out) {
+  for (int item = threadIdx.x; item < 16 * NCH; item += blockDim.x) {
+    const int ch = item % NCH, g = item / NCH, c = c0 + ch;
+    double s = 0.0, q = 0.0;
+    if (c < C) {
+#pragma unroll 4
+      for (int p = g; p < P; p += 16) {
+        s += (double)bn_load_agent(partial + ((long)p * 2 + 0) * C + c);
+        q += (double)bn_load_agent(partial + ((long)p * 2 + 1) * C + c);
+      }
+    }
+    dred[(0 * 16 + g) * NCH + ch] = s;
+    dred[(1 * 16 + g) * NCH + ch] = q;
+  }
+  __syncthreads();
+  const int ch = threadIdx.x;
+  if (ch >= NCH || c0 + ch >= C) return false;
+  double ss = 0.0, qq = 0.0;
+#pragma unroll
+  for (int k = 0; k < 16; ++k) { ss += dred[(0 * 16 + k) * NCH + ch]; qq += dred[(1 * 16 + k) * NCH + ch]; }
+  *s_out = ss;
+  *q_out = qq;
+  return true;
+}
+
+__device__ __forceinline__ BnChannelStats bn_last_stats(double s, double q, long M, float gamma, float beta, float eps) {
+#pragma clang fp contract(off)
+  BnChannelStats r;
+  const double mean = s / (double)M;
+  double var = fma(-mean, mean, q / (double)M);
+  if (var < 0.0) var = 0.0;
+  r.mean = (float)mean;
+  r.invstd = (float)(1.0 / sqrt(var + (double)eps));
+  r.scale = gamma * r.invstd;
+  r.shift = fmaf(-r.scale, r.mean, beta);
+  r.unbiased_var = (float)((M > 1) ? var * ((double)M / (double)(M - 1)) : var);
+  return r;
+}
+__device__ __forceinline__ float bn_last_moving_update(float moving, float momentum, float value) {
+#pragma clang fp contract(off)
+  const float kept = momentum * moving;
+  const float fresh = (1.f - momentum) * value;
+  return kept + fresh;
+}
+
+template <int NCH>
+__device__ __forceinline__ void bn_last_finalize_fwd(const BnLastFwd& f, const float* partial, int P, int C, int c0,
+                                                     double* dred) {
+  double s, q;
+  if (!bn_last_combine<NCH>(partial, P, C, c0, dred, &s, &q)) return;
+  const int c = c0 + threadIdx.x;
+  const BnChannelStats st = bn_last_stats(s, q, f.M, f.gamma[c], f.beta[c], f.eps);
+  f.save_mean[c] = st.mean;
+  f.save_invstd[c] = st.invstd;
+  f.scale[c] = st.scale;
+  f.shift[c] = st.shift;
+  f.moving_mean[c] = bn_last_moving_update(f.moving_mean[c], f.momentum, st.mean);
+  f.moving_var[c] = bn_last_moving_update(f.moving_var[c], f.momentum, st.unbiased_var);
+}
+
+template <int NCH>
+__device__ __forceinline__ void bn_last_finalize_bwd(const BnLastBwd& f, const float* partial, int P, int C, int c0,
+                                                     double* dred) {
+  double sg, sgx;
+  if (!bn_last_combine<NCH>(partial, P, C, c0, dred, &sg, &sgx)) return;
+  {
+#pragma clang fp contract(off)
+    const int c = c0 + threadIdx.x;
+    f.dbeta[c] = (float)sg;
+    f.dgamma[c] = (float)sgx;
+    const double is = (double)f.invstd[c];
+    const double a = (double)f.gamma[c] * is;
+    const double b = -a * sgx / (double)f.M, d = -a * sg / (double)f.M;
+    f.k1[c] = (float)a;
+    f.k2[c] = (float)b;
+    f.k3[c] = (float)d;
+  }
+}
+
 __device__ __forceinline__ int xcd_remap(int bid, int nblk) {
   const int nx = 8;
   int q = nblk / nx, r = nblk % nx;
diff --git a/spnet_amd/csrc/gemm_bf16x3.hip b/spnet_amd/csrc/gemm_bf16x3.hip
--- a/spnet_amd/csrc/gemm_bf16x3.hip
+++ b/spnet_amd/csrc/gemm_bf16x3.hip
@@ -129,7 +129,7 @@
     }                                                                                                          \
   }
 
-#define X3_COLSTATS()                                                                                          \
+#define X3_COLSTATS_(ST_)                                                                                        \
   do {                                                                                                         \
     __syncthreads();                                                                                           \
     float* sred = reinterpret_cast<float*>(smem);                              \
@@ -153,14 +153,17 @@
     __syncthreads();                                                                                           \
     if (tid < 2 * X3_BN) {                                                                                     \
       const int q = tid / X3_BN, cl = tid % X3_BN, col = n0 + cl;                                              \
-      if (col < N) colstats[((long)tm * 2 + q) * N + col] = sred[(q * 2 + 0) * X3_BN + cl] + sred[(q * 2 + 1) * X3_BN + cl]; \
-    }                                                                                                          \
-  } while (0)
-
+      if (col < N) ST_(colstats + ((long)tm * 2 + q) * N + col, sred[(q * 2 + 0) * X3_BN + cl] + sred[(q * 2 + 1) * X3_BN + cl]); \
+    }                                                                                                          \
+  } while (0)
+#define X3_ST_PLAIN(P_, V_) (*(P_) = (V_))
+#define X3_COLSTATS() X3_COLSTATS_(X3_ST_PLAIN)
+
+template <bool FIN>
 __global__ __launch_bounds__(256, 2) void gemm_bf16x3_pp_kernel(const unsigned short* __restrict__ Ap, long a_ps,
                                                                 const unsigned short* __restrict__ Bp, long b_ps,
                                                                 float* __restrict__ C, int ldc, int M, int N, int nk, int tiles_n,
-                                                                float* __restrict__ colstats) {
+                                                                float* __restrict__ colstats, BnLastFwd fin) {
   __shared__ __attribute__((aligned(16))) unsigned short smem[2 * X3_STEP];
   const int tid = threadIdx.x, lane = tid & 63;
   const int wave = __builtin_amdgcn_readfirstlane(tid >> 6);
@@ -202,7 +205,14 @@
   X3_PIPELINE(nk, X3_READ_ROWS, 1);
 #undef X3_ISSUE
   X3_STORE_C(C, ldc, m0, n0, M, N);
-  if (colstats) X3_COLSTATS();
+  if (FIN) {
+    X3_COLSTATS_(bn_store_agent);
+    const int tiles_m = gridDim.x / tiles_n;
+    if (!bn_last_arriver(fin.counters + tn, tiles_m)) return;
+    bn_last_finalize_fwd<X3_BN>(fin, colstats, tiles_m, N, n0, reinterpret_cast<double*>(smem));
+  } else if (colstats) {
+    X3_COLSTATS();
+  }
 }
 
 #undef X3_NDMA
@@ -210,13 +220,14 @@
 #define FB_BM 192
 #define FB_STEP (3 * (FB_BM + X3_BN) * X3_LDR)
 #define FB_LD 100
-template <int MODE, bool ADD, bool BNX>
+template <int MODE, bool ADD, bool BNX, bool FIN = false>
 __global__ __launch_bounds__(512, 2) void gemm_bf16x3_pp_dwbwd_kernel(
     const unsigned short* __restrict__ Ap, long a_ps, const unsigned short* __restrict__ Bp, long b_ps, int M, int N, int nk,
     int tiles_n, int H, int W, const float* __restrict__ x, const float* __restrict__ wt, float* __restrict__ dx, int relu_in,
     const float* __restrict__ add, float* __restrict__ partial, const float* __restrict__ in_scale,
     const float* __restrict__ in_shift, const float* __restrict__ bn_mean, const float* __restrict__ bn_invstd,
-    float* __restrict__ bn_partial, const float* __restrict__ bn_x, unsigned short* __restrict__ out_planes, long out_ps) {
+    float* __restrict__ bn_partial, const float* __restrict__ bn_x, unsigned short* __restrict__ out_planes, long out_ps,
+    BnLastBwd fin) {
   __shared__ __attribute__((aligned(16))) unsigned short smem[2 * FB_STEP];
   const int tid = threadIdx.x, lane = tid & 63;
   const int wave = __builtin_amdgcn_readfirstlane(tid >> 6);
@@ -459,8 +470,18 @@
       v4 sum = red[(tp * 16) * 32 + ll];
       for (int g = 1; g < 16; ++g) sum += red[(tp * 16 + g) * 32 + ll];
       if (tp < 9) *reinterpret_cast<v4*>(partial + ((long)tm * 9 + tp) * N + co) = sum;
+      else if (FIN) {
+        float* dst = bn_partial + ((long)tm * 2 + (tp - 9)) * N + co;
+        bn_store_agent(dst + 0, sum.x); bn_store_agent(dst + 1, sum.y);
+        bn_store_agent(dst + 2, sum.z); bn_store_agent(dst + 3, sum.w);
+      }
       else *reinterpret_cast<v4*>(bn_partial + ((long)tm * 2 + (tp - 9)) * N + co) = sum;
     }
+  }
+  if (FIN) {
+    const int tiles_m = gridDim.x / tiles_n;
+    if (!bn_last_arriver(fin.counters + tn, tiles_m)) return;
+    bn_last_finalize_bwd<X3_BN>(fin, bn_partial, tiles_m, N, n0, reinterpret_cast<double*>(smem));
   }
 }
 #undef X3_NDMA
@@ -727,10 +748,30 @@
   if (!x3_planes_ok(a_planes, M, K) || !x3_planes_ok(b_planes, N, K)) return (int)hipErrorInvalidValue;
   const int tm = spnet_cdiv(M, X3_BM), tn = spnet_cdiv(N, X3_BN);
   if (stat_rows) *stat_rows = tm;
-  hipLaunchKernelGGL(gemm_bf16x3_pp_kernel, dim3(tm * tn), dim3(256), 0, (hipStream_t)stream,
+  hipLaunchKernelGGL(gemm_bf16x3_pp_kernel<false>, dim3(tm * tn), dim3(256), 0, (hipStream_t)stream,
                      reinterpret_cast<const unsigned short*>(a_planes), x3t_plane_elems(M, K),
                      reinterpret_cast<const unsigned short*>(b_planes), x3t_plane_elems(N, K), C, ldc, M, N, (K + 31) / 32, tn,
-                     colstats);
+                     colstats, BnLastFwd{});
+  SPNET_RETURN_LAUNCH_STATUS();
+}
+
+extern "C" int spnet_gemm_bf16x3_pp_bnlast(const void* a_planes, const void* b_planes, float* C, int ldc, int M, int N, int K,
+                                           float* colstats, int* stat_rows, const float* gamma, const float* beta,
+                                           float* moving_mean, float* moving_var, float* save_mean, float* save_invstd,
+                                           float* scale_shift, float eps, float momentum, void* counters, void* stream) {
+  if (!C || M < 1 || N < 1 || K < 1 || ldc < N || !colstats || !stat_rows) return (int)hipErrorInvalidValue;
+  if (!gamma || !beta || !moving_mean || !moving_var || !save_mean || !save_invstd || !scale_shift || !counters)
+    return (int)hipErrorInvalidValue;
+  if (!x3_planes_ok(a_planes, M, K) || !x3_planes_ok(b_planes, N, K)) return (int)hipErrorInvalidValue;
+  const int tm = spnet_cdiv(M, X3_BM), tn = spnet_cdiv(N, X3_BN);
+  if (tn > BN_LAST_MAX_BLOCKS || tm >= 1024) return (int)hipErrorInvalidValue;
+  *stat_rows = tm;
+  const BnLastFwd fin{gamma, beta, moving_mean, moving_var, save_mean, save_invstd, scale_shift, scale_shift + N,
+                      reinterpret_cast<unsigned*>(counters), (long)M, eps, momentum};
+  hipLaunchKernelGGL(gemm_bf16x3_pp_kernel<true>, dim3(tm * tn), dim3(256), 0, (hipStream_t)stream,
+                     reinterpret_cast<const unsigned short*>(a_planes), x3t_plane_elems(M, K),
+                     reinterpret_cast<const unsigned short*>(b_planes), x3t_plane_elems(N, K), C, ldc, M, N, (K + 31) / 32, tn,
+                     colstats, fin);
   SPNET_RETURN_LAUNCH_STATUS();
 }
 
@@ -753,7 +794,38 @@
                      reinterpret_cast<const unsigned short*>(dy_planes), x3t_plane_elems(M, cout),                              \
                      reinterpret_cast<const unsigned short*>(w_planes), x3t_plane_elems(cin, cout), (int)M, cin, (cout + 31) / 32, tn, \
                      H, W, x_fwd, w, dx, relu_in, add, partial, in_scale, in_shift, bn_mean, bn_invstd, bn_partial, bn_x,        \
-                     (unsigned short*)nullptr, 0L)
+                     (unsigned short*)nullptr, 0L, BnLastBwd{})
+  if (add && bn_x) FB_LAUNCH(true, true);
+  else if (add) FB_LAUNCH(true, false);
+  else if (bn_x) FB_LAUNCH(false, true);
+  else FB_LAUNCH(false, false);
+#undef FB_LAUNCH
+  SPNET_RETURN_LAUNCH_STATUS();
+}
+
+extern "C" int spnet_gemm_bf16x3_pp_dwbwd_bnlast(const void* dy_planes, const void* w_planes, int B, int H, int W, int cin,
+                                                 int cout, const float* x_fwd, const float* w, float* dx, int relu_in,
+                                                 const float* add, float* partial, const float* in_scale,
+                                                 const float* in_shift, const float* bn_mean, const float* bn_invstd,
+                                                 float* bn_partial, const float* bn_x, const float* bn_gamma,
+                                                 float* bn_dgamma, float* bn_dbeta, float* bn_coef, int cld, void* counters,
+                                                 void* stream) {
+  const long M = (long)B * H * W;
+  if (!x_fwd || !w || !dx || !partial || B < 1 || !spnet_gemm_bf16x3_dwbwd_ok(H, W, cin)) return (int)hipErrorInvalidValue;
+  if (!bn_partial || !bn_mean || !bn_invstd || !bn_gamma || !bn_dgamma || !bn_dbeta || !bn_coef || cld < cin || !counters)
+    return (int)hipErrorInvalidValue;
+  if (!x3_planes_ok(dy_planes, M, cout) || !x3_planes_ok(w_planes, cin, cout)) return (int)hipErrorInvalidValue;
+  if ((((uintptr_t)x_fwd) | ((uintptr_t)dx) | ((uintptr_t)add) | ((uintptr_t)bn_x) | ((uintptr_t)w)) & 15) return (int)hipErrorInvalidValue;
+  const int tm = spnet_cdiv(M, FB_BM), tn = spnet_cdiv(cin, X3_BN);
+  if (tn > BN_LAST_MAX_BLOCKS) return (int)hipErrorInvalidValue;
+  const BnLastBwd fin{bn_gamma, bn_invstd, bn_dgamma, bn_dbeta, bn_coef, bn_coef + cld, bn_coef + 2 * cld,
+                      reinterpret_cast<unsigned*>(counters), M};
+#define FB_LAUNCH(ADD_, BNX_)                                                                                  \
+  hipLaunchKernelGGL((gemm_bf16x3_pp_dwbwd_kernel<0, ADD_, BNX_, true>), dim3(tm * tn), dim3(512), 0, (hipStream_t)stream,          \
+                     reinterpret_cast<const unsigned short*>(dy_planes), x3t_plane_elems(M, cout),                              \
+                     reinterpret_cast<const unsigned short*>(w_planes), x3t_plane_elems(cin, cout), (int)M, cin, (cout + 31) / 32, tn, \
+                     H, W, x_fwd, w, dx, relu_in, add, partial, in_scale, in_shift, bn_mean, bn_invstd, bn_partial, bn_x,        \
+                     (unsigned short*)nullptr, 0L, fin)
   if (add && bn_x) FB_LAUNCH(true, true);
   else if (add) FB_LAUNCH(true, false);
   else if (bn_x) FB_LAUNCH(false, true);
@@ -776,7 +848,8 @@
                      reinterpret_cast<const unsigned short*>(w_planes), x3t_plane_elems(cout, cin), (int)M, cout, (cin + 31) / 32, tn,
                      H, W, (const float*)nullptr, w_next, (float*)nullptr, relu_next, (const float*)nullptr, (float*)nullptr,
                      scale_shift, scale_shift ? scale_shift + cout : nullptr, (const float*)nullptr, (const float*)nullptr,
-                     (float*)nullptr, (const float*)nullptr, reinterpret_cast<unsigned short*>(out_planes), x3t_plane_elems(M, cout));
+                     (float*)nullptr, (const float*)nullptr, reinterpret_cast<unsigned short*>(out_planes), x3t_plane_elems(M, cout),
+                     BnLastBwd{});
   SPNET_RETURN_LAUNCH_STATUS();
 }
 
diff --git a/spnet_amd/engine.py b/spnet_amd/engine.py
--- a/spnet_amd/engine.py
+++ b/spnet_amd/engine.py
@@ -9,6 +9,7 @@
 
 BN_EPS = 1e-3
 BN_MOMENTUM = 0.99
+BN_LAST_MAX_BLOCKS = 32
 L2_COEF = 1e-4
 ACT_NONE, ACT_RELU, ACT_LRELU, ACT_RELU6 = 0, 1, 2, 3
 BACKBONES = ("Xception", "MobileNet", "InceptionResNetV2", "DenseNet121")
@@ -545,13 +546,16 @@
 class Engine:
     def __init__(self, H, W, batch, n_out=576, device="cuda:0", loss_type="same", seed=0,
                  train=True, adam_eps=1e-7, share_from=None, rank=0, sigmoid_cols=None, backbone="Xception",
-                 pointwise="bf16x3", x3_min_tiles=192, fuse_dw_bwd=True, early_head=True):
+                 pointwise="bf16x3", x3_min_tiles=192, fuse_dw_bwd=True, early_head=True, bn_finalize="producer"):
         if pointwise not in ("bf16x3", "f32"):
             raise ValueError("pointwise must be 'bf16x3' or 'f32'")
         self._pointwise = pointwise
         self.fuse_dw_bwd = bool(fuse_dw_bwd)
         self.fuse_dw_fwd = bool(fuse_dw_bwd)
         self.early_head = bool(early_head)
+        if bn_finalize not in ("producer", "launch"):
+            raise ValueError("bn_finalize must be 'producer' or 'launch'")
+        self.bn_finalize = bn_finalize
         self.x3_min_tiles = int(x3_min_tiles)
         self.fuse_min_tiles = 256 if self.x3_min_tiles else 0
         if not torch.cuda.is_available():
@@ -1259,6 +1263,21 @@
         tag = "x3p aB" if colstats_region is None else "x3p aB+stats"
         return self._x3p(tag, zp, self.planes(0), y, self.cout, self.cin, colstats_region)
 
+    def fwd_p_bnlast(self, zp, y, bn):
+        e = self.e
+        prof = e.prof
+        t0 = prof.start() if prof is not None else None
+        N, K = self.cout, self.cin
+        if (self.M + 95) // 96 * 2 * N > WS_BNP[1]:
+            raise RuntimeError("BatchNorm partial region too small for M=%d N=%d" % (self.M, N))
+        L.spnet_gemm_bf16x3_pp_bnlast(L.ptr(zp), L.ptr(self.planes(0)), L.ptr(y), N, self.M, N, K, e.ws_ptr(WS_BNP),
+                                      __import__("ctypes").addressof(_stat_rows), L.ptr(bn.gamma), L.ptr(bn.beta),
+                                      L.ptr(bn.mm), L.ptr(bn.mv), bn.mean_ptr, bn.invstd_ptr, L.ptr(bn.ss), bn.eps,
+                                      BN_MOMENTUM, bn.counters.data_ptr(), _stream())
+        if prof is not None:
+            prof.stop("gemm", t0, 2.0 * self.M * N * K, ("x3p aB+stats", self.M, N, K))
+        return _stat_rows.value
+
     def bwd_p(self, zp, dyp, dx):
         e = self.e
         if self.defer_wgrad:
@@ -1383,6 +1402,9 @@
             self.save = eng.new(2 * C)
             self.cld = (C + 63) // 64 * 64
             self.coef = torch.zeros(3 * self.cld, device=eng.dev, dtype=torch.float32)
+            self.counters = torch.zeros(2 * BN_LAST_MAX_BLOCKS, device=eng.dev, dtype=torch.int32)
+        self.unit = None
+        self.coef_ready = False
 
     def coeffs_from_partials(self, rows):
         e = self.e
@@ -1445,6 +1467,16 @@
         L.spnet_bn_bwd_x3(L.ptr(x), L.ptr(g), self.M, C, L.ptr(self.gamma), L.ptr(self.beta), self.mean_ptr,
                           self.invstd_ptr, act, L.ptr(out_planes), L.ptr(self.ggamma), L.ptr(self.gbeta),
                           L.ptr(e.small[:3 * C]), e.ws_ptr(WS_MISC), _stream())
+        return out_planes
+
+    def last_ok(self, rows):
+        return (self.e.bn_finalize == "producer" and self.e.train_capable and rows <= 256
+                and (self.C + 95) // 96 <= BN_LAST_MAX_BLOCKS)
+
+    def bwd_apply_x3(self, x, g, out_planes):
+        L.spnet_bn_bwd_apply_x3(L.ptr(x), L.ptr(g), self.M, self.C, L.ptr(self.gamma), L.ptr(self.beta), self.mean_ptr,
+                                self.invstd_ptr, L.ptr(self.coef), self.cld, L.ptr(out_planes), _stream())
+        self.coef_ready = False
         return out_planes
 
     def bwd_from_partials_x3(self, x, g, out_planes, rows):
@@ -1513,6 +1545,7 @@
         self.z = None if self.x3p else eng.new(B, H, W, cin)
         self.zp = eng.new_planes(self.M, cin) if self.x3p else None
         self.bn = BN(eng, cout, self.M, name + "_bn")
+        self.bn.unit = self
         self.y = eng.new(B, H, W, cout) if mode == "apply" else None
         self.dwb = _DwBwdPlan(B, H, W, cin)
         self.fuse_bwd = bool(self.x3p and eng.train_capable and eng.fuse_dw_bwd and L.spnet_gemm_bf16x3_dwbwd_ok(H, W, cin)
@@ -1572,7 +1605,9 @@
                                                   sb.shift_ptr if sb else None)
         if prof is not None and ran_dw:
             prof.stop("dw", t0, 2.0 * 4 * self.M * self.cin, ("dw fwd", self.H, self.W, self.cin))
-        if training:
+        if training and self.x3p and self.bn.last_ok((self.M + 95) // 96):
+            self.pw.fwd_p_bnlast(self.zp, self.yp, self.bn)
+        elif training:
             rows = self.pw.fwd_p(self.zp, self.yp, WS_BNP) if self.x3p else self.pw.fwd_colstats(self.z, self.yp)
             if self.fin_by_consumer and rows <= 128:
                 self.pending_rows = rows
@@ -1614,7 +1649,9 @@
                 self.bn.coeffs_full(self.yp, g)
             self.pw.bwd_blend(self.z, g, self.yp, self.bn, self.dyb, self.dz)
         elif self.x3p:
-            if from_partials:
+            if from_partials and self.bn.coef_ready:
+                self.bn.bwd_apply_x3(self.yp, g, self.dyp)
+            elif from_partials:
                 self.bn.bwd_from_partials_x3(self.yp, g, self.dyp, self.consumer_rows)
             else:
                 self.bn.bwd_full_x3(self.yp, g, self.dyp, self.act if self.mode == "apply" else ACT_NONE)
@@ -1623,12 +1660,18 @@
                 st = self.src.stats_bn if self.src.stats_bn is not None else sb
                 prof = e.prof
                 t0 = prof.start() if prof is not None else None
-                L.spnet_gemm_bf16x3_pp_dwbwd(L.ptr(self.dyp), L.ptr(self.pw.planes(1)), e.B, self.H, self.W, self.cin,
-                                             self.cout, L.ptr(self.src.t), L.ptr(self.wd), L.ptr(self.dx), self.relu_in,
-                                             L.ptr(add), L.ptr(self.wpart), sb.scale_ptr if sb else None,
-                                             sb.shift_ptr if sb else None, st.mean_ptr if st else None,
-                                             st.invstd_ptr if st else None, e.ws_ptr(WS_BNP) if st else None,
-                                             L.ptr(self.src.stats_x), _stream())
+                a = (L.ptr(self.dyp), L.ptr(self.pw.planes(1)), e.B, self.H, self.W, self.cin, self.cout, L.ptr(self.src.t),
+                     L.ptr(self.wd), L.ptr(self.dx), self.relu_in, L.ptr(add), L.ptr(self.wpart),
+                     sb.scale_ptr if sb else None, sb.shift_ptr if sb else None, st.mean_ptr if st else None,
+                     st.invstd_ptr if st else None, e.ws_ptr(WS_BNP) if st else None, L.ptr(self.src.stats_x))
+                su = st.unit if st is not None else None
+                if (su is not None and su.x3p and not su.blend and su.consumer_rows == self.rows_src
+                        and (su.mode == "lazy" or su.act == ACT_NONE) and st.last_ok(self.rows_src)):
+                    L.spnet_gemm_bf16x3_pp_dwbwd_bnlast(*a, L.ptr(st.gamma), L.ptr(st.ggamma), L.ptr(st.gbeta), L.ptr(st.coef),
+                                                        st.cld, st.counters.data_ptr() + 4 * BN_LAST_MAX_BLOCKS, _stream())
+                    st.coef_ready = True
+                else:
+                    L.spnet_gemm_bf16x3_pp_dwbwd(*a, _stream())
                 if prof is not None:
                     prof.stop("gemm", t0, 2.0 * self.M * self.cin * self.cout, ("x3p ab+dwbwd", self.M, self.cin, self.cout))
                 return self.dx
```

Measured after the change: 3066 images/sec. -5.3%, worse.
